# FangjinhuaWang/PatchmatchNet

Hardware: AMD Instinct MI355X
Metric: depth-maps/sec at 1600x1200 N=5 src views (higher is better)
Workload: dtype f32

## Files before the change

### include/pmn_hip.h

```cpp
#ifndef PMN_HIP_H
#define PMN_HIP_H

#include <stdint.h>

#ifdef __cplusplus
extern "C" {
#endif

#define PMN_ABI_VERSION 25
#define PMN_MLP_FLOATS 340
#define PMN_MAX_DEPTH 64
#define PMN_MAX_NEIGHBORS 17
#define PMN_MAX_FUSE_SRC 32
#define PMN_TSDF_MAX_VIEWS 16
#define PMN_TSDF_MARK_SPAN 8
#define PMN_RASTER_MAX_DIM 16384
#define PMN_RASTER_MAX_BOX 64
#define PMN_SPLAT_MAX_RADIUS 32

#define PMN_OK 0
#define PMN_ERR_ARG (-1)
#define PMN_ERR_SHAPE (-2)
#define PMN_ERR_LAUNCH (-3)

int pmn_abi_version(void);

const char *pmn_error_string(int code);

int pmn_nchw_to_nhwc(const float *in, float *out, int B, int C, int h, int w, void *stream);

int pmn_feature_weight(const float *ref_nhwc, const float *eval_offsets, const int *eval_table_host,
                       const float *mlp, int B, int C, int G, int K, int h, int w,
                       float *out_feature_weight, void *stream);

int pmn_init_hypotheses(const float *noise, const float *depth, int depth_shift, const float *depth_min,
                        const float *depth_max, int num_sample, float interval_scale, const float *propa_offsets,
                        const int *propa_table_host, int K, int B, int h, int w, float *depth_sample,
                        float *xnorm, void *stream);

int pmn_warp_correlate(const float *ref_nhwc, const float *src_nhwc, const float *rel_proj,
                       const float *depth_sample, const float *view_weights_in, int vw_shift,
                       const float *similarity_mlp, const float *pixelwise_mlp, int B, int N, int C,
                       int G, int D, int h, int w, int hs, int ws, float *cost_out, float *view_weights_out,
                       int *vw_argmax_out, float *similarity_out, void *stream);

int pmn_warp_correlate_views(const float *ref_nhwc, const void *src_view_table, const float *rel_proj,
                             const float *depth_sample, const float *view_weights_in, int vw_shift,
                             const float *similarity_mlp, const float *pixelwise_mlp, int B, int N, int C,
                             int G, int D, int h, int w, int hs, int ws, float *cost_out, float *view_weights_out,
                             int *vw_argmax_out, float *similarity_out, void *stream);

int pmn_aggregate_regress(const float *cost, const float *depth_sample, const float *xnorm,
                          const float *feature_weight, const float *eval_offsets, const int *eval_table_host,
                          int K, float interval_scale, int is_inverse, int B, int D, int h, int w,
                          float *score_out, float *depth_out, void *stream);

int pmn_confidence(const float *score, int B, int D, int h, int w, int H, int W, float *confidence_out,
                   int *depth_index_out, void *stream);

int pmn_conv2d(const float *in, const float *weights, const float *shift, const float *up, float *out, int N, int H,
               int W, int cin, int cout, int K, int stride, int pad, int dil, int relu, int in_nchw, int out_nchw,
               int up_h, int up_w, void *stream);

int pmn_fpn_tail(const float *x, const float *up, const float *w_in, const float *b_in, const float *w_out, float *out,
                 int N, int H, int W, int cin, int cmid, int cout, void *stream);

int pmn_conv2d_mfma(const float *in, const float *weights, const float *shift, float *out, float *out_b, int N, int H, int W,
                    int cin, int cout, int ca, int K, int stride, int pad, int dil, int relu, int planar, void *stream);


int pmn_conv2d_f16s(const float *in, const void *weights, const float *shift, float *out, int N, int H, int W, int cin, int cout,
                    int k, int stride, int relu, void *stream);

int pmn_conv2d_f16s_pair(const float *in, const void *weights_a, const float *shift_a, const void *weights_b, const float *shift_b,
                         float *out, int N, int H, int W, int channels, int relu, void *stream);

int pmn_offset_heads_f16s(const float *in, const void *weights, const float *shift, float *out_a, float *out_b, int N, int H, int W,
                          int cin, int cout, int ca, int dil, void *stream);

int pmn_fpn_level(const float *x, const float *u, const float *w, const float *b, float *out_a, float *out_b, int N, int H,
                  int W, int cin, int cout, int ca, void *stream);

int pmn_deconv3x3s2(const float *in, const float *weights, const float *shift, float *out, int N, int Hi, int Wi, int cin,
                    int cout, int relu, void *stream);

int pmn_refine_front(const float *img, const float *t2, const float *w0, const float *s0, const float *wd, const float *sd,
                     float *x16, int B, int H, int W, void *stream);
int pmn_refine_tail(const float *x16, const float *w3, const float *s3, const float *wr, const float *dnorm,
                    const float *depth_min, const float *depth_max, float *out, int B, int H, int W, void *stream);

int pmn_refine_fused(const float *img, const float *t2, const float *w0, const float *s0, const float *wd, const float *sd,
                     const void *w3a, const float *s3, const float *wr, const float *dnorm, const float *depth_min,
                     const float *depth_max, float *out, int B, int H, int W, void *stream);

int pmn_stage_projections(const float *intrinsics, const float *extrinsics, int B, int V, int nstages, float scale0,
                          float *rel, void *stream);

int pmn_stem(const float *img, const float *w0, const float *s0, const float *w1, const float *s1, float *out, int N, int H,
             int W, void *stream);

int pmn_stem_f16s(const float *img, const float *w0, const float *s0, const void *w1a, const float *s1, float *out, int N, int H,
                  int W, void *stream);

int pmn_stem_f16s_views(const float *const *img_table, int views, const float *w0, const float *s0, const void *w1a,
                        const float *s1, float *out, int B, int H, int W, void *stream);

int pmn_differentiable_warping(const float *src_nchw, const float *rel_proj, const float *depth, int B, int C,
                               int D, int h, int w, int hs, int ws, float *warped, void *stream);

int pmn_fuse_view(const float *maps, long long slot_stride, int ref_slot, const int *src_slots_host,
                  const int *src_hw_host, int n_src, const float *mats, int H, int W, float geo_pixel_thres, float geo_depth_thres, int geo_mask_thres,
                  float photo_thres, unsigned char *masks, float *xyz, double *depth_avg, int *geo_sum, void *stream);

int pmn_fuse_view_merged(const float *maps, long long slot_stride, int ref_slot, const int *src_slots_host,
                         const int *src_hw_host, int n_src, const float *mats, int H, int W, float geo_pixel_thres,
                         float geo_depth_thres, int geo_mask_thres, float photo_thres, unsigned char *masks, float *xyz,
                         double *depth_avg, int *geo_sum, unsigned char *claimed, long long claim_stride, unsigned char *emit,
                         void *stream);

int pmn_pack_points(const unsigned char *final_mask, const float *xyz, const void *image_hwc, int image_is_float, int H, int W,
                    unsigned char *records, long long capacity_points, long long *cursor, int *view_count, long long *scratch,
                    void *stream);

int pmn_pack_points_normals(const unsigned char *final_mask, const float *xyz, const float *normals_chw, const float *rotation,
                            int rotation_stride, const void *image_hwc, int image_is_float, int H, int W, unsigned char *records,
                            long long capacity_points, long long *cursor, int *view_count, long long *scratch, void *stream);

int pmn_depth_normals(const float *depth, int H, int W, const float *intrinsics_host, int radius, float rel_thres,
                      float *normals_out, void *stream);

int pmn_normalize_depth(const float *depth, const float *depth_min, const float *depth_max, int B, int n, float *out,
                        void *stream);

int pmn_check_f16_domain(const float *x, long long n, int *flag, void *stream);

#define PMN_PLAN_PART_PRE 0
#define PMN_PLAN_PART_SIDE 1
#define PMN_PLAN_PART_MAIN 2
#define PMN_PLAN_PART_POST 3
int pmn_plan_create(void **plan_out);
int pmn_plan_begin(void *plan);
int pmn_plan_end(void *plan);
int pmn_plan_count(const void *plan);
const char *pmn_plan_kernel_name(const void *plan, int index);
int pmn_plan_launch(const void *plan, void *stream);
int pmn_plan_destroy(void *plan);
int pmn_plan_fork(void *plan);
int pmn_plan_switch(void *plan, int branch);
int pmn_plan_join(void *plan);
int pmn_plan_entry_branch(const void *plan, int index);
int pmn_plan_launch_part(const void *plan, int part, void *stream);

int pmn_view_scores(const double *cam_centers, const double *xyz, const long long *obs_ptr, const int *obs_pt,
                    const long long *trk_ptr, const int *trk_img, int N, int P, long long n_obs, long long n_trk,
                    double theta0, double sigma1, double sigma2, double *score, void *stream);

#define PMN_METRICS_MAX_STAGES 4
#define PMN_METRICS_MAX_ITERS 5
#define PMN_METRICS_MAX_THRESHOLDS 8
#define PMN_METRICS_COUNT 0
#define PMN_METRICS_ABS 4
#define PMN_METRICS_THR 8
#define PMN_METRICS_SL1 16
#define PMN_METRICS_ROW 36
#define PMN_METRICS_PIXELS_PER_BLOCK 4096
#define PMN_METRICS_MAX_BLOCKS 128
#define PMN_METRICS_BLOCKS(H, W)                                                                                                     \
    ((int)((((long long)(H) * (W) + PMN_METRICS_PIXELS_PER_BLOCK - 1) / PMN_METRICS_PIXELS_PER_BLOCK) > PMN_METRICS_MAX_BLOCKS        \
               ? PMN_METRICS_MAX_BLOCKS                                                                                               \
               : (((long long)(H) * (W) + PMN_METRICS_PIXELS_PER_BLOCK - 1) / PMN_METRICS_PIXELS_PER_BLOCK)))
#define PMN_METRICS_SCRATCH(B, H, W) ((long long)(B) * PMN_METRICS_BLOCKS(H, W) * PMN_METRICS_ROW)
int pmn_depth_metrics(const float *depth_gt, const float *depth_min, const float *const *maps_host, const int *iters_host,
                      const int *hw_host, int stages, const float *thresholds_host, int n_thresholds, int B, int H, int W,
                      double *scratch, long long scratch_doubles, double *rows, void *stream);

int pmn_nn_distance(const float *to_xyz, const long long *to_keys, long long n_to, const double *origin_host, double cell,
                    const int *dims_host, const float *query, const int *order, long long n_from, double max_dist, double *dist,
                    int *index, void *stream);
int pmn_reduce_round(const float *xyz, const long long *keys, long long n, const double *origin_host, double cell,
                     const int *dims_host, double dst, const int *rank, unsigned char *state, unsigned int *counter, void *stream);

int pmn_tsdf_integrate(float *tsdf, float *weight, float *rgb, float *cweight, const int *dims_host, const float *origin_host,
                       float voxel, float trunc, const float *maps, long long slot_stride, const int *slots_host,
                       const int *hw_host, const void *const *masks_host, const void *const *images_host, const float *cams_host,
                       int n_views, void *stream);
int pmn_mt_count(const float *tsdf, const float *weight, const int *dims_host, float min_weight, unsigned char *vertex_mask,
                 unsigned char *cell_triangles, void *stream);
int pmn_mt_emit(const float *tsdf, const float *weight, const float *rgb, const float *cweight, const int *dims_host,
                const float *origin_host, float voxel, float min_weight, const unsigned char *vertex_mask,
                const unsigned char *cell_triangles, const int *vertex_scan, const int *triangle_scan, float *vertices,
                unsigned char *colors, float *normals, int *faces, void *stream);

int pmn_tsdf_mark_blocks(unsigned char *flags, int *overflow, const int *dims_host, const float *origin_host, float voxel, float trunc,
                         const float *maps, long long slot_stride, const int *slots_host, const int *hw_host,
                         const void *const *masks_host, const float *inv_cams_host, int n_views, void *stream);
int pmn_tsdf_integrate_blocks(float *tsdf, float *weight, float *rgb, float *cweight, const int *blocks, int n_blocks,
                              const int *dims_host, const float *origin_host, float voxel, float trunc, const float *maps,
                              long long slot_stride, const int *slots_host, const int *hw_host, const void *const *masks_host,
                              const void *const *images_host, const float *cams_host, int n_views, void *stream);
int pmn_mt_count_blocks(const float *tsdf, const float *weight, const int *table, const int *blocks, int n_blocks,
                        const int *dims_host, float min_weight, unsigned char *vertex_mask, unsigned char *cell_triangles, void *stream);
int pmn_mt_emit_blocks(const float *tsdf, const float *weight, const float *rgb, const float *cweight, const int *table,
                       const int *blocks, int n_blocks, const int *dims_host, const float *origin_host, float voxel, float min_weight,
                       const unsigned char *vertex_mask, const unsigned char *cell_triangles, const int *vertex_scan,
                       const int *triangle_scan, float *vertices, unsigned char *colors, float *normals, int *faces, void *stream);

int pmn_raster_triangles(const float *vertices, int n_vertices, const int *faces, int n_faces, const float *cam_host, int h, int w,
                         long long max_box, unsigned long long *keys, int *counters, int *worklist, void *stream);
int pmn_splat_points(const float *points, long long n_points, const float *cam_host, int h, int w, float radius_px, float radius_world,
                     unsigned long long *keys, int *counters, void *stream);
int pmn_raster_resolve(const unsigned long long *keys, int h, int w, const float *cam_host, const float *vertices, long long n_vertices,
                       const int *faces, long long n_faces, const unsigned char *colors, const float *normals, int shade, float *depth,
                       int *index, unsigned char *rgb, float *normal, void *stream);

#define PMN_ICP_SUMS 17
#define PMN_ICP_LIMBS 5
#define PMN_ICP_BLOCK_POINTS 256
#define PMN_ICP_BLOCKS(n) (((long long)(n) + PMN_ICP_BLOCK_POINTS - 1) / PMN_ICP_BLOCK_POINTS)
#define PMN_ICP_SCRATCH(n) (PMN_ICP_BLOCKS(n) * PMN_ICP_SUMS * PMN_ICP_LIMBS)
#define PMN_VOXEL_LONG_RUN 256
#define PMN_VOXEL_MAX_CHANNELS 8
#define PMN_CROP_MAX_VERTICES 4096
int pmn_icp_accumulate(const float *to_xyz, const long long *to_keys, long long n_to, const double *origin_host, double cell,
                       const int *dims_host, const float *src, const int *order, long long n, const double *pose_host,
                       const double *centre_host, double max_dist, double *scratch, long long scratch_doubles, double *sums,
                       void *stream);
int pmn_voxel_mean(const float *xyz, const float *attr, int channels, long long n, const long long *starts, long long m, float *out_xyz,
                   float *out_attr, void *stream);
int pmn_crop_prism(const float *xyz, long long n, const double *polygon, int k, int axis, double axis_min, double axis_max,
                   const double *pose_host, unsigned char *mask, void *stream);

int pmn_mesh_components(const int *faces, int n_faces, int n_vertices, int *label, int *invalid, void *stream);
int pmn_mesh_face_samples(const float *vertices, int n_vertices, const int *faces, int n_faces, double density, unsigned long long seed,
                          int *counts, int *invalid, void *stream);
int pmn_mesh_sample(const float *vertices, int n_vertices, const int *faces, int n_faces, const unsigned char *colors,
                    const long long *sample_scan, long long n_samples, unsigned long long seed, float *points, int *face,
                    unsigned char *out_colors, void *stream);

int pmn_undistort_image(const unsigned char *src, int Hs, int Ws, int channels, int model, const double *src_params_host,
                        const double *dst_pinhole_host, int Hd, int Wd, unsigned char *dst, unsigned char *valid, double *coords,
                        void *stream);

int pmn_knn_distance(const float *to_xyz, const long long *to_keys, long long n_to, const double *origin_host, double cell,
                     const int *dims_host, const float *query, const int *order, long long n_from, int k, double max_dist,
                     int same_cloud, double *d2, int *index, double *mean, void *stream);
int pmn_radius_count(const float *to_xyz, const long long *to_keys, long long n_to, const double *origin_host, double cell,
                     const int *dims_host, const float *query, const int *order, long long n_from, double radius, int same_cloud,
                     int *count, void *stream);

int pmn_mesh_distance(const float *ref_xyz, const long long *ref_keys, long long n_ref, const double *origin_host, double cell,
                      const int *dims_host, const int *entry_face, double radius, const float *vertices, int n_vertices,
                      const int *faces, int n_faces, const float *query, const int *order, long long n_query, double max_dist,
                      double *dist, int *face, double *closest, int *invalid, void *stream);

#define PMN_MESH_PLACE_LONG_RUN 256
#define PMN_MESH_SIMPLIFY_MAX_FACES 715827882
int pmn_mesh_remap_faces(const int *faces, int n_faces, int n_vertices, const int *cluster, int n_clusters, int *corner_cluster,
                         int *out_faces, unsigned char *flag, int *invalid, void *stream);
int pmn_mesh_cluster_place(const float *vertices, int n_vertices, const int *faces, int n_faces, const int *corners,
                           const long long *corner_starts, const long long *cluster_keys, int n_clusters, const float *mean,
                           const double *origin_host, double cell, const int *dims_host, double stiffness, float *out, void *stream);

#ifdef __cplusplus
}
#endif
#endif
```

### patchmatchnet_amd/_lib.py

```python
from __future__ import annotations

import ctypes
import os
import subprocess
from typing import Optional

_CSRC = os.path.join(os.path.dirname(os.path.abspath(__file__)), "csrc")
LIB_PATH = os.path.join(_CSRC, "libpmn_hip.so")
ABI_VERSION = 25
MLP_FLOATS = 340
MAX_DEPTH = 64
MAX_NEIGHBORS = 17
MAX_FUSE_SRC = 32
TSDF_MAX_VIEWS = 16
TSDF_MARK_SPAN = 8
RASTER_MAX_DIM = 16384
RASTER_MAX_BOX = 64
SPLAT_MAX_RADIUS = 32
ICP_SUMS = 17
ICP_LIMBS = 5
ICP_BLOCK_POINTS = 256
VOXEL_LONG_RUN = 256
VOXEL_MAX_CHANNELS = 8
CROP_MAX_VERTICES = 4096
MESH_PLACE_LONG_RUN = 256
MESH_SIMPLIFY_MAX_FACES = 715827882

_fp = ctypes.c_void_p
_ip = ctypes.c_void_p
_hp = ctypes.c_void_p
_i = ctypes.c_int
_f = ctypes.c_float
_s = ctypes.c_void_p

SIGNATURES = {
    "pmn_abi_version": [],
    "pmn_error_string": [_i],
    "pmn_nchw_to_nhwc": [_fp, _fp, _i, _i, _i, _i, _s],
    "pmn_feature_weight": [_fp, _fp, _hp, _fp, _i, _i, _i, _i, _i, _i, _fp, _s],
    "pmn_init_hypotheses": [_fp, _fp, _i, _fp, _fp, _i, _f, _fp, _hp, _i, _i, _i, _i, _fp, _fp, _s],
    "pmn_warp_correlate": [_fp, _fp, _fp, _fp, _fp, _i, _fp, _fp, _i, _i, _i, _i, _i, _i, _i, _i, _i, _fp, _fp, _ip,
                           _fp, _s],
    "pmn_warp_correlate_views": [_fp, _fp, _fp, _fp, _fp, _i, _fp, _fp, _i, _i, _i, _i, _i, _i, _i, _i, _i, _fp, _fp, _ip,
                                 _fp, _s],
    "pmn_aggregate_regress": [_fp, _fp, _fp, _fp, _fp, _hp, _i, _f, _i, _i, _i, _i, _i, _fp, _fp, _s],
    "pmn_confidence": [_fp, _i, _i, _i, _i, _i, _i, _fp, _ip, _s],
    "pmn_conv2d": [_fp, _fp, _fp, _fp, _fp] + [_i] * 14 + [_s],
    "pmn_fpn_tail": [_fp] * 6 + [_i] * 6 + [_s],
    "pmn_fpn_level": [_fp] * 6 + [_i] * 6 + [_s],
    "pmn_conv2d_f16s": [_fp] * 4 + [_i] * 8 + [_s],
    "pmn_offset_heads_f16s": [_fp] * 5 + [_i] * 7 + [_s],
    "pmn_conv2d_f16s_pair": [_fp] * 6 + [_i] * 5 + [_s],
    "pmn_refine_front": [_fp] * 7 + [_i] * 3 + [_s],
    "pmn_refine_tail": [_fp] * 8 + [_i] * 3 + [_s],
    "pmn_refine_fused": [_fp] * 13 + [_i] * 3 + [_s],
    "pmn_conv2d_mfma": [_fp] * 5 + [_i] * 12 + [_s],
    "pmn_deconv3x3s2": [_fp] * 4 + [_i] * 6 + [_s],
    "pmn_stage_projections": [_fp, _fp, _i, _i, _i, _f, _fp, _s],
    "pmn_stem": [_fp] * 6 + [_i] * 3 + [_s],
    "pmn_stem_f16s": [_fp] * 6 + [_i] * 3 + [_s],
    "pmn_stem_f16s_views": [_fp, _i] + [_fp] * 5 + [_i] * 3 + [_s],
    "pmn_differentiable_warping": [_fp, _fp, _fp, _i, _i, _i, _i, _i, _i, _i, _fp, _s],
    "pmn_fuse_view": [_fp, ctypes.c_longlong, _i, _hp, _hp, _i, _fp, _i, _i, _f, _f, _i, _f, _fp, _fp, _fp, _ip, _s],
    "pmn_fuse_view_merged": [_fp, ctypes.c_longlong, _i, _hp, _hp, _i, _fp, _i, _i, _f, _f, _i, _f, _fp, _fp, _fp, _ip, _fp,
                             ctypes.c_longlong, _fp, _s],
    "pmn_pack_points": [_fp, _fp, _fp, _i, _i, _i, _fp, ctypes.c_longlong, _fp, _ip, _fp, _s],
    "pmn_pack_points_normals": [_fp, _fp, _fp, _fp, _i, _fp, _i, _i, _i, _fp, ctypes.c_longlong, _fp, _ip, _fp, _s],
    "pmn_depth_normals": [_fp, _i, _i, _hp, _i, _f, _fp, _s],
    "pmn_normalize_depth": [_fp, _fp, _fp, _i, _i, _fp, _s],
    "pmn_check_f16_domain": [_fp, ctypes.c_longlong, _ip, _s],
    "pmn_plan_create": [ctypes.POINTER(ctypes.c_void_p)],
    "pmn_plan_begin": [_hp],
    "pmn_plan_end": [_hp],
    "pmn_plan_count": [_hp],
    "pmn_plan_kernel_name": [_hp, _i],
    "pmn_plan_launch": [_hp, _s],
    "pmn_plan_destroy": [_hp],
    "pmn_plan_fork": [_hp],
    "pmn_plan_switch": [_hp, _i],
    "pmn_plan_join": [_hp],
    "pmn_plan_entry_branch": [_hp, _i],
    "pmn_plan_launch_part": [_hp, _i, _s],
    "pmn_view_scores": [_fp] * 6 + [_i, _i, ctypes.c_longlong, ctypes.c_longlong] + [ctypes.c_double] * 3 + [_fp, _s],
    "pmn_depth_metrics": [_fp, _fp, _hp, _hp, _hp, _i, _hp, _i, _i, _i, _i, _fp, ctypes.c_longlong, _fp, _s],
    "pmn_nn_distance": [_fp, _ip, ctypes.c_longlong, _hp, ctypes.c_double, _hp, _fp, _ip, ctypes.c_longlong, ctypes.c_double, _fp, _ip,
                        _s],
    "pmn_reduce_round": [_fp, _ip, ctypes.c_longlong, _hp, ctypes.c_double, _hp, ctypes.c_double, _ip, _ip, _ip, _s],
    "pmn_tsdf_integrate": [_fp] * 4 + [_hp, _hp, _f, _f, _fp, ctypes.c_longlong] + [_hp] * 5 + [_i, _s],
    "pmn_mt_count": [_fp, _fp, _hp, _f, _ip, _ip, _s],
    "pmn_mt_emit": [_fp] * 4 + [_hp, _hp, _f, _f] + [_ip] * 4 + [_fp, _ip, _fp, _ip, _s],
    "pmn_tsdf_mark_blocks": [_ip, _ip, _hp, _hp, _f, _f, _fp, ctypes.c_longlong] + [_hp] * 4 + [_i, _s],
    "pmn_tsdf_integrate_blocks": [_fp] * 4 + [_ip, _i, _hp, _hp, _f, _f, _fp, ctypes.c_longlong] + [_hp] * 5 + [_i, _s],
    "pmn_mt_count_blocks": [_fp, _fp, _ip, _ip, _i, _hp, _f, _ip, _ip, _s],
    "pmn_mt_emit_blocks": [_fp] * 4 + [_ip, _ip, _i, _hp, _hp, _f, _f] + [_ip] * 4 + [_fp, _ip, _fp, _ip, _s],
    "pmn_raster_triangles": [_fp, _i, _ip, _i, _hp, _i, _i, ctypes.c_longlong, _ip, _ip, _ip, _s],
    "pmn_splat_points": [_fp, ctypes.c_longlong, _hp, _i, _i, _f, _f, _ip, _ip, _s],
    "pmn_raster_resolve": [_ip, _i, _i, _hp, _fp, ctypes.c_longlong, _ip, ctypes.c_longlong, _ip, _fp, _i, _fp, _ip, _ip, _fp, _s],
    "pmn_icp_accumulate": [_fp, _ip, ctypes.c_longlong, _hp, ctypes.c_double, _hp, _fp, _ip, ctypes.c_longlong, _hp, _hp, ctypes.c_double,
                           _fp, ctypes.c_longlong, _fp, _s],
    "pmn_voxel_mean": [_fp, _fp, _i, ctypes.c_longlong, _ip, ctypes.c_longlong, _fp, _fp, _s],
    "pmn_crop_prism": [_fp, ctypes.c_longlong, _fp, _i, _i, ctypes.c_double, ctypes.c_double, _hp, _ip, _s],
    "pmn_mesh_components": [_ip, _i, _i, _ip, _ip, _s],
    "pmn_mesh_face_samples": [_fp, _i, _ip, _i, ctypes.c_double, ctypes.c_ulonglong, _ip, _ip, _s],
    "pmn_mesh_sample": [_fp, _i, _ip, _i, _ip, _ip, ctypes.c_longlong, ctypes.c_ulonglong, _fp, _ip, _ip, _s],
    "pmn_undistort_image": [_fp, _i, _i, _i, _i, _hp, _hp, _i, _i, _fp, _fp, _fp, _s],
    "pmn_knn_distance": [_fp, _ip, ctypes.c_longlong, _hp, ctypes.c_double, _hp, _fp, _ip, ctypes.c_longlong, _i, ctypes.c_double, _i,
                         _fp, _ip, _fp, _s],
    "pmn_radius_count": [_fp, _ip, ctypes.c_longlong, _hp, ctypes.c_double, _hp, _fp, _ip, ctypes.c_longlong, ctypes.c_double, _i, _ip,
                         _s],
    "pmn_mesh_distance": [_fp, _ip, ctypes.c_longlong, _hp, ctypes.c_double, _hp, _ip, ctypes.c_double, _fp, _i, _ip, _i, _fp, _ip,
                          ctypes.c_longlong, ctypes.c_double, _fp, _ip, _fp, _ip, _s],
    "pmn_mesh_remap_faces": [_ip, _i, _i, _ip, _i, _ip, _ip, _ip, _ip, _s],
    "pmn_mesh_cluster_place": [_fp, _i, _ip, _i, _ip, _ip, _ip, _i, _fp, _hp, ctypes.c_double, _hp, ctypes.c_double, _fp, _s],
}

PLAN_PART_PRE, PLAN_PART_SIDE, PLAN_PART_MAIN, PLAN_PART_POST = 0, 1, 2, 3

METRICS_MAX_STAGES = 4
METRICS_MAX_ITERS = 5
METRICS_MAX_THRESHOLDS = 8
METRICS_COUNT, METRICS_ABS, METRICS_THR, METRICS_SL1 = 0, 4, 8, 16
METRICS_ROW = 36
METRICS_PIXELS_PER_BLOCK = 4096
METRICS_MAX_BLOCKS = 128


def metrics_scratch(B: int, H: int, W: int) -> int:
    return B * min(METRICS_MAX_BLOCKS, -(-H * W // METRICS_PIXELS_PER_BLOCK)) * METRICS_ROW

def icp_scratch(n: int) -> int:
    return -(-n // ICP_BLOCK_POINTS) * ICP_SUMS * ICP_LIMBS


EXPERIMENTAL_SIGNATURES = {"pmn_set_tuning": [_i, _i],
                           "pmn_conv3x3_wino": [_fp] * 4 + [_i] * 5 + [_s],
                           "pmn_conv5x5s2_wino": [_fp] * 4 + [_i] * 6 + [_s]}
EXPERIMENTAL_LIB_PATH = os.path.join(_CSRC, "libpmn_hip_experimental.so")


def experimental() -> bool:
    return os.environ.get("PMN_EXPERIMENTAL", "") == "1"


_LIB: Optional[ctypes.CDLL] = None


class PmnError(RuntimeError):
    pass


def build(force: bool = False, verbose: bool = False) -> str:
    args = ["make", "-C", _CSRC, "-j4"] + (["-B"] if force else []) + (["EXPERIMENTAL=1"] if experimental() else [])
    if not verbose:
        args.insert(1, "-s")
    subprocess.check_call(args)
    return LIB_PATH


def lib() -> ctypes.CDLL:
    global _LIB
    if _LIB is None:
        path, sigs = LIB_PATH, SIGNATURES
        if experimental():
            path, sigs = EXPERIMENTAL_LIB_PATH, {**SIGNATURES, **EXPERIMENTAL_SIGNATURES}
        if not os.path.isfile(path):
            raise PmnError(f"{path} not found: build it with `python -c 'import __graft_entry__ as g; g.build()'` "
                           f"or `make -C patchmatchnet_amd/csrc` -- patchmatchnet_amd has no fallback path")
        L = (ctypes.CDLL if os.environ.get("PMN_CTYPES", "") == "cdll" else ctypes.PyDLL)(path)
        for name, argtypes in sigs.items():
            try:
                fn = getattr(L, name)
            except AttributeError as e:
                raise PmnError(f"libpmn_hip.so does not export {name}") from e
            fn.argtypes = argtypes
            fn.restype = ctypes.c_char_p if name in ("pmn_error_string", "pmn_plan_kernel_name") else ctypes.c_int
        if L.pmn_abi_version() != ABI_VERSION:
            raise PmnError(f"libpmn_hip.so ABI {L.pmn_abi_version()} != expected {ABI_VERSION}: rebuild")
        _LIB = L
    return _LIB


def check(code: int, what: str) -> None:
    if code != 0:
        raise PmnError(f"{what} failed: {lib().pmn_error_string(code).decode()} (code {code})")
```

### patchmatchnet_amd/csrc/aggregate.hip

```cpp
#include <cstring>

#include "pmn_common.hpp"
#define PMN_DIV_DM1(acc, D) ((acc) / (float)((D) - 1))

struct AggArgs {
    const float* cost;
    const float* depth;
    const float* xnorm;
    const float* fweight;
    const float* offsets;
    float* score;
    float* depth_out;
    int K, is_inverse, B, D, h, w;
    float interval_scale;
    int table[2 * PMN_MAX_NEIGHBORS];
};

template <int KMAX, int DL>
__global__ __launch_bounds__(PMN_BLOCK, (KMAX <= 9 ? 3 : 1)) void aggregate_regress_kernel(const AggArgs a) {
#pragma clang fp contract(off)
    constexpr int NPX = PMN_BLOCK / DL;
    __shared__ float red[DL][NPX];
    __shared__ float red2[DL][NPX];
    const int h = a.h, w = a.w, hw = h * w, D = a.D, K = a.K;
    const int px = threadIdx.x % NPX, dl = threadIdx.x / NPX;
    const int p_raw = blockIdx.x * NPX + px;
    const bool ok = p_raw < hw;
    const int p = ok ? p_raw : hw - 1;
    const int b = blockIdx.y;
    const int y = p / w, x = p - y * w;

    int off[KMAX];
    float w00[KMAX], w01[KMAX], w10[KMAX], w11[KMAX], fw[KMAX];
#pragma unroll
    for (int k = 0; k < KMAX; ++k) {
        off[k] = 0;
        w00[k] = w01[k] = w10[k] = w11[k] = fw[k] = 0.0f;
        if (k < K) {
            const float ox = a.offsets[((size_t)b * 2 * K + 2 * k) * hw + p];
            const float oy = a.offsets[((size_t)b * 2 * K + 2 * k + 1) * hw + p];
            float ix, iy;
            pmn_neighbor_position((float)x, (float)y, a.table[2 * k], a.table[2 * k + 1], ox, oy, h, w, ix, iy);
            const PmnTaps t = pmn_make_taps(ix, iy, h, w);
            off[k] = t.off;
            w00[k] = t.w00;
            w01[k] = t.w01;
            w10[k] = t.w10;
            w11[k] = t.w11;
            fw[k] = a.fweight[((size_t)b * K + k) * hw + p];
        }
    }

    float smax = -__builtin_inff();
#pragma unroll 1
    for (int d = dl; d < D; d += DL) {
        const float* xp = a.xnorm + (size_t)b * hw * D + d;
        const float* cp = a.cost + (size_t)b * hw * D + d;
        const float xc = xp[(size_t)p * D];
        float wk[KMAX], ck[KMAX];
        float wsum = 0.0f;
#pragma unroll
        for (int k = 0; k < KMAX; ++k) {
            wk[k] = 0.0f;
            ck[k] = 0.0f;
            if (k < K) {
                const size_t o = (size_t)off[k] * D, o1 = o + D, o2 = o + (size_t)w * D, o3 = o2 + D;
                const float x1 = fmaf(xp[o3], w11[k], fmaf(xp[o2], w10[k], fmaf(xp[o1], w01[k], xp[o] * w00[k])));
                ck[k] = fmaf(cp[o3], w11[k], fmaf(cp[o2], w10[k], fmaf(cp[o1], w01[k], cp[o] * w00[k])));
                float t = fabsf(x1 - xc) / a.interval_scale;
                t = fminf(fmaxf(t, 0.0f), 4.0f);
                wk[k] = pmn_sigmoid(4.0f - 2.0f * t) * fw[k];
                wsum = wsum + wk[k];
            }
        }
        float s = 0.0f;
#pragma unroll
        for (int k = 0; k < KMAX; ++k)
            if (k < K) s = s + ck[k] * (wk[k] / wsum);
        if (ok) a.score[((size_t)b * D + d) * hw + p] = s;
        smax = fmaxf(smax, s);
    }
    red[dl][px] = smax;
    __syncthreads();
#pragma unroll
    for (int i = 0; i < DL; ++i) smax = fmaxf(smax, red[i][px]);
    __syncthreads();

    float esum = 0.0f;
#pragma unroll 1
    for (int d = dl; d < D; d += DL)
        if (ok) esum = esum + expf(a.score[((size_t)b * D + d) * hw + p] - smax);
    red[dl][px] = esum;
    __syncthreads();
    esum = 0.0f;
#pragma unroll
    for (int i = 0; i < DL; ++i) esum = esum + red[i][px];
    const float lse = logf(esum);

    float acc = 0.0f;
#pragma unroll 1
    for (int d = dl; d < D; d += DL) {
        if (ok) {
            const size_t o = ((size_t)b * D + d) * hw + p;
            const float prob = expf((a.score[o] - smax) - lse);
            a.score[o] = prob;
            acc = acc + (a.is_inverse ? (float)d : a.depth[o]) * prob;
        }
    }
    red2[dl][px] = acc;
    __syncthreads();
    if (dl != 0 || !ok) return;
    acc = 0.0f;
#pragma unroll
    for (int i = 0; i < DL; ++i) acc = acc + red2[i][px];
    float out = acc;
    if (a.is_inverse) {
        const float inv_min = 1.0f / a.depth[((size_t)b * D + (D - 1)) * hw + p];
        const float inv_max = 1.0f / a.depth[((size_t)b * D) * hw + p];
        const float inv = inv_max + PMN_DIV_DM1(acc, D) * (inv_min - inv_max);
        out = 1.0f / inv;
    }
    a.depth_out[(size_t)b * hw + p] = out;
}

__device__ __forceinline__ float sigmoid_rcp(float x) {
    const float d = 1.0f + __builtin_amdgcn_exp2f(x * -1.4426950408889634f);
    float r = __builtin_amdgcn_rcpf(d);
    return r * fmaf(-d, r, 2.0f);
}

template <int G, int SL>
__device__ __forceinline__ int agg_group_bcast_i(int v) {
    static_assert(G == 2 || G == 4 || G == 8 || G == 16, "lane groups inside a DPP row");
    if constexpr (G == 2) {
        return __builtin_amdgcn_mov_dpp(v, SL | (SL << 2) | ((2 + SL) << 4) | ((2 + SL) << 6), 0xF, 0xF, true);
    } else if constexpr (G == 4) {
        return __builtin_amdgcn_mov_dpp(v, SL | (SL << 2) | (SL << 4) | (SL << 6), 0xF, 0xF, true);
    } else if constexpr (G == 16) {
        return __builtin_amdgcn_mov_dpp(v, 0x150 + SL, 0xF, 0xF, true);
    } else {
        const int lo = __builtin_amdgcn_update_dpp(v, v, 0x150 + SL, 0xF, 0x3, false);
        return __builtin_amdgcn_update_dpp(lo, v, 0x150 + 8 + SL, 0xF, 0xC, false);
    }
}
template <int G, int SL>
__device__ __forceinline__ float agg_group_bcast_f(float v) {
    return __int_as_float(agg_group_bcast_i<G, SL>(__float_as_int(v)));
}

template <int KMAX>
__device__ __forceinline__ void agg_form_tap_set(const AggArgs& a, int b, int k, int p, int x, int y, int& off, float& w00, float& w01,
                                                 float& w10, float& w11, float& fw) {
    const int h = a.h, w = a.w, hw = h * w, K = a.K;
    const float ox = a.offsets[((size_t)b * 2 * K + 2 * k) * hw + p];
    const float oy = a.offsets[((size_t)b * 2 * K + 2 * k + 1) * hw + p];
    float ix, iy;
    pmn_neighbor_position((float)x, (float)y, a.table[2 * k], a.table[2 * k + 1], ox, oy, h, w, ix, iy);
    const PmnTaps t = pmn_make_taps(ix, iy, h, w);
    off = t.off;
    w00 = t.w00;
    w01 = t.w01;
    w10 = t.w10;
    w11 = t.w11;
    fw = a.fweight[((size_t)b * K + k) * hw + p];
}

template <int KMAX, int DQT>
__global__ __launch_bounds__(PMN_BLOCK, (KMAX <= 9 ? 3 : 1)) void aggregate_regress_q4_kernel(const AggArgs a) {
#pragma clang fp contract(off)
    __shared__ float red[PMN_BLOCK];
    const int h = a.h, w = a.w, hw = h * w, D = a.D, K = a.K, DQ = DQT > 0 ? DQT : D >> 2;
    const int npx = blockDim.x / DQ;
    const int px = threadIdx.x / DQ, q = threadIdx.x - px * DQ;
    const int p_raw = blockIdx.x * npx + px;
    const bool ok = p_raw < hw;
    const int p = ok ? p_raw : hw - 1;
    const int b = blockIdx.y;
    const int y = p / w, x = p - y * w;

    int off[KMAX];
    float w00[KMAX], w01[KMAX], w10[KMAX], w11[KMAX], fw[KMAX];
    if constexpr (DQT > 1) {
        constexpr int KPT = (KMAX + DQT - 1) / DQT;
        int moff[KPT];
        float m00[KPT], m01[KPT], m10[KPT], m11[KPT], mfw[KPT];
#pragma unroll
        for (int i = 0; i < KPT; ++i) {
            const int k = q + i * DQT;
            moff[i] = 0;
            m00[i] = m01[i] = m10[i] = m11[i] = mfw[i] = 0.0f;
            if (k < K) agg_form_tap_set<KMAX>(a, b, k, p, x, y, moff[i], m00[i], m01[i], m10[i], m11[i], mfw[i]);
        }
#define AGG_TAKE(k_)                                                                                         \
    if constexpr ((k_) < KMAX) {                                                                               \
        constexpr int sl_ = (k_) % DQT, it_ = (k_) / DQT;                                                      \
        off[k_] = agg_group_bcast_i<DQT, sl_>(moff[it_]);                                                      \
        w00[k_] = agg_group_bcast_f<DQT, sl_>(m00[it_]);                                                       \
        w01[k_] = agg_group_bcast_f<DQT, sl_>(m01[it_]);                                                       \
        w10[k_] = agg_group_bcast_f<DQT, sl_>(m10[it_]);                                                       \
        w11[k_] = agg_group_bcast_f<DQT, sl_>(m11[it_]);                                                       \
        fw[k_] = agg_group_bcast_f<DQT, sl_>(mfw[it_]);                                                        \
    }
        AGG_TAKE(0) AGG_TAKE(1) AGG_TAKE(2) AGG_TAKE(3) AGG_TAKE(4) AGG_TAKE(5) AGG_TAKE(6) AGG_TAKE(7) AGG_TAKE(8)
        static_assert(KMAX <= 9, "AGG_TAKE list");
#undef AGG_TAKE
    } else {
#pragma unroll
        for (int k = 0; k < KMAX; ++k) {
            off[k] = 0;
            w00[k] = w01[k] = w10[k] = w11[k] = fw[k] = 0.0f;
            if (k < K) agg_form_tap_set<KMAX>(a, b, k, p, x, y, off[k], w00[k], w01[k], w10[k], w11[k], fw[k]);
        }
    }

    const float inv_interval = 1.0f / a.interval_scale;
    const float* xn = a.xnorm + (size_t)b * hw * D + 4 * q;
    const float* cs = a.cost + (size_t)b * hw * D + 4 * q;
    const float4 xc4 = *reinterpret_cast<const float4*>(xn + (size_t)p * D);
    const float xc[4] = {xc4.x, xc4.y, xc4.z, xc4.w};
    float wk[KMAX][4], ck[KMAX][4], wsum[4] = {0.f, 0.f, 0.f, 0.f};
#pragma unroll
    for (int k = 0; k < KMAX; ++k) {
#pragma unroll
        for (int j = 0; j < 4; ++j) wk[k][j] = ck[k][j] = 0.0f;
        if (k < K) {
            const size_t o = (size_t)off[k] * D, o2 = o + (size_t)w * D;
            const float4 xa = *reinterpret_cast<const float4*>(xn + o), xb = *reinterpret_cast<const float4*>(xn + o + D);
            const float4 xcn = *reinterpret_cast<const float4*>(xn + o2), xd = *reinterpret_cast<const float4*>(xn + o2 + D);
            const float4 ca = *reinterpret_cast<const float4*>(cs + o), cb = *reinterpret_cast<const float4*>(cs + o + D);
            const float4 cc = *reinterpret_cast<const float4*>(cs + o2), cd = *reinterpret_cast<const float4*>(cs + o2 + D);
            const float x00[4] = {xa.x, xa.y, xa.z, xa.w}, x01[4] = {xb.x, xb.y, xb.z, xb.w};
            const float x10[4] = {xcn.x, xcn.y, xcn.z, xcn.w}, x11[4] = {xd.x, xd.y, xd.z, xd.w};
            const float c00[4] = {ca.x, ca.y, ca.z, ca.w}, c01[4] = {cb.x, cb.y, cb.z, cb.w};
            const float c10[4] = {cc.x, cc.y, cc.z, cc.w}, c11[4] = {cd.x, cd.y, cd.z, cd.w};
#pragma unroll
            for (int j = 0; j < 4; ++j) {
                const float x1 = fmaf(x11[j], w11[k], fmaf(x10[j], w10[k], fmaf(x01[j], w01[k], x00[j] * w00[k])));
                ck[k][j] = fmaf(c11[j], w11[k], fmaf(c10[j], w10[k], fmaf(c01[j], w01[k], c00[j] * w00[k])));
                float t = fabsf(x1 - xc[j]) * inv_interval;
                t = fminf(fmaxf(t, 0.0f), 4.0f);
                wk[k][j] = sigmoid_rcp(4.0f - 2.0f * t) * fw[k];
                wsum[j] = wsum[j] + wk[k][j];
            }
        }
    }
    float s[4] = {0.f, 0.f, 0.f, 0.f}, rsum[4];
#pragma unroll
    for (int j = 0; j < 4; ++j) rsum[j] = 1.0f / wsum[j];
#pragma unroll
    for (int k = 0; k < KMAX; ++k)
        if (k < K) {
#pragma unroll
            for (int j = 0; j < 4; ++j) s[j] = s[j] + ck[k][j] * (wk[k][j] * rsum[j]);
        }

    float smax = fmaxf(fmaxf(s[0], s[1]), fmaxf(s[2], s[3]));
    red[threadIdx.x] = smax;
    __syncthreads();
    for (int i = 0; i < DQ; ++i) smax = fmaxf(smax, red[px * DQ + i]);
    __syncthreads();
    float esum = ((expf(s[0] - smax) + expf(s[1] - smax)) + expf(s[2] - smax)) + expf(s[3] - smax);
    red[threadIdx.x] = esum;
    __syncthreads();
    esum = 0.0f;
    for (int i = 0; i < DQ; ++i) esum = esum + red[px * DQ + i];
    __syncthreads();
    const float lse = logf(esum);
    float acc = 0.0f;
#pragma unroll
    for (int j = 0; j < 4; ++j) {
        const int d = 4 * q + j;
        const size_t o = ((size_t)b * D + d) * hw + p;
        const float prob = expf((s[j] - smax) - lse);
        if (ok) a.score[o] = prob;
        acc = acc + (a.is_inverse ? (float)d : a.depth[o]) * prob;
    }
    red[threadIdx.x] = acc;
    __syncthreads();
    if (q != 0 || !ok) return;
    acc = 0.0f;
    for (int i = 0; i < DQ; ++i) acc = acc + red[px * DQ + i];
    float out = acc;
    if (a.is_inverse) {
        const float inv_min = 1.0f / a.depth[((size_t)b * D + (D - 1)) * hw + p];
        const float inv_max = 1.0f / a.depth[((size_t)b * D) * hw + p];
        const float inv = inv_max + PMN_DIV_DM1(acc, D) * (inv_min - inv_max);
        out = 1.0f / inv;
    }
    a.depth_out[(size_t)b * hw + p] = out;
}

template <int KMAX>
static int launch_agg_q4(const AggArgs& a, hipStream_t s) {
    const int DQ = a.D / 4, npx = PMN_BLOCK / DQ;
    const dim3 grid((a.h * a.w + npx - 1) / npx, a.B), block(npx * DQ);
    if (DQ == 2) PMN_LAUNCH((aggregate_regress_q4_kernel<KMAX, 2>), grid, block, 0, s, a);
    else if (DQ == 4) PMN_LAUNCH((aggregate_regress_q4_kernel<KMAX, 4>), grid, block, 0, s, a);
    else if (DQ == 8) PMN_LAUNCH((aggregate_regress_q4_kernel<KMAX, 8>), grid, block, 0, s, a);
    else if (DQ == 16) PMN_LAUNCH((aggregate_regress_q4_kernel<KMAX, 16>), grid, block, 0, s, a);
    else PMN_LAUNCH((aggregate_regress_q4_kernel<KMAX, 0>), grid, block, 0, s, a);
    PMN_CHECK_LAUNCH();
    return PMN_OK;
}

template <int KMAX, int DL>
static int launch_agg_dl(const AggArgs& a, hipStream_t s) {
    constexpr int NPX = PMN_BLOCK / DL;
    const dim3 grid((a.h * a.w + NPX - 1) / NPX, a.B), block(PMN_BLOCK);
    PMN_LAUNCH((aggregate_regress_kernel<KMAX, DL>), grid, block, 0, s, a);
    PMN_CHECK_LAUNCH();
    return PMN_OK;
}

template <int KMAX>
static int launch_agg(const AggArgs& a, hipStream_t s) {
    if constexpr (KMAX <= 9) {
        if (a.D % 4 == 0) return launch_agg_q4<KMAX>(a, s);
    }
    if (a.D >= 32) return launch_agg_dl<KMAX, 16>(a, s);
    if (a.D >= 16) return launch_agg_dl<KMAX, 4>(a, s);
    return launch_agg_dl<KMAX, 1>(a, s);
}

extern "C" int pmn_aggregate_regress(const float* cost, const float* depth_sample, const float* xnorm,
                                     const float* feature_weight, const float* eval_offsets, const int* eval_table_host,
                                     int K, float interval_scale, int is_inverse, int B, int D, int h, int w,
                                     float* score_out, float* depth_out, void* stream) {
    if (!cost || !depth_sample || !xnorm || !feature_weight || !eval_offsets || !eval_table_host || !score_out ||
        !depth_out)
        return PMN_ERR_ARG;
    if (B < 1 || D < 1 || h < 2 || w < 2) return PMN_ERR_ARG;
    if (K < 1 || K > PMN_MAX_NEIGHBORS || D > PMN_MAX_DEPTH) return PMN_ERR_SHAPE;
    if (is_inverse && D < 2) return PMN_ERR_ARG;
    AggArgs a;
    memset(&a, 0, sizeof(a));
    a.cost = cost;
    a.depth = depth_sample;
    a.xnorm = xnorm;
    a.fweight = feature_weight;
    a.offsets = eval_offsets;
    a.score = score_out;
    a.depth_out = depth_out;
    a.K = K;
    a.is_inverse = is_inverse;
    a.B = B; a.D = D; a.h = h; a.w = w;
    a.interval_scale = interval_scale;
    for (int i = 0; i < 2 * K; ++i) a.table[i] = eval_table_host[i];
    if (K <= 9) return launch_agg<9>(a, (hipStream_t)stream);
    return launch_agg<17>(a, (hipStream_t)stream);
}
```

### patchmatchnet_amd/csrc/gather_corr.hip

```cpp
#include <type_traits>

#include "gather_common.hpp"


template <int LPI, int SL>
__device__ __forceinline__ int group_bcast_i(int v) {
    if constexpr (LPI == 4) {
        return __builtin_amdgcn_mov_dpp(v, SL | (SL << 2) | (SL << 4) | (SL << 6), 0xF, 0xF, true);
    } else if constexpr (LPI == 16) {
        return __builtin_amdgcn_mov_dpp(v, 0x150 + SL, 0xF, 0xF, true);
    } else {
        const int lo = __builtin_amdgcn_update_dpp(v, v, 0x150 + SL, 0xF, 0x3, false);
        return __builtin_amdgcn_update_dpp(lo, v, 0x150 + 8 + SL, 0xF, 0xC, false);
    }
}
template <int LPI, int SL>
__device__ __forceinline__ float group_bcast_f(float v) {
    return __int_as_float(group_bcast_i<LPI, SL>(__float_as_int(v)));
}

template <int C>
__device__ __forceinline__ const char* pmn_view_base(const GatherArgs& a, int v, int b, int hs, int ws) {
    if (a.src_tab) return reinterpret_cast<const char*>(a.src_tab[v]) + ((size_t)b * hs * ws) * (C * 4);
    return reinterpret_cast<const char*>(a.src) + ((size_t)(v * a.B + b) * hs * ws) * (C * 4);
}

struct PmnCorners { float4 t00, t01, t10, t11; };

typedef float pmn_f4n __attribute__((ext_vector_type(4)));
typedef const pmn_f4n __attribute__((address_space(1))) * pmn_gptr4;
__device__ __forceinline__ float4 pmn_global_load4(const char __attribute__((address_space(1))) * p) {
    const pmn_f4n v = *(pmn_gptr4)p;
    return make_float4(v.x, v.y, v.z, v.w);
}
template <int C>
__device__ __forceinline__ PmnCorners load_corners(const char* __restrict__ sbase, const unsigned bo, const unsigned row_bytes) {
    typedef const char __attribute__((address_space(1))) * gptr1;
    const gptr1 g = (gptr1)sbase;
    PmnCorners c;
    c.t00 = pmn_global_load4(g + bo);
    c.t01 = pmn_global_load4(g + bo + C * 4);
    c.t10 = pmn_global_load4(g + (bo + row_bytes));
    c.t11 = pmn_global_load4(g + (bo + row_bytes) + C * 4);
    return c;
}

template <int LPG, int CG>
__device__ __forceinline__ float blend_corners(const PmnCorners& c, float4 w4, const float4 refq) {
    w4 = pmn_settle4(w4);
    const pmn_f2 wa = {w4.x, w4.x}, wb = {w4.y, w4.y}, wc = {w4.z, w4.z}, wd = {w4.w, w4.w};
    pmn_f2 lo = pmn_f2{c.t00.x, c.t00.y} * wa;
    pmn_f2 hi = pmn_f2{c.t00.z, c.t00.w} * wa;
    lo = __builtin_elementwise_fma(pmn_f2{c.t01.x, c.t01.y}, wb, lo);
    hi = __builtin_elementwise_fma(pmn_f2{c.t01.z, c.t01.w}, wb, hi);
    lo = __builtin_elementwise_fma(pmn_f2{c.t10.x, c.t10.y}, wc, lo);
    hi = __builtin_elementwise_fma(pmn_f2{c.t10.z, c.t10.w}, wc, hi);
    lo = __builtin_elementwise_fma(pmn_f2{c.t11.x, c.t11.y}, wd, lo);
    hi = __builtin_elementwise_fma(pmn_f2{c.t11.z, c.t11.w}, wd, hi);
    float s = fmaf(hi.y, refq.w, fmaf(hi.x, refq.z, fmaf(lo.y, refq.y, lo.x * refq.x)));
    if (LPG == 2) s += pmn_pair_swap(s);
    return s * (1.0f / CG);
}

template <int C, int G, int MODE, int DT, bool EXACT>
__global__ __launch_bounds__(PMN_BLOCK, (MODE == MODE_PIXELWISE ? 3 : (MODE == MODE_NEIGHBOR && DT <= 16) ? 5 : 4)) void gather_corr_kernel(const GatherArgs a) {
    constexpr int LPI = C / 4;
    constexpr int NPIX = PMN_BLOCK / LPI;
    constexpr int CG = C / G;
    constexpr int LPG = CG / 4;
    constexpr int PAD = 32 / G;
    constexpr int DSTEP = PMN_BLOCK / NPIX;
    constexpr int NIT = DT / DSTEP;
    constexpr int NI_MAX = (MODE == MODE_PIXELWISE) ? 2 : 4;
    constexpr int NI = NIT < NI_MAX ? NIT : NI_MAX;
    static_assert(CG == 4 || CG == 8, "group size must be 4 or 8 channels");
    static_assert(NIT >= 1, "DT must cover at least one hypothesis per item-role thread");

    const int tid = threadIdx.x;
    const int b = blockIdx.y;
    const int tile = pmn_xcd_tile(blockIdx.x, a.ntiles);
    constexpr int DEXACT = (MODE == MODE_NEIGHBOR) ? (DT == 16 ? 9 : 17) : DT;
    const int D = EXACT ? DEXACT : a.D;
    const int N = a.N, h = a.h, w = a.w, hs = a.hs, ws = a.ws;
    const int hw = h * w;
    const int items = NPIX * D;
    const int SS = items + PAD;
    const int p0 = tile * NPIX;

    extern __shared__ float4 smem4[];
    float* simt = reinterpret_cast<float*>(smem4);
    float* wlds_a = simt + ((G * SS + 3) & ~3);
    float* wlds_b = wlds_a + MLP_LDS_FLOATS;
    unsigned long long* vwkey = reinterpret_cast<unsigned long long*>(wlds_b + MLP_LDS_FLOATS);
    int* tab = reinterpret_cast<int*>(vwkey + NPIX);

    for (int i = tid; i < PMN_MLP_FLOATS; i += PMN_BLOCK) {
        wlds_a[i] = a.mlp_a[i];
        if (MODE == MODE_PIXELWISE) wlds_b[i] = a.mlp_b[i];
    }
    if (MODE == MODE_NEIGHBOR) {
#pragma unroll
        for (int i = 0; i < 2 * PMN_MAX_NEIGHBORS; ++i)
            if (tid == i) tab[i] = a.table[i];
    }

    const int pixA = tid % NPIX, dA0 = tid / NPIX;
    const int pA = p0 + pixA;
    const bool okA = pA < hw;
    const int yA = okA ? pA / w : 0, xA = okA ? pA - yA * w : 0;

    const int grp = tid / LPI, lc = tid % LPI;
    const int pB = p0 + grp;
    const bool okB = pB < hw;
    float4 refq = make_float4(0.f, 0.f, 0.f, 0.f);
    if (okB) refq = reinterpret_cast<const float4*>(a.ref)[((size_t)b * hw + pB) * LPI + lc];
    const int yB = okB ? pB / w : 0, xB = okB ? pB - yB * w : 0;
    const int wv = w >> a.vw_shift, hwv = (h >> a.vw_shift) * wv;
    const int vw_idx = (yB >> a.vw_shift) * wv + (xB >> a.vw_shift);
    const bool owner = (lc % LPG) == 0;
    const int gB = lc / LPG;


    if (MODE == MODE_VIEWS) {
        constexpr int RPL = DT / LPI;
        static_assert(DT % LPI == 0, "DT is a multiple of the lane-group size");
        float acc[DT];
#pragma unroll
        for (int d = 0; d < DT; ++d) acc[d] = 0.0f;
        const float xf = (float)xB, yf = (float)yB;
        float rdep[RPL];
#pragma unroll
        for (int j = 0; j < RPL; ++j) {
            const int d = lc + j * LPI;
            rdep[j] = (okB && d < D) ? a.depth[((size_t)b * D + d) * hw + pB] : -1.0f;
        }
        for (int v = 0; v < N; ++v) {
            const PmnPose lane_pose = pmn_make_pose(a.proj + ((size_t)b * N + v) * 16, xf, yf, h, w);
            float rw00[RPL], rw01[RPL], rw10[RPL], rw11[RPL];
            int roff[RPL];
#pragma unroll
            for (int j = 0; j < RPL; ++j) {
                const int d = lc + j * LPI;
                PmnTaps t;
                t.off = 0;
                t.w00 = t.w01 = t.w10 = t.w11 = 0.0f;
                if (okB && d < D) {
                    float ix, iy;
                    pmn_pose_position(lane_pose, rdep[j], h, w, hs, ws, ix, iy);
                    t = pmn_make_taps(ix, iy, hs, ws);
                }
                rw00[j] = t.w00; rw01[j] = t.w01; rw10[j] = t.w10; rw11[j] = t.w11;
                roff[j] = t.off;
            }
            const char* sbase = pmn_view_base<C>(a, v, b, hs, ws);
            const unsigned lane_bytes = lc * 16u, row_bytes = (unsigned)ws * (C * 4);
            const float vw = okB ? a.vw_in[((size_t)b * N + v) * hwv + vw_idx] : 0.0f;
            constexpr int NB = 2;
            static_assert(DT % NB == 0, "hypothesis bound is a multiple of the batch");
#pragma unroll
            for (int d0 = 0; d0 < DT; d0 += NB) {
                PmnCorners cn[NB];
                float4 wq[NB];
#pragma unroll
                for (int i = 0; i < NB; ++i) {
                    const int d = d0 + i;
                    if (EXACT || d < D) {
                        float4 w4;
                        int off;
#define PMN_BCAST_CASE(SL)                                                    \
    case SL:                                                                  \
        w4.x = group_bcast_f<LPI, SL>(rw00[d / LPI]);                         \
        w4.y = group_bcast_f<LPI, SL>(rw01[d / LPI]);                         \
        w4.z = group_bcast_f<LPI, SL>(rw10[d / LPI]);                         \
        w4.w = group_bcast_f<LPI, SL>(rw11[d / LPI]);                         \
        off = group_bcast_i<LPI, SL>(roff[d / LPI]);                          \
        break;
                        switch (d % LPI) {
                            PMN_BCAST_CASE(0) PMN_BCAST_CASE(1) PMN_BCAST_CASE(2) PMN_BCAST_CASE(3)
                            PMN_BCAST_CASE(4) PMN_BCAST_CASE(5) PMN_BCAST_CASE(6) PMN_BCAST_CASE(7)
                            PMN_BCAST_CASE(8) PMN_BCAST_CASE(9) PMN_BCAST_CASE(10) PMN_BCAST_CASE(11)
                            PMN_BCAST_CASE(12) PMN_BCAST_CASE(13) PMN_BCAST_CASE(14) PMN_BCAST_CASE(15)
                            default: w4 = make_float4(0.f, 0.f, 0.f, 0.f); off = 0; break;
                        }
#undef PMN_BCAST_CASE
                        wq[i] = w4;
                        cn[i] = load_corners<C>(sbase, (unsigned)off * (C * 4) + lane_bytes, row_bytes);
                    }
                }
                __builtin_amdgcn_sched_barrier(0);
#pragma unroll
                for (int i = 0; i < NB; ++i) {
                    const int d = d0 + i;
                    if (EXACT || d < D) acc[d] = mul_add_unfused(acc[d], blend_corners<LPG, CG>(cn[i], wq[i], refq), vw);
                }
                __builtin_amdgcn_sched_barrier(0);
            }
        }
        if (owner) {
#pragma unroll
            for (int d = 0; d < DT; ++d)
                if (d < D) simt[gB * SS + d * NPIX + grp] = acc[d];
        }
        __syncthreads();
        if (!okA) return;
        float wtot = 1e-5f;
        const int vwi = (yA >> a.vw_shift) * wv + (xA >> a.vw_shift);
        for (int v = 0; v < N; ++v) wtot += a.vw_in[((size_t)b * N + v) * hwv + vwi];
        float x[NIT][G], o[NIT];
#pragma unroll
        for (int j = 0; j < NIT; ++j) {
            const int d = min(dA0 + j * DSTEP, D - 1);
#pragma unroll
            for (int g = 0; g < G; ++g) x[j][g] = simt[g * SS + d * NPIX + pixA] / wtot;
        }
        mlp_items<G, NIT, NI>(wlds_a, x, o);
#pragma unroll
        for (int j = 0; j < NIT; ++j) {
            const int d = dA0 + j * DSTEP;
            if (d < D) {
                if (a.sim_out) {
#pragma unroll
                    for (int g = 0; g < G; ++g) a.sim_out[(((size_t)b * G + g) * D + d) * hw + pA] = x[j][g];
                }
                a.out[((size_t)b * hw + pA) * D + d] = o[j];
            }
        }
        return;
    }

    float ssum[NIT][G];
#pragma unroll
    for (int j = 0; j < NIT; ++j)
#pragma unroll
        for (int g = 0; g < G; ++g) ssum[j][g] = 0.0f;
    float wsum = 1e-5f;
    __syncthreads();

    for (int v = 0; v < N; ++v) {
        if (MODE == MODE_PIXELWISE && tid < NPIX) vwkey[tid] = 0ull;
        const char* sbase = MODE == MODE_NEIGHBOR ? reinterpret_cast<const char*>(a.ref) + ((size_t)b * hs * ws) * (C * 4)
                                                  : pmn_view_base<C>(a, v, b, hs, ws);
        const unsigned lane_bytes = lc * 16u, row_bytes = (unsigned)ws * (C * 4);
        if constexpr (MODE == MODE_PIXELWISE) {
            constexpr int RPL = DT / LPI;
            const float xf = (float)xB, yf = (float)yB;
            const PmnPose lane_pose = pmn_make_pose(a.proj + ((size_t)b * N + v) * 16, xf, yf, h, w);
            float rw00[RPL], rw01[RPL], rw10[RPL], rw11[RPL];
            int roff[RPL];
#pragma unroll
            for (int j = 0; j < RPL; ++j) {
                const int d = lc + j * LPI;
                PmnTaps t;
                t.off = 0;
                t.w00 = t.w01 = t.w10 = t.w11 = 0.0f;
                if (okB && d < D) {
                    float ix, iy;
                    pmn_pose_position(lane_pose, a.depth[((size_t)b * D + d) * hw + pB], h, w, hs, ws, ix, iy);
                    t = pmn_make_taps(ix, iy, hs, ws);
                }
                rw00[j] = t.w00; rw01[j] = t.w01; rw10[j] = t.w10; rw11[j] = t.w11;
                roff[j] = t.off;
            }
            constexpr int NB = 2;
#pragma unroll
            for (int d0 = 0; d0 < DT; d0 += NB) {
                PmnCorners cn[NB];
                float4 wq[NB];
#pragma unroll
                for (int i = 0; i < NB; ++i) {
                    const int d = d0 + i;
                    if (EXACT || d < D) {
                        float4 w4;
                        int off;
#define PMN_BCAST_CASE(SL)                                                    \
    case SL:                                                                  \
        w4.x = group_bcast_f<LPI, SL>(rw00[d / LPI]);                         \
        w4.y = group_bcast_f<LPI, SL>(rw01[d / LPI]);                         \
        w4.z = group_bcast_f<LPI, SL>(rw10[d / LPI]);                         \
        w4.w = group_bcast_f<LPI, SL>(rw11[d / LPI]);                         \
        off = group_bcast_i<LPI, SL>(roff[d / LPI]);                          \
        break;
                        switch (d % LPI) {
                            PMN_BCAST_CASE(0) PMN_BCAST_CASE(1) PMN_BCAST_CASE(2) PMN_BCAST_CASE(3)
                            PMN_BCAST_CASE(4) PMN_BCAST_CASE(5) PMN_BCAST_CASE(6) PMN_BCAST_CASE(7)
                            PMN_BCAST_CASE(8) PMN_BCAST_CASE(9) PMN_BCAST_CASE(10) PMN_BCAST_CASE(11)
                            PMN_BCAST_CASE(12) PMN_BCAST_CASE(13) PMN_BCAST_CASE(14) PMN_BCAST_CASE(15)
                            default: w4 = make_float4(0.f, 0.f, 0.f, 0.f); off = 0; break;
                        }
#undef PMN_BCAST_CASE
                        wq[i] = w4;
                        cn[i] = load_corners<C>(sbase, (unsigned)off * (C * 4) + lane_bytes, row_bytes);
                    }
                }
                __builtin_amdgcn_sched_barrier(0);
#pragma unroll
                for (int i = 0; i < NB; ++i) {
                    const int d = d0 + i;
                    if (EXACT || d < D) {
                        const float s = blend_corners<LPG, CG>(cn[i], wq[i], refq);
                        if (owner) simt[gB * SS + d * NPIX + grp] = s;
                    }
                }
                __builtin_amdgcn_sched_barrier(0);
            }
            __syncthreads();
        } else if constexpr (MODE == MODE_NEIGHBOR) {
// ... 134 lines not shown
        for (int j = 0; j < NIT; ++j) {
            const int d = min(dA0 + j * DSTEP, D - 1);
#pragma unroll
            for (int g = 0; g < G; ++g) ssum[j][g] = mul_add_unfused(ssum[j][g], pmn_settle(simt[g * SS + d * NPIX + pixA]), vwp);
        }
        wsum += vwp;
        if (tid < NPIX && okA) {
            const size_t o = ((size_t)b * N + v) * hw + pA;
            a.vw_out[o] = vwp;
            if (a.vw_argmax) a.vw_argmax[o] = (int)(0xFFFFFFFFu - (unsigned)(key & 0xFFFFFFFFull));
        }
        __syncthreads();
    }

    if constexpr (MODE == MODE_NEIGHBOR) return;
    if (!okA) return;
    float o[NIT];
#pragma unroll
    for (int j = 0; j < NIT; ++j)
#pragma unroll
        for (int g = 0; g < G; ++g) ssum[j][g] = ssum[j][g] / wsum;
    mlp_items<G, NIT, NI>(wlds_a, ssum, o);
#pragma unroll
    for (int j = 0; j < NIT; ++j) {
        const int d = dA0 + j * DSTEP;
        if (d < D) {
            if (a.sim_out) {
#pragma unroll
                for (int g = 0; g < G; ++g) a.sim_out[(((size_t)b * G + g) * D + d) * hw + pA] = ssum[j][g];
            }
            a.out[((size_t)b * hw + pA) * D + d] = o[j];
        }
    }
}

template <int LPI>
__device__ __forceinline__ void bcast_record(const int sl, const float r00, const float r01, const float r10, const float r11,
                                             const int ro, float4& w4, int& off) {
#define PMN_BCAST_CASE(SL)                      \
    case SL:                                    \
        w4.x = group_bcast_f<LPI, SL>(r00);     \
        w4.y = group_bcast_f<LPI, SL>(r01);     \
        w4.z = group_bcast_f<LPI, SL>(r10);     \
        w4.w = group_bcast_f<LPI, SL>(r11);     \
        off = group_bcast_i<LPI, SL>(ro);       \
        break;
    switch (sl) {
        PMN_BCAST_CASE(0) PMN_BCAST_CASE(1) PMN_BCAST_CASE(2) PMN_BCAST_CASE(3)
        PMN_BCAST_CASE(4) PMN_BCAST_CASE(5) PMN_BCAST_CASE(6) PMN_BCAST_CASE(7)
        PMN_BCAST_CASE(8) PMN_BCAST_CASE(9) PMN_BCAST_CASE(10) PMN_BCAST_CASE(11)
        PMN_BCAST_CASE(12) PMN_BCAST_CASE(13) PMN_BCAST_CASE(14) PMN_BCAST_CASE(15)
        default: w4 = make_float4(0.f, 0.f, 0.f, 0.f); off = 0; break;
    }
#undef PMN_BCAST_CASE
}

template <int CTRL>
__device__ __forceinline__ unsigned long long dpp_max_u64(const unsigned long long v) {
    const int lo = (int)(unsigned)(v & 0xFFFFFFFFull), hi = (int)(unsigned)(v >> 32);
    const unsigned olo = (unsigned)__builtin_amdgcn_update_dpp(lo, lo, CTRL, 0xF, 0xF, false);
    const unsigned ohi = (unsigned)__builtin_amdgcn_update_dpp(hi, hi, CTRL, 0xF, 0xF, false);
    const unsigned long long o = ((unsigned long long)ohi << 32) | olo;
    return o > v ? o : v;
}

#ifndef PMN_PW
#define PMN_PW 2
#endif
#ifndef PMN_PW_WAVES
#define PMN_PW_WAVES 4
#endif
#ifndef PMN_PW_INTERLEAVE
#define PMN_PW_INTERLEAVE 1
#endif

template <int PW, bool EXACT>
__global__ __launch_bounds__(PMN_BLOCK, PMN_PW_WAVES) void pixelwise_wave_kernel(const GatherArgs a) {
    constexpr int C = 64, G = 8, DT = 64, LPI = 16, CG = 8, LPG = 2;
    constexpr int LGP = 4 / PW;
    constexpr int DL = DT / LGP;
    constexpr int RPL = DL / LPI;
    constexpr int LPP = 64 / PW;
    constexpr int NIT = DT / LPP;
    constexpr int GS = DT + 4;
    constexpr int PS = G * GS;
    constexpr int WPB = PMN_BLOCK / 64;
    constexpr int NPIX = WPB * PW;
    constexpr bool IL = PMN_PW_INTERLEAVE != 0 && LGP > 1;
    auto hyp_of = [](int kk, int il) { return IL ? kk + LGP * il : kk * DL + il; };
    static_assert(PW == 4 || PW == 2, "pixels per wave");
    static_assert(NIT % 2 == 0, "PixelwiseNet runs on pairs of items");

    const int tid = threadIdx.x, wave = tid >> 6, lane = tid & 63;
    const int b = blockIdx.y;
    const int tile = pmn_xcd_tile(blockIdx.x, a.ntiles);
    const int D = EXACT ? DT : a.D;
    const int N = a.N, h = a.h, w = a.w, hs = a.hs, ws = a.ws;
    const int hw = h * w;
    const int pw0 = tile * NPIX + wave * PW;

    extern __shared__ float4 smem4[];
    float* wlds_a = reinterpret_cast<float*>(smem4);
    float* wlds_b = wlds_a + MLP_LDS_FLOATS;
    float* simw = wlds_b + MLP_LDS_FLOATS + wave * (PW * PS);
    for (int i = tid; i < PMN_MLP_FLOATS; i += PMN_BLOCK) {
        wlds_a[i] = a.mlp_a[i];
        wlds_b[i] = a.mlp_b[i];
    }
    __syncthreads();

    const int lg = lane >> 4, lc = lane & 15;
    const int pl = lg / LGP, k = lg % LGP;
    const int pB = pw0 + pl;
    const bool okB = pB < hw;
    float4 refq = make_float4(0.f, 0.f, 0.f, 0.f);
    if (okB) refq = reinterpret_cast<const float4*>(a.ref)[((size_t)b * hw + pB) * LPI + lc];
    const int yB = okB ? pB / w : 0, xB = okB ? pB - yB * w : 0;
    const bool owner = (lc % LPG) == 0;
    const int gB = lc / LPG;
    float rdep[RPL];
    bool rok[RPL];
#pragma unroll
    for (int j = 0; j < RPL; ++j) {
        const int d = hyp_of(k, lc + j * LPI);
        rok[j] = okB && (EXACT || d < D);
        rdep[j] = rok[j] ? a.depth[((size_t)b * D + d) * hw + pB] : 1.0f;
    }
    float* srow = simw + pl * PS + gB * GS + k * DL;

    const int pi = lane / LPP, q = lane % LPP;
    const int d0 = q * NIT;
    const int pA = pw0 + pi;
    const bool okA = pA < hw;
    const float* xrow = simw + pi * PS + d0;

    float ssum[NIT][G];
#pragma unroll
    for (int j = 0; j < NIT; ++j)
#pragma unroll
        for (int g = 0; g < G; ++g) ssum[j][g] = 0.0f;
    float wsum = 1e-5f;
    const float xf = (float)xB, yf = (float)yB;
    const unsigned lane_bytes = lc * 16u, row_bytes = (unsigned)ws * (C * 4);

    for (int v = 0; v < N; ++v) {
        const PmnPose lane_pose = pmn_make_pose(a.proj + ((size_t)b * N + v) * 16, xf, yf, h, w);
        float rw00[RPL], rw01[RPL], rw10[RPL], rw11[RPL];
        int roff[RPL];
#pragma unroll
        for (int j = 0; j < RPL; ++j) {
            PmnTaps t;
            t.off = 0;
            t.w00 = t.w01 = t.w10 = t.w11 = 0.0f;
            if (rok[j]) {
                float ix, iy;
                pmn_pose_position(lane_pose, rdep[j], h, w, hs, ws, ix, iy);
                t = pmn_make_taps(ix, iy, hs, ws);
            }
            rw00[j] = t.w00; rw01[j] = t.w01; rw10[j] = t.w10; rw11[j] = t.w11;
            roff[j] = t.off;
        }
        const char* sbase = pmn_view_base<C>(a, v, b, hs, ws);
        constexpr int NB = 2;
#pragma unroll
        for (int i0 = 0; i0 < DL; i0 += 2 * NB) {
            float sv[2 * NB];
#pragma unroll
            for (int hb = 0; hb < 2; ++hb) {
                PmnCorners cn[NB];
                float4 wq[NB];
#pragma unroll
                for (int i = 0; i < NB; ++i) {
                    const int il = i0 + hb * NB + i;
                    float4 w4;
                    int off;
                    bcast_record<LPI>(il % LPI, rw00[il / LPI], rw01[il / LPI], rw10[il / LPI], rw11[il / LPI], roff[il / LPI], w4, off);
                    wq[i] = w4;
                    cn[i] = load_corners<C>(sbase, (unsigned)off * (C * 4) + lane_bytes, row_bytes);
                }
                __builtin_amdgcn_sched_barrier(0);
#pragma unroll
                for (int i = 0; i < NB; ++i) sv[hb * NB + i] = blend_corners<LPG, CG>(cn[i], wq[i], refq);
                __builtin_amdgcn_sched_barrier(0);
            }
            if (owner) *reinterpret_cast<float4*>(srow + i0) = make_float4(sv[0], sv[1], sv[2], sv[3]);
        }
        __builtin_amdgcn_fence(__ATOMIC_RELEASE, "wavefront");
        __builtin_amdgcn_wave_barrier();
        __builtin_amdgcn_fence(__ATOMIC_ACQUIRE, "wavefront");

        float x[NIT][G];
        if constexpr (NIT == 2) {
#pragma unroll
            for (int g = 0; g < G; ++g) {
                const float2 t2 = *reinterpret_cast<const float2*>(xrow + g * GS);
                x[0][g] = t2.x; x[1][g] = t2.y;
            }
#pragma unroll
            for (int g = 0; g < G; ++g) {
                x[0][g] = pmn_settle(x[0][g]); x[1][g] = pmn_settle(x[1][g]);
            }
        }
        unsigned long long best = 0ull;
#pragma unroll
        for (int c = 0; c < NIT / 2; ++c) {
            pmn_f2 xq[1][G], rq[1];
#pragma unroll
            for (int g = 0; g < G; ++g) {
                if constexpr (NIT == 2) {
                    xq[0][g] = pmn_f2{x[0][g], x[1][g]};
                } else {
                    const float2 t2 = *reinterpret_cast<const float2*>(xrow + g * GS + 2 * c);
                    xq[0][g] = pmn_f2{pmn_settle(t2.x), pmn_settle(t2.y)};
                }
            }
            mlp_pairs_from_lds<G, 1>(wlds_b, xq, rq);
            const float r[2] = {rq[0].x, rq[0].y};
#pragma unroll
            for (int i = 0; i < 2; ++i) {
                const int d = hyp_of((d0 + 2 * c + i) / DL, (d0 + 2 * c + i) % DL);
                if (EXACT || d < D) {
                    const unsigned long long key = ((unsigned long long)__float_as_uint(pmn_sigmoid(r[i])) << 32) |
                                                   (unsigned long long)(0xFFFFFFFFu - (unsigned)d);
                    best = key > best ? key : best;
                }
            }
        }
        best = dpp_max_u64<0xB1>(best);
        best = dpp_max_u64<0x4E>(best);
        best = dpp_max_u64<0x124>(best);
        best = dpp_max_u64<0x128>(best);
        if constexpr (LPP == 32) {
            const unsigned long long o = __shfl_xor(best, 16, 64);
            best = o > best ? o : best;
        }
        const float vwp = __uint_as_float((unsigned)(best >> 32));
        if constexpr (NIT == 4) {
#pragma unroll
            for (int g = 0; g < G; ++g) {
                const float4 t4 = pmn_settle4(*reinterpret_cast<const float4*>(xrow + g * GS));
                x[0][g] = t4.x; x[1][g] = t4.y; x[2][g] = t4.z; x[3][g] = t4.w;
            }
        }
#pragma unroll
        for (int j = 0; j < NIT; ++j)
#pragma unroll
            for (int g = 0; g < G; ++g) ssum[j][g] = mul_add_unfused(ssum[j][g], x[j][g], vwp);
        wsum += vwp;
        if (q == 0 && okA) {
            const size_t o = ((size_t)b * N + v) * hw + pA;
            a.vw_out[o] = vwp;
            if (a.vw_argmax) a.vw_argmax[o] = (int)(0xFFFFFFFFu - (unsigned)(best & 0xFFFFFFFFull));
        }
        __builtin_amdgcn_fence(__ATOMIC_RELEASE, "wavefront");
        __builtin_amdgcn_wave_barrier();
    }

    if (!okA) return;
    float o[NIT];
#pragma unroll
    for (int j = 0; j < NIT; ++j)
#pragma unroll
        for (int g = 0; g < G; ++g) ssum[j][g] = ssum[j][g] / wsum;
    mlp_items<G, NIT, 2>(wlds_a, ssum, o);
    float* orow = a.out + ((size_t)b * hw + pA) * D + d0;
    if constexpr (IL) {
#pragma unroll
        for (int j = 0; j < NIT; ++j) {
            const int d = hyp_of((d0 + j) / DL, (d0 + j) % DL);
            if (EXACT || d < D) a.out[((size_t)b * hw + pA) * D + d] = o[j];
        }
    } else if constexpr (EXACT) {
        if constexpr (NIT == 4) *reinterpret_cast<float4*>(orow) = make_float4(o[0], o[1], o[2], o[3]);
        else *reinterpret_cast<float2*>(orow) = make_float2(o[0], o[1]);
    } else {
#pragma unroll
        for (int j = 0; j < NIT; ++j)
            if (d0 + j < D) orow[j] = o[j];
    }
    if (a.sim_out) {
#pragma unroll
        for (int j = 0; j < NIT; ++j) {
            const int d = hyp_of((d0 + j) / DL, (d0 + j) % DL);
            if (d < D) {
#pragma unroll
                for (int g = 0; g < G; ++g) a.sim_out[(((size_t)b * G + g) * D + d) * hw + pA] = ssum[j][g];
            }
        }
    }
}

template <int PW>
static int launch_pixelwise_wave(GatherArgs& a, hipStream_t stream) {
    constexpr int NPIX = (PMN_BLOCK / 64) * PW, PS = 8 * (64 + 4);
    a.ntiles = (a.h * a.w + NPIX - 1) / NPIX;
    const size_t lds = (size_t)2 * MLP_LDS_FLOATS * 4 + (size_t)NPIX * PS * 4;
    if (a.D == 64) {
        PMN_LAUNCH((pixelwise_wave_kernel<PW, true>), dim3(a.ntiles, a.B), dim3(PMN_BLOCK), lds, stream, a);
    } else {
        PMN_LAUNCH((pixelwise_wave_kernel<PW, false>), dim3(a.ntiles, a.B), dim3(PMN_BLOCK), lds, stream, a);
    }
    PMN_CHECK_LAUNCH();
    return PMN_OK;
}


template <int C, int G, int MODE, int DT, bool EXACT>
static int launch_gather_impl(GatherArgs& a, hipStream_t stream) {
    constexpr int LPI = C / 4, NPIX = PMN_BLOCK / LPI, PAD = 32 / G;
    const int hw = a.h * a.w;
    a.ntiles = (hw + NPIX - 1) / NPIX;
    const int items = NPIX * a.D, SS = items + PAD;
    size_t lds = (size_t)((G * SS + 3) & ~3) * 4 + 2 * MLP_LDS_FLOATS * 4 + NPIX * 8 +
                 2 * PMN_MAX_NEIGHBORS * 4;
    lds = (lds + 15) & ~(size_t)15;
    auto kern = gather_corr_kernel<C, G, MODE, DT, EXACT>;
    if (lds > 160 * 1024) return PMN_ERR_SHAPE;
    if (lds > 48 * 1024) {
        const int rc = pmn_raise_dynamic_lds(reinterpret_cast<const void*>(kern), lds);
        if (rc != PMN_OK) return rc;
    }
    PMN_LAUNCH(kern, dim3(a.ntiles, a.B), dim3(PMN_BLOCK), lds, stream, a);
    PMN_CHECK_LAUNCH();
    return PMN_OK;
}

template <int C, int G, int MODE, int DT>
static int launch_gather(GatherArgs& a, hipStream_t stream) {
    if constexpr (MODE == MODE_VIEWS || MODE == MODE_PIXELWISE) {
        if (a.D == DT) return launch_gather_impl<C, G, MODE, DT, true>(a, stream);
    } else {
        if (a.D == (DT == 16 ? 9 : 17)) return launch_gather_impl<C, G, MODE, DT, true>(a, stream);
    }
    return launch_gather_impl<C, G, MODE, DT, false>(a, stream);
}

template <int C, int G, int MODE>
static int dispatch_depth(GatherArgs& a, hipStream_t stream) {
    constexpr int DSTEP = C / 4;
    if constexpr (MODE == MODE_PIXELWISE) {
        return launch_gather<C, G, MODE, 64>(a, stream);
    } else if constexpr (MODE == MODE_NEIGHBOR) {
        if (a.D <= 16) return launch_gather<C, G, MODE, 16>(a, stream);
        return launch_gather<C, G, MODE, 32>(a, stream);
    } else {
        if constexpr (DSTEP <= 8) {
            if (a.D <= 8) return launch_gather<C, G, MODE, 8>(a, stream);
        }
        if (a.D <= 16) return launch_gather<C, G, MODE, 16>(a, stream);
        if (a.D <= 32) return launch_gather<C, G, MODE, 32>(a, stream);
        return launch_gather<C, G, MODE, 64>(a, stream);
    }
}

template <int MODE>
static int dispatch_gather(GatherArgs& a, int C, int G, hipStream_t stream) {
    if (C == 64 && G == 8) return dispatch_depth<64, 8, MODE>(a, stream);
    if (C == 32 && G == 8) return dispatch_depth<32, 8, MODE>(a, stream);
    if (C == 16 && G == 4) return dispatch_depth<16, 4, MODE>(a, stream);
    return PMN_ERR_SHAPE;
}

static int warp_correlate_impl(const float* ref_nhwc, const float* src_nhwc, const unsigned long long* src_table,
                               const float* rel_proj, const float* depth_sample, const float* view_weights_in, int vw_shift,
                               const float* similarity_mlp, const float* pixelwise_mlp, int B, int N, int C, int G,
                               int D, int h, int w, int hs, int ws, float* cost_out, float* view_weights_out,
                               int* vw_argmax_out, float* similarity_out, void* stream) {
    if (!ref_nhwc || (!src_nhwc && !src_table) || !rel_proj || !depth_sample || !similarity_mlp || !cost_out) return PMN_ERR_ARG;
    if (!view_weights_in && (!pixelwise_mlp || !view_weights_out)) return PMN_ERR_ARG;
    if (B < 1 || N < 1 || D < 1 || h < 2 || w < 2 || hs < 2 || ws < 2 || vw_shift < 0 || vw_shift > 2) return PMN_ERR_ARG;
    if (D > PMN_MAX_DEPTH) return PMN_ERR_SHAPE;
    if ((h | w) & ((1 << vw_shift) - 1)) return PMN_ERR_ARG;
    GatherArgs a;
    memset(&a, 0, sizeof(a));
    a.ref = ref_nhwc;
    a.src = src_nhwc;
    a.src_tab = src_table;
    a.proj = rel_proj;
    a.depth = depth_sample;
    a.vw_in = view_weights_in;
    a.mlp_a = similarity_mlp;
    a.mlp_b = pixelwise_mlp;
    a.vw_out = view_weights_out;
    a.vw_argmax = vw_argmax_out;
    a.sim_out = similarity_out;
    a.out = cost_out;
    a.B = B; a.N = N; a.D = D; a.h = h; a.w = w; a.hs = hs; a.ws = ws;
    a.vw_shift = vw_shift;
#ifdef PMN_EXPERIMENTAL
    const int flags = src_table ? 0 : pmn_gather_flags();
    const bool pixelwise = view_weights_in == nullptr;
    if (flags & 64) {
        const int rc = pmn_launch_corr_mfma(a, C, G, pixelwise, (hipStream_t)stream);
        if (rc != PMN_ERR_SHAPE) return rc;
    }
    if ((flags & 32) && !pixelwise) {
        const int rc = pmn_launch_gather_tile(a, C, G, (hipStream_t)stream);
        if (rc != PMN_ERR_SHAPE) return rc;
    }
    if ((flags & 1) && !(flags & (pixelwise ? 4 : 8))) {
        const int rc = (flags & 16) ? pmn_launch_gather_win(a, C, G, pixelwise, (hipStream_t)stream)
                                    : pmn_launch_gather_lane(a, C, G, pixelwise, (hipStream_t)stream);
        if (rc != PMN_ERR_SHAPE) return rc;
    }
#endif
    if (view_weights_in) return dispatch_gather<MODE_VIEWS>(a, C, G, (hipStream_t)stream);
#if PMN_PW != 0
    if (C == 64 && G == 8 && D <= 64) return launch_pixelwise_wave<PMN_PW>(a, (hipStream_t)stream);
#endif
    return dispatch_gather<MODE_PIXELWISE>(a, C, G, (hipStream_t)stream);
}

extern "C" int pmn_warp_correlate(const float* ref_nhwc, const float* src_nhwc, const float* rel_proj,
                                  const float* depth_sample, const float* view_weights_in, int vw_shift,
                                  const float* similarity_mlp, const float* pixelwise_mlp, int B, int N, int C, int G,
                                  int D, int h, int w, int hs, int ws, float* cost_out, float* view_weights_out,
                                  int* vw_argmax_out, float* similarity_out, void* stream) {
    return warp_correlate_impl(ref_nhwc, src_nhwc, nullptr, rel_proj, depth_sample, view_weights_in, vw_shift, similarity_mlp,
                               pixelwise_mlp, B, N, C, G, D, h, w, hs, ws, cost_out, view_weights_out, vw_argmax_out, similarity_out,
                               stream);
}

extern "C" int pmn_warp_correlate_views(const float* ref_nhwc, const void* src_view_table, const float* rel_proj,
                                        const float* depth_sample, const float* view_weights_in, int vw_shift,
                                        const float* similarity_mlp, const float* pixelwise_mlp, int B, int N, int C, int G,
                                        int D, int h, int w, int hs, int ws, float* cost_out, float* view_weights_out,
                                        int* vw_argmax_out, float* similarity_out, void* stream) {
    if (!src_view_table) return PMN_ERR_ARG;
    return warp_correlate_impl(ref_nhwc, nullptr, static_cast<const unsigned long long*>(src_view_table), rel_proj, depth_sample,
                               view_weights_in, vw_shift, similarity_mlp, pixelwise_mlp, B, N, C, G, D, h, w, hs, ws, cost_out,
                               view_weights_out, vw_argmax_out, similarity_out, stream);
}

extern "C" int pmn_feature_weight(const float* ref_nhwc, const float* eval_offsets, const int* eval_table_host,
                                  const float* mlp, int B, int C, int G, int K, int h, int w, float* out_feature_weight,
                                  void* stream) {
    if (!ref_nhwc || !eval_offsets || !eval_table_host || !mlp || !out_feature_weight) return PMN_ERR_ARG;
    if (B < 1 || h < 2 || w < 2) return PMN_ERR_ARG;
    if (K < 1 || K > PMN_MAX_NEIGHBORS) return PMN_ERR_SHAPE;
    GatherArgs a;
    memset(&a, 0, sizeof(a));
    a.ref = ref_nhwc;
    a.src = ref_nhwc;
    a.offsets = eval_offsets;
    a.mlp_a = mlp;
    a.out = out_feature_weight;
    a.B = B; a.N = 1; a.D = K; a.h = h; a.w = w; a.hs = h; a.ws = w;
    for (int i = 0; i < 2 * K; ++i) a.table[i] = eval_table_host[i];
    return dispatch_gather<MODE_NEIGHBOR>(a, C, G, (hipStream_t)stream);
}
```

### patchmatchnet_amd/csrc/hypotheses.hip

```cpp
#include <cstring>

#include "pmn_common.hpp"
#define PMN_DIV48(u) ((u) / 48.0f)
#define PMN_DIV48R(u) pmn_div_by((u), 48.0f, r48)

struct HypArgs {
    const float* noise;
    const float* depth;
    const float* depth_min;
    const float* depth_max;
    const float* offsets;
    float* depth_sample;
    float* xnorm;
    int depth_shift, num_sample, K, B, h, w;
    float interval_scale;
    int table[2 * PMN_MAX_NEIGHBORS];
};

__device__ __forceinline__ float centre_hypothesis(const HypArgs& a, int b, int qy, int qx, float inv_min, float inv_max,
                                                   float interval, int kc) {
#pragma clang fp contract(off)
    const int h = a.h, w = a.w;
    if (a.noise) {
        const float u = a.noise[((size_t)b * 48 + 24) * h * w + (size_t)qy * w + qx] + 24.0f;
        const float inv = inv_max + PMN_DIV48(u) * (inv_min - inv_max);
        return 1.0f / inv;
    }
    const int ws = w >> a.depth_shift;
    const float dprev = a.depth[(size_t)b * (h >> a.depth_shift) * ws + (size_t)(qy >> a.depth_shift) * ws +
                                (qx >> a.depth_shift)];
    if (a.num_sample == 1) return dprev;
    float inv = 1.0f / dprev + interval * (float)kc;
    inv = fminf(fmaxf(inv, inv_max), inv_min);
    return 1.0f / inv;
}

template <int NP2>
__global__ __launch_bounds__(PMN_BLOCK) void init_hypotheses_kernel(const HypArgs a) {
#pragma clang fp contract(off)
    const int h = a.h, w = a.w, hw = h * w;
    const int p = blockIdx.x * blockDim.x + threadIdx.x;
    const int b = blockIdx.y;
    if (p >= hw) return;
    const int y = p / w, x = p - y * w;
    const float inv_min = 1.0f / a.depth_min[b];
    const float inv_max = 1.0f / a.depth_max[b];
    const int D0 = a.noise ? 48 : a.num_sample;
    const int K = a.K;
    const int D = D0 + K;
    const float interval = (inv_min - inv_max) * a.interval_scale;
    const int k0 = -((a.num_sample + 1) / 2);
    const int kc = k0 + a.num_sample / 2;

    float v[NP2];
#pragma unroll
    for (int j = 0; j < NP2; ++j) v[j] = __builtin_inff();

    if (a.noise) {
#pragma unroll
        for (int j = 0; j < 48; ++j) {
            if (j < NP2) {
                const float u = a.noise[((size_t)b * 48 + j) * hw + p] + (float)j;
                const float inv = inv_max + PMN_DIV48(u) * (inv_min - inv_max);
                v[j] = 1.0f / inv;
            }
        }
    } else {
        const int ws = w >> a.depth_shift;
        const float dprev =
            a.depth[(size_t)b * (h >> a.depth_shift) * ws + (size_t)(y >> a.depth_shift) * ws + (x >> a.depth_shift)];
        if (a.num_sample == 1) {
            v[0] = dprev;
        } else {
            const float inv_prev = 1.0f / dprev;
#pragma unroll
            for (int j = 0; j < NP2; ++j) {
                if (j < a.num_sample) {
                    float inv = inv_prev + interval * (float)(k0 + j);
                    inv = fminf(fmaxf(inv, inv_max), inv_min);
                    v[j] = 1.0f / inv;
                }
            }
        }
    }

    if (K > 0) {
        for (int k = 0; k < K; ++k) {
            const float ox = a.offsets[((size_t)b * 2 * K + 2 * k) * hw + p];
            const float oy = a.offsets[((size_t)b * 2 * K + 2 * k + 1) * hw + p];
            float ix, iy;
            pmn_neighbor_position((float)x, (float)y, a.table[2 * k], a.table[2 * k + 1], ox, oy, h, w, ix, iy);
            const PmnTaps t = pmn_make_taps(ix, iy, h, w);
            const int qy = t.off / w, qx = t.off - qy * w;
            const float c00 = centre_hypothesis(a, b, qy, qx, inv_min, inv_max, interval, kc);
            const float c01 = centre_hypothesis(a, b, qy, qx + 1, inv_min, inv_max, interval, kc);
            const float c10 = centre_hypothesis(a, b, qy + 1, qx, inv_min, inv_max, interval, kc);
            const float c11 = centre_hypothesis(a, b, qy + 1, qx + 1, inv_min, inv_max, interval, kc);
            const float val = fmaf(c11, t.w11, fmaf(c10, t.w10, fmaf(c01, t.w01, c00 * t.w00)));
            const int slot = D0 + k;
#pragma unroll
            for (int j = 0; j < NP2; ++j)
                if (j == slot) v[j] = val;
        }
#pragma unroll
        for (int kk = 2; kk <= NP2; kk <<= 1) {
#pragma unroll
            for (int jj = kk >> 1; jj > 0; jj >>= 1) {
#pragma unroll
                for (int i = 0; i < NP2; ++i) {
                    const int l = i ^ jj;
                    if (l > i) {
                        const float lo = fminf(v[i], v[l]), hi = fmaxf(v[i], v[l]);
                        if ((i & kk) == 0) {
                            v[i] = lo;
                            v[l] = hi;
                        } else {
                            v[i] = hi;
                            v[l] = lo;
                        }
                    }
                }
            }
        }
    }

    const float range = inv_min - inv_max;
#pragma unroll
    for (int j = 0; j < NP2; ++j) {
        if (j < D) {
            const size_t o = ((size_t)b * D + j) * hw + p;
            a.depth_sample[o] = v[j];
            a.xnorm[((size_t)b * hw + p) * D + j] = (1.0f / v[j] - inv_max) / range;
        }
    }
}

template <int NP2, int D0T, int KT>
__global__ __launch_bounds__(PMN_BLOCK) void init_hypotheses_fixed_kernel(const HypArgs a) {
#pragma clang fp contract(off)
    static_assert(D0T + KT <= NP2, "hypotheses fit the sorting network");
    const int h = a.h, w = a.w, hw = h * w;
    const int p = blockIdx.x * blockDim.x + threadIdx.x;
    const int b = blockIdx.y;
    if (p >= hw) return;
    const int y = p / w, x = p - y * w;
    const float inv_min = 1.0f / a.depth_min[b];
    const float inv_max = 1.0f / a.depth_max[b];
    constexpr int D = D0T + KT;
    const float interval = (inv_min - inv_max) * a.interval_scale;
    const int k0 = -((a.num_sample + 1) / 2);
    const int kc = k0 + a.num_sample / 2;
    const bool from_noise = a.noise != nullptr;
    const float r48 = pmn_uniform(pmn_rcp_refined(48.0f));

    float v[NP2];
#pragma unroll
    for (int j = 0; j < NP2; ++j) v[j] = __builtin_inff();

    const int ws = w >> a.depth_shift;
    if (from_noise) {
        float u[D0T];
#pragma unroll
        for (int j = 0; j < D0T; ++j) u[j] = a.noise[((size_t)b * 48 + j) * hw + p];
#pragma unroll
        for (int j = 0; j < D0T; ++j) {
            const float inv = inv_max + PMN_DIV48R(u[j] + (float)j) * (inv_min - inv_max);
            v[j] = pmn_div(1.0f, inv);
        }
    } else {
        const float dprev =
            a.depth[(size_t)b * (h >> a.depth_shift) * ws + (size_t)(y >> a.depth_shift) * ws + (x >> a.depth_shift)];
        if (D0T == 1) {
            v[0] = dprev;
        } else {
            const float inv_prev = pmn_div(1.0f, dprev);
#pragma unroll
            for (int j = 0; j < D0T; ++j) {
                float inv = inv_prev + interval * (float)(k0 + j);
                inv = fminf(fmaxf(inv, inv_max), inv_min);
                v[j] = pmn_div(1.0f, inv);
            }
        }
    }

    if constexpr (KT > 0) {
        constexpr int KB = KT < 8 ? KT : 8;
        static_assert(KT % KB == 0, "whole batches");
        const float* cbase = from_noise ? a.noise + ((size_t)b * 48 + 24) * hw
                                        : a.depth + (size_t)b * (h >> a.depth_shift) * ws;
        const int sh = from_noise ? 0 : a.depth_shift, cw = from_noise ? w : ws;
#pragma unroll
        for (int k0b = 0; k0b < KT; k0b += KB) {
            float ox[KB], oy[KB];
#pragma unroll
            for (int i = 0; i < KB; ++i) {
                ox[i] = a.offsets[((size_t)b * 2 * KT + 2 * (k0b + i)) * hw + p];
                oy[i] = a.offsets[((size_t)b * 2 * KT + 2 * (k0b + i) + 1) * hw + p];
            }
            PmnTaps t[KB];
            float c[KB][4];
#pragma unroll
            for (int i = 0; i < KB; ++i) {
                float ix, iy;
                pmn_neighbor_position((float)x, (float)y, a.table[2 * (k0b + i)], a.table[2 * (k0b + i) + 1], ox[i], oy[i], h, w, ix,
                                      iy);
                t[i] = pmn_make_taps(ix, iy, h, w);
                const int qy = t[i].off / w, qx = t[i].off - qy * w;
                c[i][0] = cbase[(size_t)(qy >> sh) * cw + (qx >> sh)];
                c[i][1] = cbase[(size_t)(qy >> sh) * cw + ((qx + 1) >> sh)];
                c[i][2] = cbase[(size_t)((qy + 1) >> sh) * cw + (qx >> sh)];
                c[i][3] = cbase[(size_t)((qy + 1) >> sh) * cw + ((qx + 1) >> sh)];
            }
#pragma unroll
            for (int i = 0; i < KB; ++i) {
                float cc[4];
#pragma unroll
                for (int q = 0; q < 4; ++q) {
                    if (from_noise) {
                        const float inv = inv_max + PMN_DIV48R(c[i][q] + 24.0f) * (inv_min - inv_max);
                        cc[q] = pmn_div(1.0f, inv);
                    } else if (a.num_sample == 1) {
                        cc[q] = c[i][q];
                    } else {
                        float inv = pmn_div(1.0f, c[i][q]) + interval * (float)kc;
                        inv = fminf(fmaxf(inv, inv_max), inv_min);
                        cc[q] = pmn_div(1.0f, inv);
                    }
                }
                v[D0T + k0b + i] = fmaf(cc[3], t[i].w11, fmaf(cc[2], t[i].w10, fmaf(cc[1], t[i].w01, cc[0] * t[i].w00)));
            }
        }
#pragma unroll
        for (int kk = 2; kk <= NP2; kk <<= 1) {
#pragma unroll
            for (int jj = kk >> 1; jj > 0; jj >>= 1) {
#pragma unroll
                for (int i = 0; i < NP2; ++i) {
                    const int l = i ^ jj;
                    if (l > i) {
                        const float lo = fminf(v[i], v[l]), hi = fmaxf(v[i], v[l]);
                        if ((i & kk) == 0) {
                            v[i] = lo;
                            v[l] = hi;
                        } else {
                            v[i] = hi;
                            v[l] = lo;
                        }
                    }
                }
            }
        }
    }

    const float range = inv_min - inv_max, rrange = pmn_rcp_refined(range);
#pragma unroll
    for (int j = 0; j < D; ++j) {
        const size_t o = ((size_t)b * D + j) * hw + p;
        a.depth_sample[o] = v[j];
        a.xnorm[((size_t)b * hw + p) * D + j] = pmn_div_by(pmn_div(1.0f, v[j]) - inv_max, range, rrange);
    }
}

extern "C" int pmn_init_hypotheses(const float* noise, const float* depth, int depth_shift, const float* depth_min,
                                   const float* depth_max, int num_sample, float interval_scale,
                                   const float* propa_offsets, const int* propa_table_host, int K, int B, int h, int w,
                                   float* depth_sample, float* xnorm, void* stream) {
    if ((!noise && !depth) || !depth_min || !depth_max || !depth_sample || !xnorm) return PMN_ERR_ARG;
    if (B < 1 || h < 2 || w < 2 || K < 0 || depth_shift < 0 || depth_shift > 1) return PMN_ERR_ARG;
    if (K > 0 && (!propa_offsets || !propa_table_host)) return PMN_ERR_ARG;
    if (K > 16) return PMN_ERR_SHAPE;
    if (!noise && num_sample < 1) return PMN_ERR_ARG;
    if (depth_shift && ((h | w) & 1)) return PMN_ERR_ARG;
    const int D0 = noise ? 48 : num_sample;
    const int D = D0 + K;
    if (D > PMN_MAX_DEPTH) return PMN_ERR_SHAPE;
    HypArgs a;
    memset(&a, 0, sizeof(a));
    a.noise = noise;
    a.depth = noise ? nullptr : depth;
    a.depth_min = depth_min;
    a.depth_max = depth_max;
    a.offsets = propa_offsets;
    a.depth_sample = depth_sample;
    a.xnorm = xnorm;
    a.depth_shift = depth_shift;
    a.num_sample = noise ? 48 : num_sample;
    a.K = K;
    a.B = B; a.h = h; a.w = w;
    a.interval_scale = interval_scale;
    for (int i = 0; i < 2 * K; ++i) a.table[i] = propa_table_host[i];
    const int bs = (h * w <= 64 * 1024) ? 64 : PMN_BLOCK;
    const dim3 grid((h * w + bs - 1) / bs, B), block(bs);
    hipStream_t s = (hipStream_t)stream;
    if (noise && K == 16) PMN_LAUNCH((init_hypotheses_fixed_kernel<64, 48, 16>), grid, block, 0, s, a);
    else if (!noise && num_sample == 16 && K == 16) PMN_LAUNCH((init_hypotheses_fixed_kernel<32, 16, 16>), grid, block, 0, s, a);
    else if (!noise && num_sample == 8 && K == 8) PMN_LAUNCH((init_hypotheses_fixed_kernel<16, 8, 8>), grid, block, 0, s, a);
    else if (!noise && num_sample == 8 && K == 0) PMN_LAUNCH((init_hypotheses_fixed_kernel<8, 8, 0>), grid, block, 0, s, a);
    else if (D <= 8) PMN_LAUNCH(init_hypotheses_kernel<8>, grid, block, 0, s, a);
    else if (D <= 16) PMN_LAUNCH(init_hypotheses_kernel<16>, grid, block, 0, s, a);
    else if (D <= 32) PMN_LAUNCH(init_hypotheses_kernel<32>, grid, block, 0, s, a);
    else PMN_LAUNCH(init_hypotheses_kernel<64>, grid, block, 0, s, a);
    PMN_CHECK_LAUNCH();
    return PMN_OK;
}
```

### patchmatchnet_amd/net.py

```python
from __future__ import annotations

from typing import Dict, List, Optional, Tuple

import warnings

import numpy as np
import torch
import torch.nn as nn
import torch.nn.functional as F

from . import _lib, ops, params
from ._lib import PmnError
from .module import ConvBnReLU
from .patchmatch import PatchMatch


class FeatureNet(nn.Module):

    def __init__(self) -> None:
        super().__init__()
        spec = [(3, 8, 3, 1, 1), (8, 8, 3, 1, 1), (8, 16, 5, 2, 2), (16, 16, 3, 1, 1), (16, 16, 3, 1, 1),
                (16, 32, 5, 2, 2), (32, 32, 3, 1, 1), (32, 32, 3, 1, 1), (32, 64, 5, 2, 2), (64, 64, 3, 1, 1),
                (64, 64, 3, 1, 1)]
        for i, (cin, cout, k, s, p) in enumerate(spec):
# ... 66 lines not shown
        B, _, H, W = imgs[0].shape
        in_place = image_table is not None
        if in_place and not (self.f16_split and "conv1_f16s" in pk):
            raise PmnError("image_table: only the fp16-split stem (FeatureNet.f16_split, weights inside its domain) reads images in place")
        if in_place:
            t = ops.stem_f16s_views(image_table, *pk["conv0"], *pk["conv1_f16s"])
        else:
            t = torch.empty((B * len(imgs), H, W, 8), dtype=torch.float32, device=imgs[0].device)
        for i, im in enumerate(() if in_place else imgs):
            if self.f16_split and "conv1_f16s" in pk:
                ops.stem_f16s(im.contiguous(), *pk["conv0"], *pk["conv1_f16s"], out=t[i * B:(i + 1) * B])
            else:
                ops.stem(im.contiguous(), *pk["conv0"], *pk["conv1"], out=t[i * B:(i + 1) * B])
        feats = {}
        for i, (k, s, p) in enumerate(self._SPEC):
            if i < 2:
                continue
            if i == 4 and self.f16_split and self.fuse_conv34 and "conv3_f16s" in pk and "conv4_f16s" in pk:
                continue
            if i == 3 and self.f16_split and self.fuse_conv34 and "conv3_f16s" in pk and "conv4_f16s" in pk:
                t = ops.conv2d_f16s_pair(t, *pk["conv3_f16s"], *pk["conv4_f16s"], relu=True)
                feats[4] = t
            elif self.f16_split and f"conv{i}_f16s" in pk:
                t = ops.conv2d_f16s(t, *pk[f"conv{i}_f16s"], k, s, relu=True)
            elif self.layer_hook is not None and (hooked := self.layer_hook(i, t)) is not None:
                t = hooked
            else:
                w, sh = pk[f"conv{i}"]
                t = ops.conv2d(t, w, sh, getattr(self, f"conv{i}").conv.out_channels, k, s, p, relu=True)
            if i in (4, 7, 10):
                feats[i] = t
        half, quarter, eighth = feats[4], feats[7], feats[10]
        if self.fold_fpn:
            if self.fpn8_valu:
                f3, u8 = ops.fpn_level(eighth, None, *pk["fpn8"], ca=64)
            else:
                f3, u8 = ops.pointwise_split_mfma(eighth, *pk["fpn8_mfma"], cout=112, ca=64)
            if pending is not None:
                pending.update(half=half, quarter=quarter, u8=u8)
                return {3: f3}
            return {3: f3, **self.finish_hip(dict(half=half, quarter=quarter, u8=u8))}
        out = {3: ops.conv2d(eighth, *pk["output1"], 64, 1)}
        top = ops.conv2d(quarter, *pk["inner1"], 64, 1, up=eighth)
        out[2] = ops.conv2d(top, *pk["output2"], 32, 1)
        out[1] = ops.fpn_tail(half, top, pk["inner2"][0], pk["inner2"][1], pk["output3"][0])
        return out

    def finish_hip(self, pending: dict) -> Dict[int, torch.Tensor]:
        pk = self._packed()
        f2, u4 = ops.fpn_level(pending["quarter"], pending["u8"], *pk["fpn4"], ca=32)
        f1, _ = ops.fpn_level(pending["half"], u4, *pk["fpn2"], ca=16)
        return {2: f2, 1: f1}

    def forward(self, x: torch.Tensor) -> Dict[int, torch.Tensor]:
        half = self.conv4(self.conv3(self.conv2(self.conv1(self.conv0(x)))))
        quarter = self.conv7(self.conv6(self.conv5(half)))
        eighth = self.conv10(self.conv9(self.conv8(quarter)))
        out: Dict[int, torch.Tensor] = {3: self.output1(eighth)}
        top = F.interpolate(eighth, scale_factor=2.0, mode="bilinear", align_corners=False) + self.inner1(quarter)
        out[2] = self.output2(top)
        top = F.interpolate(top, scale_factor=2.0, mode="bilinear", align_corners=False) + self.inner2(half)
        out[1] = self.output3(top)
        return out


class Refinement(nn.Module):

    def __init__(self) -> None:
        super().__init__()
        self.conv0 = ConvBnReLU(in_channels=3, out_channels=8)
        self.conv1 = ConvBnReLU(in_channels=1, out_channels=8)
        self.conv2 = ConvBnReLU(in_channels=8, out_channels=8)
        self.deconv = nn.ConvTranspose2d(8, 8, kernel_size=3, padding=1, output_padding=1, stride=2, bias=False)
        self.bn = nn.BatchNorm2d(8)
        self.conv3 = ConvBnReLU(in_channels=16, out_channels=8)
        self.res = nn.Conv2d(8, 1, kernel_size=3, padding=1, bias=False)
        self.f16_split = True
        self.f16_domain_error: Optional[str] = None
        self.research = dict(layers=False)

    def _packed(self):
        srcs = [p for p in self.parameters()] + [b for b in self.buffers() if b.dtype.is_floating_point]
        key = params.versions(srcs)
        if getattr(self, "_pack_key", None) != key:
            dev = self.res.weight.device

            def bn_of(m):
                return (m.weight, m.bias, m.running_mean, m.running_var)

            pk = {}
            for name in ("conv0", "conv1", "conv2", "conv3"):
                m = getattr(self, name)
                w, s = params.pack_conv(m.conv.weight, bn=bn_of(m.bn), eps=m.bn.eps)
                pk[name] = (torch.from_numpy(w).to(dev), torch.from_numpy(s).to(dev))
            w, s = params.pack_deconv(self.deconv.weight, bn=bn_of(self.bn), eps=self.bn.eps)
            pk["deconv"] = (torch.from_numpy(w).to(dev), torch.from_numpy(s).to(dev))
            w, s = params.pack_conv(self.res.weight)
            pk["res"] = (torch.from_numpy(w).to(dev), torch.from_numpy(s).to(dev))
            pk["tail"] = tuple(torch.from_numpy(a).to(dev) for a in params.pack_refine_tail(
                self.conv3.conv.weight, bn_of(self.conv3.bn), self.res.weight, eps=self.conv3.bn.eps))
            self.f16_domain_error = None
            try:
                w, s = params.pack_refine_conv3_f16s(self.conv3.conv.weight, bn_of(self.conv3.bn), eps=self.conv3.bn.eps)
                pk["conv3_f16s"] = (torch.from_numpy(w).to(dev), torch.from_numpy(s).to(dev))
            except params.F16DomainError as e:
                self.f16_domain_error = f"conv3: {e}"
                warnings.warn("Refinement: " + self.f16_domain_error + " -- using the fp32 kernels (pmn_refine_front / pmn_refine_tail)",
                              RuntimeWarning, stacklevel=2)
            self._pack, self._pack_key = pk, key
        return self._pack

    def forward_hip(self, img: torch.Tensor, depth_0: torch.Tensor, depth_min: torch.Tensor, depth_max: torch.Tensor
                    ) -> torch.Tensor:
        pk = self._packed()
        b = depth_min.size()[0]
        if not self.research["layers"]:
            d = ops.normalize_depth(depth_0, depth_min, depth_max)
        else:
            lo = depth_min.view(b, 1, 1, 1)
            span = (depth_max - depth_min).view(b, 1, 1, 1)
            d = ((depth_0 - lo) / span).contiguous()
        t = ops.conv2d(d, *pk["conv1"], 8, 3, 1, 1, relu=True, in_nchw=True)
        t = ops.conv2d(t, *pk["conv2"], 8, 3, 1, 1, relu=True)
        if not self.research["layers"]:
            if self.f16_split and "conv3_f16s" in pk:
                return ops.refine_fused(img.contiguous(), t, *pk["conv0"], *pk["deconv"], *pk["conv3_f16s"], pk["tail"][2], d,
                                        depth_min.float().contiguous(), depth_max.float().contiguous())
            x16 = ops.refine_front(img.contiguous(), t, *pk["conv0"], *pk["deconv"])
            return ops.refine_tail(x16, *pk["tail"], d, depth_min.float().contiguous(), depth_max.float().contiguous())
        img_feat = ops.conv2d(img.contiguous(), *pk["conv0"], 8, 3, 1, 1, relu=True, in_nchw=True)
        up = ops.deconv3x3s2(t, *pk["deconv"], relu=True)
        t = ops.conv2d(torch.cat((up, img_feat), dim=3), *pk["conv3"], 8, 3, 1, 1, relu=True)
        res = ops.conv2d(t, *pk["res"], 1, 3, 1, 1, out_nchw=True)
        d = F.interpolate(d, scale_factor=2.0, mode="nearest") + res
        return d * span + lo

    def forward(self, img: torch.Tensor, depth_0: torch.Tensor, depth_min: torch.Tensor, depth_max: torch.Tensor
                ) -> torch.Tensor:
        b = depth_min.size()[0]
        lo = depth_min.view(b, 1, 1, 1)
        span = (depth_max - depth_min).view(b, 1, 1, 1)
        d = (depth_0 - lo) / span
        img_feat = self.conv0(img)
        up = F.relu(self.bn(self.deconv(self.conv2(self.conv1(d)))), inplace=True)
        res = self.res(self.conv3(torch.cat((up, img_feat), dim=1)))
        d = F.interpolate(d, scale_factor=2.0, mode="nearest") + res
        return d * span + lo


class PatchmatchNet(nn.Module):

    def __init__(self, patchmatch_interval_scale: List[float], propagation_range: List[int],
                 patchmatch_iteration: List[int], patchmatch_num_sample: List[int], propagate_neighbors: List[int],
                 evaluate_neighbors: List[int]) -> None:
        super().__init__()
        self.stages = 4
        self.feature = FeatureNet()
        self.patchmatch_num_sample = patchmatch_num_sample
        num_features = [16, 32, 64]
        self.propagate_neighbors = propagate_neighbors
        self.evaluate_neighbors = evaluate_neighbors
        self.G = [4, 8, 8]
        for i in range(self.stages - 1):
            setattr(self, f"patchmatch_{i + 1}", PatchMatch(
                propagation_out_range=propagation_range[i], patchmatch_iteration=patchmatch_iteration[i],
                patchmatch_num_sample=patchmatch_num_sample[i], patchmatch_interval_scale=patchmatch_interval_scale[i],
                num_feature=num_features[i], G=self.G[i], propagate_neighbors=self.propagate_neighbors[i],
                evaluate_neighbors=evaluate_neighbors[i], stage=i + 1))
        self.upsample_net = Refinement()
        self.batch_feature_extraction = True
        self.hip_feature_net = True
        self.hip_projections = True

    def load_state_dict(self, state_dict, strict: bool = True, **kw):
        if any(k.startswith("module.") for k in state_dict):
            state_dict = {(k[len("module."):] if k.startswith("module.") else k): v for k, v in state_dict.items()}
        return super().load_state_dict(state_dict, strict=strict, **kw)

    @staticmethod
    def scripted_module_config(archive) -> Dict[str, list]:
        stages = [getattr(archive, f"patchmatch_{i}") for i in (1, 2, 3)]
        return dict(patchmatch_interval_scale=[float(s.patchmatch_interval_scale) for s in stages],
                    propagation_range=[int(s.dilation) for s in stages],
                    patchmatch_iteration=[int(s.patchmatch_iteration) for s in stages],
                    patchmatch_num_sample=[int(x) for x in archive.patchmatch_num_sample],
                    propagate_neighbors=[int(s.propagate_neighbors) for s in stages],
                    evaluate_neighbors=[int(s.evaluate_neighbors) for s in stages])

    @classmethod
    def from_scripted_module(cls, path: str) -> "PatchmatchNet":
        archive = torch.jit.load(path, map_location="cpu")
        model = cls(**cls.scripted_module_config(archive))
        model.load_state_dict({k: v.detach().clone() for k, v in archive.state_dict().items()}, strict=True)
        return model

    def extract_features(self, images: List[torch.Tensor], stacked: Optional[dict] = None,
                         image_table: Optional["ops.SourceTable"] = None, pending: Optional[dict] = None
                         ) -> List[Dict[int, torch.Tensor]]:
        same = all(im.shape == images[0].shape for im in images)
        B = images[0].shape[0]
        if image_table is not None and not (self.hip_feature_net and same and images[0].is_cuda and self.feature.f16_split):
            raise PmnError("image_table needs the HIP FeatureNet (f16_split) and same-size images on a ROCm device")
        if self.hip_feature_net and same and images[0].is_cuda:
            f = self.feature.forward_hip(images, image_table=image_table, pending=pending)
            if stacked is not None:
                stacked.update({("nhwc", s): t for s, t in f.items()})
            return [{s: t[i * B:(i + 1) * B].permute(0, 3, 1, 2) for s, t in f.items()} for i in range(len(images))]
        if self.hip_feature_net and images[0].is_cuda:
            outs = [self.feature.forward_hip(im) for im in images]
            return [{s: t.permute(0, 3, 1, 2) for s, t in f.items()} for f in outs]
        if self.batch_feature_extraction and same and len(images) > 1:
            f = self.feature(torch.cat(images, dim=0))
            if stacked is not None:
                stacked.update(f)
            return [{s: t[i * B:(i + 1) * B] for s, t in f.items()} for i in range(len(images))]
        return [self.feature(im) for im in images]

    def finish_features(self, features: List[Dict[int, torch.Tensor]], stacked: dict, pending: dict) -> None:
        f = self.feature.finish_hip(pending)
        B = f[2].shape[0] // len(features)
        stacked.update({("nhwc", s): t for s, t in f.items()})
        for i, view in enumerate(features):
            view.update({s: t[i * B:(i + 1) * B].permute(0, 3, 1, 2) for s, t in f.items()})

    def forward(self, images: List[torch.Tensor], intrinsics: torch.Tensor, extrinsics: torch.Tensor,
                depth_min: torch.Tensor, depth_max: torch.Tensor, noise: Optional[torch.Tensor] = None,
                features: Optional[List[Dict[int, torch.Tensor]]] = None, debug: Optional[dict] = None,
                features_nhwc: Optional[Dict[int, torch.Tensor]] = None, source_tables: Optional[Dict[int, "ops.SourceTable"]] = None,
                ref_nhwc_maps: Optional[Dict[int, torch.Tensor]] = None, image_table: Optional["ops.SourceTable"] = None
                ) -> Tuple[torch.Tensor, torch.Tensor, Dict[int, List[torch.Tensor]]]:
        assert len(images) == intrinsics.size()[1], "Different number of images and intrinsic matrices"
        assert len(images) == extrinsics.size()[1], "Different number of images and extrinsic matrices"
        if self.training:
            raise PmnError("patchmatchnet_amd.PatchmatchNet is inference-only: call .eval() (the HIP kernels have no "
                           "backward pass)")
        images, intrinsics, orig_height, orig_width = adjust_image_dims(images, intrinsics)
        ref_image = images[0]
        _, _, ref_height, ref_width = ref_image.size()

        stacked: Dict[int, torch.Tensor] = {}
        pending: dict = {}
        if features is None:
            features = self.extract_features(images, stacked, image_table, pending)
        elif features_nhwc is not None:
            stacked.update({("nhwc", st): t for st, t in features_nhwc.items()})
        ref_feature, src_features = features[0], features[1:]
        batch = ref_image.shape[0]

        depth_min = depth_min.float()
        depth_max = depth_max.float()
        device = intrinsics.device
        depth = torch.empty(0, device=device)
        score = torch.empty(0, device=device)
        view_weights = torch.empty(0, device=device)
        depth_patchmatch: Dict[int, List[torch.Tensor]] = {}

        scale = 0.125
        depth_shift, vw_shift = 0, 0
        rel_all = ops.stage_projections(intrinsics, extrinsics, self.stages - 1, scale) if self.hip_projections else None


        def stage_maps(stage):
            if source_tables is not None:
                return ref_nhwc_maps[stage], source_tables[stage]
            if ("nhwc", stage) in stacked:
                allv = stacked[("nhwc", stage)]
            elif stage in stacked:
                allv = stacked[("nhwc", stage)] = ops.nchw_to_nhwc(stacked[stage].contiguous())
            else:
                return None, None
            return allv[:batch], allv[batch:].view(len(features) - 1, batch, *allv.shape[1:])

        precomputed: Dict[int, dict] = {}
        ops.plan_fork()
        ops.plan_switch(1)
        if pending:
            self.finish_features(features, stacked, pending)
        for stage in range(self.stages - 2, 0, -1):
            precomputed[stage] = getattr(self, f"patchmatch_{stage}").prepare(features[0][stage], stage_maps(stage)[0])
        ops.plan_switch(0)
        for stage in range(self.stages - 1, 0, -1):
            if stage == self.stages - 2:
                ops.plan_join()
                pending.clear()
            if rel_all is None:
                intrinsics_l = intrinsics.clone()
                intrinsics_l[:, :, :2] *= scale
                proj = extrinsics.clone()
                proj[:, :, :3, :4] = torch.matmul(intrinsics_l, extrinsics[:, :, :3, :4])
                proj_l = torch.unbind(proj, 1)
                ref_proj, src_proj = proj_l[0], proj_l[1:]
            else:
                ref_proj, src_proj = extrinsics[:, 0], [extrinsics[:, i] for i in range(1, extrinsics.shape[1])]
            scale *= 2.0

            dbg = [] if debug is not None else None
            pm: PatchMatch = getattr(self, f"patchmatch_{stage}")
            ref_nhwc, src_nhwc = stage_maps(stage)
            depths, score, view_weights = pm(
                ref_feature=ref_feature[stage], src_features=[f[stage] for f in src_features], ref_proj=ref_proj,
                src_projs=list(src_proj), depth_min=depth_min, depth_max=depth_max, depth=depth,
                view_weights=view_weights, depth_shift=depth_shift, vw_shift=vw_shift,
                noise=noise if stage == self.stages - 1 else None, debug=dbg, ref_nhwc=ref_nhwc, src_nhwc=src_nhwc,
                rel_proj=None if rel_all is None else rel_all[self.stages - 1 - stage], precomputed=precomputed.get(stage))
            if debug is not None:
                debug[stage] = dbg
            depth_patchmatch[stage] = depths
            depth = depths[-1].detach()
            if stage > 1:
                depth_shift = 1
                vw_shift = vw_shift + 1 if view_weights.shape[-1] != depths[-1].shape[-1] else 1

        if self.hip_feature_net and ref_image.is_cuda:
            depth = self.upsample_net.forward_hip(ref_image, depth, depth_min, depth_max)
        else:
            depth = self.upsample_net(ref_image, depth, depth_min, depth_max)
        if ref_width != orig_width or ref_height != orig_height:
            depth = F.interpolate(depth, size=[orig_height, orig_width], mode="bilinear", align_corners=False)
        depth_patchmatch[0] = [depth]

        confidence, _ = ops.confidence(score.contiguous(), orig_height, orig_width)
        return depth, confidence, depth_patchmatch


def adjust_image_dims(images: List[torch.Tensor], intrinsics: torch.Tensor
                      ) -> Tuple[List[torch.Tensor], torch.Tensor, int, int]:
    _, _, ref_height, ref_width = images[0].size()
    for i in range(len(images)):
        _, _, height, width = images[i].size()
        new_height = int(round(height / 8)) * 8
        new_width = int(round(width / 8)) * 8
        if new_width != width or new_height != height:
            intrinsics[:, i, 0] *= new_width / width
            intrinsics[:, i, 1] *= new_height / height
            images[i] = F.interpolate(images[i], size=[new_height, new_width], mode="bilinear", align_corners=False)
    return images, intrinsics, ref_height, ref_width
```

### patchmatchnet_amd/ops.py

```python
from __future__ import annotations

import ctypes
import threading
from typing import List, Optional, Sequence, Tuple

import numpy as np
import torch

from . import _lib
from ._lib import PmnError, check


_TIMING = None
_TIMING_ON = True


def enable_kernel_timing() -> None:
    global _TIMING, _TIMING_ON
    _TIMING, _TIMING_ON = [], True


def pause_kernel_timing(paused: bool) -> None:
    global _TIMING_ON
    _TIMING_ON = not paused


def disable_kernel_timing():
    global _TIMING
    rec, _TIMING = _TIMING, None
    if not rec:
        return []
    torch.cuda.synchronize()
    return [(s.elapsed_time(e), nbytes, tag) for s, e, nbytes, tag in rec]


TUNE_WINDOW_BYTES, TUNE_FLAGS, TUNE_WINDOW_BYTES_PIXELWISE, TUNE_ABLATE = 0, 1, 2, 3
TUNE_LANE_WINDOW_BYTES, TUNE_LANE_ABLATE, TUNE_LANE_WAVES_PER_SIMD = 4, 5, 6
TUNE_TILE_WINDOW_BYTES = 10
FLAG_WINDOWED, FLAG_NO_ROTATION, FLAG_STREAM_PIXELWISE, FLAG_STREAM_VIEWS, FLAG_WIN_V1, FLAG_TILE, FLAG_MFMA = 1, 2, 4, 8, 16, 32, 64
DEFAULT_FLAGS = 0


def set_tuning(key: int, value: int) -> None:
    if not _lib.experimental():
        raise PmnError("pmn_set_tuning exists only in libpmn_hip_experimental.so: build with `make -C patchmatchnet_amd/csrc "
                       "EXPERIMENTAL=1` and run with PMN_EXPERIMENTAL=1")
    check(_lib.lib().pmn_set_tuning(int(key), int(value)), "pmn_set_tuning")


import os as _os

F16_DOMAIN_CHECK = _os.environ.get("PMN_CHECK_F16_DOMAIN", "") == "1"
_F16_FLAGS = {}


def _f16_domain_probe(*tensors: Optional[torch.Tensor]) -> None:
    if not F16_DOMAIN_CHECK:
        return
    for t in tensors:
        if t is None or not t.is_cuda or t.numel() == 0:
            continue
        flag = _F16_FLAGS.get(t.device)
        if flag is None:
            flag = _F16_FLAGS[t.device] = torch.zeros(1, dtype=torch.int32, device=t.device)
        with torch.cuda.device(t.device):
            check(_lib.lib().pmn_check_f16_domain(t.data_ptr(), t.numel(), flag.data_ptr(), _stream(t)), "pmn_check_f16_domain")


def f16_domain_check(reset: bool = True) -> None:
    bad = [str(d) for d, f in _F16_FLAGS.items() if int(f.item()) != 0]
    if reset:
        for f in _F16_FLAGS.values():
            f.zero_()
    if bad:
        raise PmnError("an activation outside the fp16-split kernels' domain (|x| >= 65504 or not finite) reached pmn_*_f16s on " +
                       ", ".join(bad) + ": the outputs contain inf / NaN where an fp32 convolution is finite -- set f16_split = False on "
                       "FeatureNet / Refinement / PatchMatch for this checkpoint or input range (include/pmn_hip.h)")


def _dev(t: torch.Tensor, name: str) -> torch.Tensor:
    if not isinstance(t, torch.Tensor):
        raise PmnError(f"{name}: expected a torch.Tensor")
    if not t.is_cuda:
        raise PmnError(f"{name}: tensor is on {t.device}; patchmatchnet_amd runs only on a ROCm GPU (no CPU fallback)")
    if t.dtype != torch.float32:
        raise PmnError(f"{name}: expected float32, got {t.dtype}")
    if not t.is_contiguous():
        raise PmnError(f"{name}: tensor must be contiguous")
    return t


def _dlast(t: torch.Tensor, name: str) -> torch.Tensor:
    if not isinstance(t, torch.Tensor) or not t.is_cuda or t.dtype != torch.float32:
        raise PmnError(f"{name}: expected a float32 tensor on a ROCm GPU (no CPU fallback)")
    if t.permute(0, 2, 3, 1).is_contiguous():
        return t
    return t.permute(0, 2, 3, 1).contiguous().permute(0, 3, 1, 2)


def _dev_as(t: torch.Tensor, name: str, dtype: torch.dtype) -> torch.Tensor:
    if not isinstance(t, torch.Tensor) or not t.is_cuda:
        raise PmnError(f"{name}: expected a tensor on a ROCm GPU (no CPU fallback)")
    if t.dtype != dtype or not t.is_contiguous():
        raise PmnError(f"{name}: expected a contiguous {dtype} tensor")
    return t


def _ptr(t: Optional[torch.Tensor]) -> Optional[int]:
    return None if t is None else t.data_ptr()


def _stream(t: torch.Tensor) -> int:
    return torch.cuda.current_stream(t.device).cuda_stream


_RECORDING = threading.local()


class PlanRegion:

    def __init__(self, plan) -> None:
        self.plan, self.open, self.branch, self.forked = plan, False, 0, False
        self.held: List[torch.Tensor] = []
        self.reads = {0: [], 1: []}
        self.writes = {0: [], 1: []}
        self.allocated = {0: [], 1: []}
        self.held_bytes = 0


def begin_plan_recording(plan) -> PlanRegion:
    _RECORDING.region = PlanRegion(plan)
    return _RECORDING.region


def end_plan_recording() -> None:
    _RECORDING.region = None


def _region() -> Optional[PlanRegion]:
    return getattr(_RECORDING, "region", None)


def plan_fork() -> None:
    r = _region()
    if r is not None:
        check(_lib.lib().pmn_plan_fork(r.plan), "pmn_plan_fork")
        r.open, r.branch, r.forked = True, 0, True


def plan_switch(branch: int) -> None:
    r = _region()
    if r is not None:
        check(_lib.lib().pmn_plan_switch(r.plan, int(branch)), "pmn_plan_switch")
        r.branch = int(branch)


def plan_join() -> None:
    r = _region()
    if r is not None:
        for b in (0, 1):
            for rng in r.allocated[b]:
                if not any(_ranges_overlap(rng, w) for w in r.writes[b]):
                    raise PmnError("plan_join: a tensor allocated between fork and join is not among the outputs its branch's calls "
                                   "declared (ops._note): the overlap check would not see it")
        check_branch_overlap(r.reads[0], r.writes[0], r.reads[1], r.writes[1])
        check(_lib.lib().pmn_plan_join(r.plan), "pmn_plan_join")
        r.open, r.branch = False, 0
        r.held.clear()


def _range(t: torch.Tensor) -> Tuple[int, int]:
    return (t.data_ptr(), t.numel() * t.element_size())


def _ranges_overlap(a: Tuple[int, int], b: Tuple[int, int]) -> bool:
    return a[1] > 0 and b[1] > 0 and a[0] < b[0] + b[1] and b[0] < a[0] + a[1]


def check_branch_overlap(main_reads, main_writes, side_reads, side_writes) -> None:
    for who, writes, others in (("main", main_writes, list(side_reads) + list(side_writes)),
                                ("side", side_writes, list(main_reads) + list(main_writes))):
        for w in writes:
            for o in others:
                if _ranges_overlap(w, o):
                    raise PmnError(f"plan fork: the {who} branch writes [{w[0]:#x}, +{w[1]}) which the other branch touches at "
                                   f"[{o[0]:#x}, +{o[1]}): the branches run concurrently on replay and must not share a buffer")


def _hold(t, fresh: bool) -> None:
    r = _region()
    if r is not None and r.open and isinstance(t, torch.Tensor) and t.is_cuda:
        r.held.append(t)
        if fresh and t.numel():
            r.allocated[r.branch].append(_range(t))
            r.held_bytes += t.numel() * t.element_size()


def _note(reads, writes) -> None:
    r = _region()
    if r is not None and r.open:
        r.reads[r.branch] += [_range(t) for t in reads if t is not None]
        r.writes[r.branch] += [_range(t) for t in writes if t is not None]


def _host_f32(a: np.ndarray, n: int, name: str):
    a = np.ascontiguousarray(a, np.float32)
    if a.size != n:
        raise PmnError(f"{name}: expected {n} floats, got {a.size}")
    return a, a.ctypes.data_as(ctypes.c_void_p)


def _host_i32(a: np.ndarray, n: int, name: str):
    a = np.ascontiguousarray(a, np.int32)
    if a.size != n:
        raise PmnError(f"{name}: expected {n} ints, got {a.size}")
    return a, a.ctypes.data_as(ctypes.c_void_p)


def nchw_to_nhwc(x: torch.Tensor, out: Optional[torch.Tensor] = None) -> torch.Tensor:
    if out is None and isinstance(x, torch.Tensor) and x.is_cuda and x.dtype == torch.float32 and not x.is_contiguous():
        v = x.permute(0, 2, 3, 1)
        if v.is_contiguous():
            return v
        x = x.contiguous()
    _dev(x, "x")
    B, C, h, w = x.shape
    if out is None:
        out = torch.empty((B, h, w, C), dtype=torch.float32, device=x.device)
    else:
        _dev(out, "out")
        if tuple(out.shape) != (B, h, w, C):
            raise PmnError("nchw_to_nhwc: bad output shape")
    _note((x,), (out,))
    with torch.cuda.device(x.device):
        check(_lib.lib().pmn_nchw_to_nhwc(x.data_ptr(), out.data_ptr(), B, C, h, w, _stream(x)), "pmn_nchw_to_nhwc")
    return out


def stack_sources_nhwc(src_features: Sequence[torch.Tensor]) -> torch.Tensor:
    buf, sizes = stack_sources_padded(src_features)
    if any(sz != sizes[0] for sz in sizes):
        raise PmnError("all source feature maps of one stage must share a shape (stack_sources_padded handles mixed sizes)")
    return buf


def stack_sources_padded(src_features: Sequence[torch.Tensor]):
    if len(src_features) == 0:
        raise PmnError("at least one source view is required")
    B, C = src_features[0].shape[:2]
    sizes = [(int(f.shape[2]), int(f.shape[3])) for f in src_features]
    if any(tuple(f.shape[:2]) != (B, C) for f in src_features):
        raise PmnError("source feature maps of one stage must share batch size and channels")
    hs, ws = max(h for h, _ in sizes), max(w for _, w in sizes)
    mixed = any(sz != (hs, ws) for sz in sizes)
    alloc = torch.zeros if mixed else torch.empty
    buf = alloc((len(src_features), B, hs, ws, C), dtype=torch.float32, device=src_features[0].device)
    for i, f in enumerate(src_features):
        v = f.permute(0, 2, 3, 1)
        if sizes[i] != (hs, ws):
            _dev(f.contiguous(), "src_feature")
            buf[i][:, :sizes[i][0], :sizes[i][1], :].copy_(v)
        elif f.is_cuda and f.dtype == torch.float32 and v.is_contiguous():
            buf[i].copy_(v)
        else:
            nchw_to_nhwc(f.contiguous(), buf[i])
    return buf, sizes


def rescale_projection_rows(rel_proj: torch.Tensor, sizes, padded_hw) -> torch.Tensor:
    HS, WS = padded_hw
    if all(sz == (HS, WS) for sz in sizes):
        return rel_proj
    out = rel_proj.clone()
    for v, (h_v, w_v) in enumerate(sizes):
        if (h_v, w_v) != (HS, WS):
            out[:, v, 0, :] *= (w_v - 1) / (WS - 1)
            out[:, v, 1, :] *= (h_v - 1) / (HS - 1)
    return out.contiguous()


def _mlp_dev(t: torch.Tensor, name: str) -> torch.Tensor:
    _dev(t, name)
    if t.numel() != _lib.MLP_FLOATS:
        raise PmnError(f"{name}: expected a packed MLP block of {_lib.MLP_FLOATS} floats")
    return t


def feature_weight(ref_nhwc: torch.Tensor, eval_offsets: torch.Tensor, table: np.ndarray, mlp: torch.Tensor,
                   G: int) -> torch.Tensor:
    _dev(ref_nhwc, "ref_nhwc")
    _dev(eval_offsets, "eval_offsets")
    B, h, w, C = ref_nhwc.shape
    K = eval_offsets.shape[1] // 2
    if tuple(eval_offsets.shape) != (B, 2 * K, h, w):
        raise PmnError("feature_weight: eval_offsets must be [B,2K,h,w]")
    tab, tab_p = _host_i32(table, 2 * K, "table")
    _mlp_dev(mlp, "mlp")
    out = torch.empty((B, K, h, w), dtype=torch.float32, device=ref_nhwc.device)
    _note((ref_nhwc, eval_offsets, mlp), (out,))
    with torch.cuda.device(ref_nhwc.device):
        check(_lib.lib().pmn_feature_weight(ref_nhwc.data_ptr(), eval_offsets.data_ptr(), tab_p, mlp.data_ptr(), B, C, G,
                                            K, h, w,
                                            out.data_ptr(), _stream(out)), "pmn_feature_weight")
    return out


def init_hypotheses(noise: Optional[torch.Tensor], depth: Optional[torch.Tensor], depth_shift: int,
                    depth_min: torch.Tensor, depth_max: torch.Tensor, num_sample: int, interval_scale: float,
                    propa_offsets: Optional[torch.Tensor], table: Optional[np.ndarray], h: int, w: int
                    ) -> Tuple[torch.Tensor, torch.Tensor]:
    _dev(depth_min, "depth_min")
    _dev(depth_max, "depth_max")
    B = depth_min.shape[0]
    dev = depth_min.device
    if noise is not None:
        _dev(noise, "noise")
        if tuple(noise.shape) != (B, 48, h, w):
            raise PmnError("init_hypotheses: noise must be [B,48,h,w]")
        D0 = 48
    else:
        if depth is None:
            raise PmnError("init_hypotheses: need noise or depth")
        _dev(depth, "depth")
        if tuple(depth.shape) != (B, 1, h >> depth_shift, w >> depth_shift):
            raise PmnError(f"init_hypotheses: depth must be [B,1,{h >> depth_shift},{w >> depth_shift}], "
                           f"got {tuple(depth.shape)}")
        D0 = num_sample
    K = 0
    tab_p = None
    tab = None
    if propa_offsets is not None:
        _dev(propa_offsets, "propa_offsets")
        K = propa_offsets.shape[1] // 2
        if tuple(propa_offsets.shape) != (B, 2 * K, h, w):
            raise PmnError("init_hypotheses: propa_offsets must be [B,2K,h,w]")
        tab, tab_p = _host_i32(table, 2 * K, "table")
    D = D0 + K
    ds = torch.empty((B, D, h, w), dtype=torch.float32, device=dev)
    xn = torch.empty((B, h, w, D), dtype=torch.float32, device=dev).permute(0, 3, 1, 2)
    _note((noise, depth if noise is None else None, depth_min, depth_max, propa_offsets), (ds, xn))
    with torch.cuda.device(dev):
        check(_lib.lib().pmn_init_hypotheses(_ptr(noise), _ptr(depth) if noise is None else None, depth_shift,
                                             depth_min.data_ptr(), depth_max.data_ptr(), num_sample,
                                             float(interval_scale), _ptr(propa_offsets), tab_p, K, B, h, w,
                                             ds.data_ptr(), xn.data_ptr(), _stream(ds)), "pmn_init_hypotheses")
    del tab
    return ds, xn


class SourceTable:

    def __init__(self, table: torch.Tensor, shape) -> None:
        if table.dtype != torch.int64 or not table.is_cuda or table.numel() != int(shape[0]):
            raise PmnError("SourceTable: int64 device tensor with one address per source view")
        self.table, self.shape, self.device = table, tuple(int(x) for x in shape), table.device

    @staticmethod
    def image_in_place(im: torch.Tensor) -> bool:
        return bool(im.is_cuda and im.dtype == torch.float32 and im.is_contiguous() and im.data_ptr() % 16 == 0)

    @staticmethod
    def addresses(maps) -> list:
        out = []
        for m in maps:
            if not (m.is_cuda and m.dtype == torch.float32 and m.is_contiguous()):
                raise PmnError("SourceTable: dense float32 channels-last device maps")
            out.append(m.data_ptr())
        return out


def warp_correlate(ref_nhwc: torch.Tensor, src_nhwc, rel_proj: torch.Tensor, depth_sample: torch.Tensor,
                   view_weights: Optional[torch.Tensor], vw_shift: int, similarity_mlp: torch.Tensor,
                   pixelwise_mlp: Optional[torch.Tensor], G: int, want_similarity: bool = False,
                   want_argmax: bool = False):
    _dev(ref_nhwc, "ref_nhwc")
    table = src_nhwc if isinstance(src_nhwc, SourceTable) else None
    if table is None:
        _dev(src_nhwc, "src_nhwc")
    _dev(rel_proj, "rel_proj")
    _dev(depth_sample, "depth_sample")
    B, h, w, C = ref_nhwc.shape
    N, Bs, hs, ws, Cs = src_nhwc.shape
    D = depth_sample.shape[1]
    if Bs != B or Cs != C or tuple(depth_sample.shape) != (B, D, h, w) or tuple(rel_proj.shape) != (B, N, 4, 4):
        raise PmnError("warp_correlate: inconsistent shapes")
    dev = ref_nhwc.device
    sim_p = _mlp_dev(similarity_mlp, "similarity_mlp").data_ptr()
    pix_p, vw_out, argmax = None, None, None
    if view_weights is not None:
        _dev(view_weights, "view_weights")
        if tuple(view_weights.shape) != (B, N, h >> vw_shift, w >> vw_shift):
            raise PmnError("Patchmatch Evaluation: Different number of images and view weights")
    else:
        if pixelwise_mlp is None:
            raise PmnError("warp_correlate: pixelwise_mlp required when view_weights is None")
        pix_p = _mlp_dev(pixelwise_mlp, "pixelwise_mlp").data_ptr()
        vw_out = torch.empty((B, N, h, w), dtype=torch.float32, device=dev)
        if want_argmax:
            argmax = torch.empty((B, N, h, w), dtype=torch.int32, device=dev)
    cost = torch.empty((B, h, w, D), dtype=torch.float32, device=dev).permute(0, 3, 1, 2)
    sim = torch.empty((B, G, D, h, w), dtype=torch.float32, device=dev) if want_similarity else None
    _note((ref_nhwc, src_nhwc if table is None else table.table, rel_proj, depth_sample, view_weights, similarity_mlp, pixelwise_mlp),
          (cost, vw_out, argmax, sim))
    with torch.cuda.device(dev):
        if _TIMING is not None and _TIMING_ON:
            ev0, ev1 = torch.cuda.Event(enable_timing=True), torch.cuda.Event(enable_timing=True)
            ev0.record()
        fn = _lib.lib().pmn_warp_correlate if table is None else _lib.lib().pmn_warp_correlate_views
        check(fn(ref_nhwc.data_ptr(), (src_nhwc if table is None else table.table).data_ptr(), rel_proj.data_ptr(),
                 depth_sample.data_ptr(), _ptr(view_weights), vw_shift, sim_p, pix_p, B, N, C,
                 G, D, h, w, hs, ws, cost.data_ptr(), _ptr(vw_out), _ptr(argmax), _ptr(sim),
                 _stream(cost)), "pmn_warp_correlate")
        if _TIMING is not None and _TIMING_ON:
            ev1.record()
            _TIMING.append((ev0, ev1, 4 * B * h * w * ((1 + N) * C + D + N + G * D),
                            f"C{C}_D{D}_{h}x{w}_N{N}_{'vw' if view_weights is not None else 'pixelwise'}"))
    return cost, (view_weights if view_weights is not None else vw_out), argmax, sim


def aggregate_regress(cost: torch.Tensor, depth_sample: torch.Tensor, xnorm: torch.Tensor, feature_weight_: torch.Tensor,
                      eval_offsets: torch.Tensor, table: np.ndarray, interval_scale: float, is_inverse: bool
                      ) -> Tuple[torch.Tensor, torch.Tensor]:
    for n, t in (("depth_sample", depth_sample), ("feature_weight", feature_weight_), ("eval_offsets", eval_offsets)):
        _dev(t, n)
    cost, xnorm = _dlast(cost, "cost"), _dlast(xnorm, "xnorm")
    B, D, h, w = cost.shape
    K = feature_weight_.shape[1]
    if tuple(depth_sample.shape) != (B, D, h, w) or tuple(xnorm.shape) != (B, D, h, w) or \
            tuple(feature_weight_.shape) != (B, K, h, w) or tuple(eval_offsets.shape) != (B, 2 * K, h, w):
        raise PmnError("aggregate_regress: inconsistent shapes")
    tab, tab_p = _host_i32(table, 2 * K, "table")
    score = torch.empty((B, D, h, w), dtype=torch.float32, device=cost.device)
    depth = torch.empty((B, h, w), dtype=torch.float32, device=cost.device)
    _note((cost, depth_sample, xnorm, feature_weight_, eval_offsets), (score, depth))
    with torch.cuda.device(cost.device):
        check(_lib.lib().pmn_aggregate_regress(cost.data_ptr(), depth_sample.data_ptr(), xnorm.data_ptr(),
                                               feature_weight_.data_ptr(), eval_offsets.data_ptr(), tab_p, K,
                                               float(interval_scale), 1 if is_inverse else 0, B, D, h, w,
                                               score.data_ptr(), depth.data_ptr(), _stream(cost)),
              "pmn_aggregate_regress")
    return score, depth


def confidence(score: torch.Tensor, H: int, W: int, want_index: bool = False):
    _dev(score, "score")
    B, D, h, w = score.shape
    conf = torch.empty((B, H, W), dtype=torch.float32, device=score.device)
    idx = torch.empty((B, h, w), dtype=torch.int32, device=score.device) if want_index else None
    with torch.cuda.device(score.device):
        check(_lib.lib().pmn_confidence(score.data_ptr(), B, D, h, w, H, W, conf.data_ptr(), _ptr(idx), _stream(score)),
              "pmn_confidence")
    return conf, idx


def relative_projection(src_projs: Sequence[torch.Tensor], ref_proj: torch.Tensor) -> torch.Tensor:
    inv = torch.inverse(ref_proj)
    return torch.matmul(torch.stack(list(src_projs), dim=1), inv.unsqueeze(1)).contiguous()


def differentiable_warping(src_fea: torch.Tensor, src_proj: torch.Tensor, ref_proj: torch.Tensor,
                           depth_samples: torch.Tensor) -> torch.Tensor:
    src_fea = _dev(src_fea.contiguous(), "src_fea")
    depth_samples = _dev(depth_samples.contiguous(), "depth_samples")
    B, C, hs, ws = src_fea.shape
    _, D, h, w = depth_samples.shape
    proj = torch.matmul(src_proj, torch.inverse(ref_proj)).contiguous()
    _dev(proj, "proj")
    out = torch.empty((B, C, D, h, w), dtype=torch.float32, device=src_fea.device)
    with torch.cuda.device(src_fea.device):
        check(_lib.lib().pmn_differentiable_warping(src_fea.data_ptr(), proj.data_ptr(), depth_samples.data_ptr(), B, C,
                                                    D, h, w, hs, ws, out.data_ptr(), _stream(out)),
              "pmn_differentiable_warping")
    return out


def stage_projections(intrinsics: torch.Tensor, extrinsics: torch.Tensor, nstages: int = 3, scale0: float = 0.125
                      ) -> torch.Tensor:
    intrinsics = _dev(intrinsics.float().contiguous(), "intrinsics")
    extrinsics = _dev(extrinsics.float().contiguous(), "extrinsics")
    B, V = intrinsics.shape[:2]
    rel = torch.empty((nstages, B, V - 1, 4, 4), dtype=torch.float32, device=intrinsics.device)
    with torch.cuda.device(rel.device):
        check(_lib.lib().pmn_stage_projections(intrinsics.data_ptr(), extrinsics.data_ptr(), B, V, nstages, float(scale0),
                                               rel.data_ptr(), _stream(rel)), "pmn_stage_projections")
    return rel


def normalize_depth(depth: torch.Tensor, depth_min: torch.Tensor, depth_max: torch.Tensor) -> torch.Tensor:
    depth = _dev(depth.contiguous(), "depth")
    lo, hi = _dev(depth_min.float().contiguous(), "depth_min"), _dev(depth_max.float().contiguous(), "depth_max")
    B = depth.shape[0]
    if lo.numel() != B or hi.numel() != B:
        raise PmnError("normalize_depth: depth_min / depth_max must hold one value per batch element")
    out = torch.empty_like(depth)
    with torch.cuda.device(depth.device):
        check(_lib.lib().pmn_normalize_depth(depth.data_ptr(), lo.data_ptr(), hi.data_ptr(), B, depth.numel() // B, out.data_ptr(),
                                             _stream(out)), "pmn_normalize_depth")
    return out


def conv2d(x: torch.Tensor, weights: torch.Tensor, shift: torch.Tensor, cout: int, K: int, stride: int = 1, pad: int = 0,
           dil: int = 1, relu: bool = False, up: Optional[torch.Tensor] = None, in_nchw: bool = False,
           out_nchw: bool = False, out: Optional[torch.Tensor] = None) -> torch.Tensor:
    _dev(x, "x")
    _dev(weights, "weights")
    _dev(shift, "shift")
    if in_nchw:
        N, cin, H, W = x.shape
    else:
        N, H, W, cin = x.shape
    if tuple(weights.shape[:3]) != (K, K, cin) or shift.numel() != weights.shape[3]:
        raise PmnError("conv2d: packed weights do not match the input")
    Ho = (H + 2 * pad - dil * (K - 1) - 1) // stride + 1
    Wo = (W + 2 * pad - dil * (K - 1) - 1) // stride + 1
    shape = (N, cout, Ho, Wo) if out_nchw else (N, Ho, Wo, cout)
    if out is None:
        out = torch.empty(shape, dtype=torch.float32, device=x.device)
    else:
        _dev(out, "out")
        if tuple(out.shape) != shape:
            raise PmnError("conv2d: bad `out` shape")
    up_h = up_w = 0
    if up is not None:
        _dev(up, "up")
        if tuple(up.shape) != (N, Ho // 2, Wo // 2, cout) or Ho % 2 or Wo % 2:
            raise PmnError("conv2d: `up` must be [N,Ho/2,Wo/2,cout]")
        up_h, up_w = up.shape[1], up.shape[2]
    _note((x, weights, shift, up), (out,))
    with torch.cuda.device(x.device):
        check(_lib.lib().pmn_conv2d(x.data_ptr(), weights.data_ptr(), shift.data_ptr(), _ptr(up), out.data_ptr(), N, H, W,
                                    cin, cout, K, stride, pad, dil, 1 if relu else 0, 1 if in_nchw else 0,
                                    1 if out_nchw else 0, up_h, up_w, _stream(x)), "pmn_conv2d")
    return out


def fpn_tail(x: torch.Tensor, up: torch.Tensor, w_in: torch.Tensor, b_in: torch.Tensor, w_out: torch.Tensor) -> torch.Tensor:
    for n_, t_ in (("x", x), ("up", up), ("w_in", w_in), ("b_in", b_in), ("w_out", w_out)):
        _dev(t_, n_)
    N, H, W, cin = x.shape
    cmid, cout = up.shape[3], w_out.shape[3]
    if tuple(up.shape) != (N, H // 2, W // 2, cmid) or tuple(w_in.shape) != (1, 1, cin, cmid) or \
            tuple(w_out.shape) != (1, 1, cmid, cout):
        raise PmnError("fpn_tail: inconsistent shapes")
    out = torch.empty((N, H, W, cout), dtype=torch.float32, device=x.device)
    with torch.cuda.device(x.device):
        check(_lib.lib().pmn_fpn_tail(x.data_ptr(), up.data_ptr(), w_in.data_ptr(), b_in.data_ptr(), w_out.data_ptr(),
                                      out.data_ptr(), N, H, W, cin, cmid, cout, _stream(x)), "pmn_fpn_tail")
    return out


MFMA_CONV_SHAPES = {(64, 64, 3, 1), (32, 32, 3, 1), (32, 64, 5, 2), (16, 32, 5, 2)}
MFMA_HEAD_SHAPES = {(64, 2), (32, 4), (16, 6)}


def conv2d_mfma(x: torch.Tensor, weights: torch.Tensor, shift: torch.Tensor, K: int, stride: int = 1, pad: int = 0,
                relu: bool = True) -> torch.Tensor:
    for n_, t_ in (("x", x), ("weights", weights), ("shift", shift)):
        _dev(t_, n_)
    N, H, W, cin = x.shape
    cout = shift.shape[0]
    if tuple(weights.shape) != (K * K, cin // 8, cout // 32, 64, 4):
        raise PmnError("conv2d_mfma: weights are not in pack_conv_mfma layout for this input")
    Ho, Wo = (H + 2 * pad - K) // stride + 1, (W + 2 * pad - K) // stride + 1
    out = torch.empty((N, Ho, Wo, cout), dtype=torch.float32, device=x.device)
    with torch.cuda.device(x.device):
        check(_lib.lib().pmn_conv2d_mfma(x.data_ptr(), weights.data_ptr(), shift.data_ptr(), out.data_ptr(), None, N, H, W,
                                         cin, cout, cout, K, stride, pad, 1, 1 if relu else 0, 0, _stream(x)),
              "pmn_conv2d_mfma")
    return out


def conv3x3_wino(x: torch.Tensor, weights: torch.Tensor, shift: torch.Tensor, relu: bool = True) -> torch.Tensor:
    if not _lib.experimental():
        raise PmnError("conv3x3_wino: research build only (make -C patchmatchnet_amd/csrc EXPERIMENTAL=1, PMN_EXPERIMENTAL=1)")
    for n_, t_ in (("x", x), ("weights", weights), ("shift", shift)):
        _dev(t_, n_)
    N, H, W, C = x.shape
    if tuple(weights.shape) != (C // 16, 16, C // 16, 64, 4) or tuple(shift.shape) != (C,):
        raise PmnError("conv3x3_wino: weights are not in pack_conv_wino layout for this input")
    out = torch.empty((N, H, W, C), dtype=torch.float32, device=x.device)
    with torch.cuda.device(x.device):
        check(_lib.lib().pmn_conv3x3_wino(x.data_ptr(), weights.data_ptr(), shift.data_ptr(), out.data_ptr(), N, H, W, C,
                                          1 if relu else 0, _stream(x)), "pmn_conv3x3_wino")
    return out


def conv5x5s2_wino(x: torch.Tensor, weights: torch.Tensor, shift: torch.Tensor, relu: bool = True) -> torch.Tensor:
    if not _lib.experimental():
        raise PmnError("conv5x5s2_wino: research build only (make -C patchmatchnet_amd/csrc EXPERIMENTAL=1, PMN_EXPERIMENTAL=1)")
    for n_, t_ in (("x", x), ("weights", weights), ("shift", shift)):
        _dev(t_, n_)
    N, H, W, cin = x.shape
    cout = shift.shape[0]
    if tuple(weights.shape) != (cin // 8, 49, cout // 16, 64, 2):
        raise PmnError("conv5x5s2_wino: weights are not in pack_conv5x5s2_wino layout for this input")
    out = torch.empty((N, (H - 1) // 2 + 1, (W - 1) // 2 + 1, cout), dtype=torch.float32, device=x.device)
    with torch.cuda.device(x.device):
        check(_lib.lib().pmn_conv5x5s2_wino(x.data_ptr(), weights.data_ptr(), shift.data_ptr(), out.data_ptr(), N, H, W, cin,
                                            cout, 1 if relu else 0, _stream(x)), "pmn_conv5x5s2_wino")
    return out


F16S_SHAPES = {(3, 1, 16, 16), (3, 1, 32, 32), (3, 1, 64, 64), (5, 2, 8, 16), (5, 2, 16, 32), (5, 2, 32, 64)}


def conv2d_f16s(x: torch.Tensor, weights: torch.Tensor, shift: torch.Tensor, k: int, stride: int, relu: bool = True) -> torch.Tensor:
    _dev(x, "x")
    _f16_domain_probe(x)
    _dev(shift, "shift")
    _dev_as(weights, "conv2d_f16s: weights (params.pack_conv_f16s)", torch.float16)
    N, H, W, cin = x.shape
    cout = shift.shape[0]
    if (k, stride, cin, cout) not in F16S_SHAPES:
        raise PmnError(f"conv2d_f16s: unsupported layer (k={k}, stride={stride}, cin={cin}, cout={cout})")
    from . import params as _params
    cc = _params.f16s_chunk(cin, k)
    if tuple(weights.shape) != (cin // cc, (k * k * (cc // 8) + 3) // 4, cout // 16, 2, 64, 8):
        raise PmnError("conv2d_f16s: weights are not in pack_conv_f16s layout for this input")
    out = torch.empty((N, (H - 1) // stride + 1, (W - 1) // stride + 1, cout), dtype=torch.float32, device=x.device)
    with torch.cuda.device(x.device):
        check(_lib.lib().pmn_conv2d_f16s(x.data_ptr(), weights.data_ptr(), shift.data_ptr(), out.data_ptr(), N, H, W, cin, cout, k,
                                         stride, 1 if relu else 0, _stream(x)), "pmn_conv2d_f16s")
    return out


def conv2d_f16s_pair(x: torch.Tensor, weights_a: torch.Tensor, shift_a: torch.Tensor, weights_b: torch.Tensor, shift_b: torch.Tensor,
                     relu: bool = True) -> torch.Tensor:
    _dev(x, "x")
    _f16_domain_probe(x)
    N, H, W, C = x.shape
    for w_, s_ in ((weights_a, shift_a), (weights_b, shift_b)):
        _dev(s_, "shift")
        _dev_as(w_, "conv2d_f16s_pair: weights", torch.float16)
        if tuple(w_.shape) != (1, 5, 1, 2, 64, 8) or s_.numel() != 16:
            raise PmnError("conv2d_f16s_pair: weights must be params.pack_conv_f16s of a (3, 1, 16, 16) layer")
    if C != 16:
        raise PmnError("conv2d_f16s_pair: 16-channel layers only")
    out = torch.empty((N, H, W, 16), dtype=torch.float32, device=x.device)
    with torch.cuda.device(x.device):
        check(_lib.lib().pmn_conv2d_f16s_pair(x.data_ptr(), weights_a.data_ptr(), shift_a.data_ptr(), weights_b.data_ptr(), shift_b.data_ptr(),
                                              out.data_ptr(), N, H, W, 16, 1 if relu else 0, _stream(x)), "pmn_conv2d_f16s_pair")
    return out


def pointwise_split_mfma(x: torch.Tensor, weights: torch.Tensor, shift: torch.Tensor, cout: int, ca: int):
    for n_, t_ in (("x", x), ("weights", weights), ("shift", shift)):
        _dev(t_, n_)
    N, H, W, cin = x.shape
    coutp = shift.shape[0]
    if tuple(weights.shape) != (1, cin // 8, coutp // 32, 64, 4) or not 0 < ca < cout <= coutp:
        raise PmnError("pointwise_split_mfma: weights are not in pack_conv_mfma layout for this input")
    out_a = torch.empty((N, H, W, ca), dtype=torch.float32, device=x.device)
    out_b = torch.empty((N, H, W, cout - ca), dtype=torch.float32, device=x.device)
    with torch.cuda.device(x.device):
        check(_lib.lib().pmn_conv2d_mfma(x.data_ptr(), weights.data_ptr(), shift.data_ptr(), out_a.data_ptr(), out_b.data_ptr(),
                                         N, H, W, cin, cout, ca, 1, 1, 0, 1, 0, 0, _stream(x)), "pmn_conv2d_mfma")
    return out_a, out_b


def offset_heads_mfma(x: torch.Tensor, weights: torch.Tensor, shift: torch.Tensor, cout: int, ca: int, dil: int):
    for n_, t_ in (("x", x), ("weights", weights), ("shift", shift)):
        _dev(t_, n_)
    N, H, W, cin = x.shape
    coutp = shift.shape[0]
    if tuple(weights.shape) != (9, cin // 8, coutp // 32, 64, 4) or not 0 < ca <= cout <= coutp:
        raise PmnError("offset_heads_mfma: weights are not in pack_conv_mfma layout for this input")
    out_a = torch.empty((N, ca, H, W), dtype=torch.float32, device=x.device)
    out_b = torch.empty((N, cout - ca, H, W), dtype=torch.float32, device=x.device) if ca < cout else None
    with torch.cuda.device(x.device):
        check(_lib.lib().pmn_conv2d_mfma(x.data_ptr(), weights.data_ptr(), shift.data_ptr(), out_a.data_ptr(), _ptr(out_b), N,
                                         H, W, cin, cout, ca, 3, 1, dil, dil, 0, 1, _stream(x)), "pmn_conv2d_mfma")
    return out_a, out_b


F16S_HEAD_SHAPES = {(64, 2), (32, 4), (16, 6)}


def offset_heads_f16s(x: torch.Tensor, weights: torch.Tensor, shift: torch.Tensor, cout: int, ca: int, dil: int):
    _dev(x, "x")
    _f16_domain_probe(x)
    _dev(shift, "shift")
    N, H, W, cin = x.shape
    coutp = shift.shape[0]
    _dev_as(weights, "offset_heads_f16s: weights", torch.float16)
    if tuple(weights.shape) != (cin // 16, (9 * 2 + 3) // 4, coutp // 16, 2, 64, 8) or not 0 < ca <= cout <= coutp \
            or coutp != (cout + 15) // 16 * 16:
        raise PmnError("offset_heads_f16s: weights are not in pack_offset_heads_f16s layout for this input")
    out_a = torch.empty((N, ca, H, W), dtype=torch.float32, device=x.device)
    out_b = torch.empty((N, cout - ca, H, W), dtype=torch.float32, device=x.device) if ca < cout else None
    _note((x, weights, shift), (out_a, out_b))
    with torch.cuda.device(x.device):
        check(_lib.lib().pmn_offset_heads_f16s(x.data_ptr(), weights.data_ptr(), shift.data_ptr(), out_a.data_ptr(), _ptr(out_b), N,
                                               H, W, cin, cout, ca, dil, _stream(x)), "pmn_offset_heads_f16s")
    return out_a, out_b


def fpn_level(x: torch.Tensor, u: Optional[torch.Tensor], w: torch.Tensor, b: torch.Tensor, ca: int):
    for n_, t_ in (("x", x), ("w", w), ("b", b)):
        _dev(t_, n_)
    N, H, W, cin = x.shape
    cout = w.shape[1]
    if tuple(w.shape) != (cin, cout) or tuple(b.shape) != (cout,) or not 0 < ca <= cout:
        raise PmnError("fpn_level: inconsistent shapes")
    if u is not None:
        _dev(u, "u")
        if tuple(u.shape) != (N, H // 2, W // 2, cout) or H % 2 or W % 2:
            raise PmnError("fpn_level: `u` must be [N,H/2,W/2,cout]")
    out_a = torch.empty((N, H, W, ca), dtype=torch.float32, device=x.device)
    out_b = torch.empty((N, H, W, cout - ca), dtype=torch.float32, device=x.device) if ca < cout else None
    _note((x, u, w, b), (out_a, out_b))
    with torch.cuda.device(x.device):
        check(_lib.lib().pmn_fpn_level(x.data_ptr(), _ptr(u), w.data_ptr(), b.data_ptr(), out_a.data_ptr(), _ptr(out_b),
                                       N, H, W, cin, cout, ca, _stream(x)), "pmn_fpn_level")
    return out_a, out_b


def refine_front(img: torch.Tensor, t2: torch.Tensor, w0: torch.Tensor, s0: torch.Tensor, wd: torch.Tensor,
                 sd: torch.Tensor) -> torch.Tensor:
    for n_, t_ in (("img", img), ("t2", t2), ("w0", w0), ("s0", s0), ("wd", wd), ("sd", sd)):
        _dev(t_, n_)
    B, c, H, W = img.shape
    if c != 3 or H % 2 or W % 2 or tuple(t2.shape) != (B, H // 2, W // 2, 8) or tuple(w0.shape) != (3, 3, 3, 8) or \
            tuple(wd.shape) != (3, 3, 8, 8):
        raise PmnError("refine_front: inconsistent shapes")
    out = torch.empty((B, H, W, 16), dtype=torch.float32, device=img.device)
    with torch.cuda.device(img.device):
        check(_lib.lib().pmn_refine_front(img.data_ptr(), t2.data_ptr(), w0.data_ptr(), s0.data_ptr(), wd.data_ptr(),
                                          sd.data_ptr(), out.data_ptr(), B, H, W, _stream(img)), "pmn_refine_front")
    return out


def refine_tail(x16: torch.Tensor, w3: torch.Tensor, s3: torch.Tensor, wr: torch.Tensor, dnorm: torch.Tensor,
                depth_min: torch.Tensor, depth_max: torch.Tensor) -> torch.Tensor:
    for n_, t_ in (("x16", x16), ("w3", w3), ("s3", s3), ("wr", wr), ("dnorm", dnorm), ("depth_min", depth_min),
                   ("depth_max", depth_max)):
        _dev(t_, n_)
    B, H, W, c = x16.shape
    if c != 16 or H % 2 or W % 2 or tuple(dnorm.shape) != (B, 1, H // 2, W // 2) or tuple(w3.shape) != (2, 3, 3, 16, 4) or \
            tuple(wr.shape) != (3, 3, 8) or depth_min.numel() != B or depth_max.numel() != B:
        raise PmnError("refine_tail: inconsistent shapes")
    out = torch.empty((B, 1, H, W), dtype=torch.float32, device=x16.device)
    with torch.cuda.device(x16.device):
        check(_lib.lib().pmn_refine_tail(x16.data_ptr(), w3.data_ptr(), s3.data_ptr(), wr.data_ptr(), dnorm.data_ptr(),
# ... 776 lines not shown
```

### patchmatchnet_amd/patchmatch.py

```python
from __future__ import annotations

from typing import List, Optional, Tuple

import numpy as np
import torch
import torch.nn as nn

import warnings

from . import _lib, ops, params
from ._lib import PmnError
from .module import ConvBnReLU3D, is_empty


class _PointwiseMLP(nn.Module):

    _last = "similarity"

    def __init__(self, G: int) -> None:
        super().__init__()
        self.G = G
        self.conv0 = ConvBnReLU3D(in_channels=G, out_channels=16, kernel_size=1, stride=1, pad=0)
        self.conv1 = ConvBnReLU3D(in_channels=16, out_channels=8, kernel_size=1, stride=1, pad=0)
        self._packed: Optional[np.ndarray] = None
        self._packed_key = None
        self._packed_dev: Optional[torch.Tensor] = None

    def _sources(self) -> List[torch.Tensor]:
        last = getattr(self, self._last)
        return [self.conv0.conv.weight, *self.conv0.bn_tensors(), self.conv1.conv.weight, *self.conv1.bn_tensors(),
                last.weight, last.bias]

    def packed(self) -> np.ndarray:
        key = params.versions(self._sources())
        if self._packed is None or key != self._packed_key:
            last = getattr(self, self._last)
            self._packed = params.pack_mlp(self.conv0.conv.weight, self.conv0.bn_tensors(), self.conv1.conv.weight,
                                           self.conv1.bn_tensors(), last.weight, last.bias)
            self._packed_key = key
            self._packed_dev = None
        return self._packed

    def packed_device(self) -> torch.Tensor:
        blk = self.packed()
        dev = self.conv0.conv.weight.device
        if self._packed_dev is None or self._packed_dev.device != dev:
            self._packed_dev = torch.from_numpy(blk).to(dev)
        return self._packed_dev


class PixelwiseNet(_PointwiseMLP):

    _last = "conv2"

    def __init__(self, G: int) -> None:
        super().__init__(G)
        self.conv2 = nn.Conv3d(in_channels=8, out_channels=1, kernel_size=1, stride=1, padding=0)
        self.output = nn.Sigmoid()


class SimilarityNet(_PointwiseMLP):

    def __init__(self, G: int) -> None:
        super().__init__(G)
        self.similarity = nn.Conv3d(in_channels=8, out_channels=1, kernel_size=1, stride=1, padding=0)


class FeatureWeightNet(_PointwiseMLP):

    def __init__(self, neighbors: int = 9, G: int = 8) -> None:
        super().__init__(G)
        self.neighbors = neighbors
        self.similarity = nn.Conv3d(in_channels=8, out_channels=1, kernel_size=1, stride=1, padding=0)
        self.output = nn.Sigmoid()

    def forward(self, ref_nhwc: torch.Tensor, eval_offsets: torch.Tensor, table: np.ndarray) -> torch.Tensor:
        return ops.feature_weight(ref_nhwc, eval_offsets, table, self.packed_device(), self.G)


class DepthInitialization(nn.Module):

    def __init__(self, patchmatch_num_sample: int = 1) -> None:
        super().__init__()
        self.patchmatch_num_sample = patchmatch_num_sample

    def forward(self, min_depth: torch.Tensor, max_depth: torch.Tensor, height: int, width: int,
                depth_interval_scale: float, device: torch.device, depth: torch.Tensor) -> torch.Tensor:
        noise = None
        if is_empty(depth):
            noise = torch.rand(size=(min_depth.size()[0], 48, height, width), device=device)
        ds, _ = ops.init_hypotheses(noise, None if noise is not None else depth.detach().contiguous(), 0,
                                    min_depth.float().contiguous(), max_depth.float().contiguous(),
                                    self.patchmatch_num_sample, depth_interval_scale, None, None, height, width)
        return ds


class Propagation(nn.Module):

    def __init__(self) -> None:
        super().__init__()


class Evaluation(nn.Module):

    def __init__(self, G: int = 8) -> None:
        super().__init__()
        self.G = G
        self.pixel_wise_net = PixelwiseNet(self.G)
        self.softmax = nn.LogSoftmax(dim=1)
        self.similarity_net = SimilarityNet(self.G)

    def forward(self, ref_feature: torch.Tensor, src_features: List[torch.Tensor], ref_proj: torch.Tensor,
                src_projs: List[torch.Tensor], depth_sample: torch.Tensor, grid: Optional[torch.Tensor],
                weight: Optional[torch.Tensor], view_weights: torch.Tensor, is_inverse: bool, *,
                fused: Optional[dict] = None, debug: Optional[dict] = None) -> Tuple[torch.Tensor, torch.Tensor, torch.Tensor]:
        N = len(src_features) if src_features is not None else fused["src_nhwc"].shape[0]
        if src_features is not None and src_projs is not None and len(src_features) != len(src_projs):
            raise AssertionError("Patchmatch Evaluation: Different number of images and projection matrices")
        have_vw = not is_empty(view_weights)
        if have_vw and view_weights.size()[1] != N:
            raise AssertionError("Patchmatch Evaluation: Different number of images and view weights")
        f = fused or {}
        ref_nhwc = f.get("ref_nhwc")
        src_nhwc = f.get("src_nhwc")
        rel_proj = f.get("rel_proj")
        if ref_nhwc is None:
            ref_nhwc = ops.nchw_to_nhwc(ref_feature.detach())
        if rel_proj is None:
            rel_proj = ops.relative_projection(src_projs, ref_proj)
        if src_nhwc is None:
            src_nhwc, sizes = ops.stack_sources_padded([s.detach() for s in src_features])
            rel_proj = ops.rescale_projection_rows(rel_proj, sizes, tuple(src_nhwc.shape[2:4]))
        depth_sample = depth_sample.contiguous()
        cost, vw, argmax, sim = ops.warp_correlate(
            ref_nhwc, src_nhwc, rel_proj.contiguous(), depth_sample, view_weights.contiguous() if have_vw else None,
            int(f.get("vw_shift", 0)), self.similarity_net.packed_device(),
            None if have_vw else self.pixel_wise_net.packed_device(), self.G,
            want_similarity=debug is not None, want_argmax=debug is not None and not have_vw)
        if fused is not None and grid is None:
            score, depth = ops.aggregate_regress(cost, depth_sample, f["xnorm"], f["feature_weight"], f["eval_offsets"],
                                                 f["table"], f["interval_scale"], is_inverse)
        else:
            if grid is None or weight is None:
                raise PmnError("Evaluation.forward needs grid and weight (reference signature) or the fused-form arguments")
            B, D, h, w = depth_sample.shape
            K = grid.shape[1] // h
            sampled = torch.nn.functional.grid_sample(cost.contiguous(), grid, mode="bilinear", padding_mode="border",
                                                      align_corners=False).view(B, D, K, h, w)
            score = torch.sum(sampled * weight, dim=2)
            score = torch.exp(self.softmax(score))
            if is_inverse:
                index = torch.arange(0, D, 1, device=score.device).view(1, D, 1, 1)
                index = torch.sum(index * score, dim=1)
                inv_min = 1.0 / depth_sample[:, -1, :, :]
                inv_max = 1.0 / depth_sample[:, 0, :, :]
                depth = 1.0 / (inv_max + index / (D - 1) * (inv_min - inv_max))
            else:
                depth = torch.sum(depth_sample * score, dim=1)
        if debug is not None:
            debug.update(cost=cost, similarity=sim, view_weight_argmax=argmax)
        return depth, score, vw.detach()


class PatchMatch(nn.Module):

    def __init__(self, propagation_out_range: int = 2, patchmatch_iteration: int = 2, patchmatch_num_sample: int = 16,
                 patchmatch_interval_scale: float = 0.025, num_feature: int = 64, G: int = 8,
                 propagate_neighbors: int = 16, evaluate_neighbors: int = 9, stage: int = 3) -> None:
        super().__init__()
        self.patchmatch_iteration = patchmatch_iteration
        self.patchmatch_interval_scale = patchmatch_interval_scale
        self.propa_num_feature = num_feature
        self.G = G
        self.stage = stage
        self.dilation = propagation_out_range
        self.propagate_neighbors = propagate_neighbors
        self.evaluate_neighbors = evaluate_neighbors
        if propagate_neighbors not in (0, 4, 8, 16) or evaluate_neighbors not in (9, 17):
            raise NotImplementedError

        self.depth_initialization = DepthInitialization(patchmatch_num_sample)
        self.propagation = Propagation()
        self.evaluation = Evaluation(self.G)
        self.propa_conv = nn.Conv2d(num_feature, max(2 * propagate_neighbors, 1), kernel_size=3, stride=1,
                                    padding=self.dilation, dilation=self.dilation, bias=True)
        nn.init.constant_(self.propa_conv.weight, 0.0)
        nn.init.constant_(self.propa_conv.bias, 0.0)
        self.eval_conv = nn.Conv2d(num_feature, 2 * evaluate_neighbors, kernel_size=3, stride=1, padding=self.dilation,
                                   dilation=self.dilation, bias=True)
        nn.init.constant_(self.eval_conv.weight, 0.0)
        nn.init.constant_(self.eval_conv.bias, 0.0)
        self.feature_weight_net = FeatureWeightNet(evaluate_neighbors, self.G)

        self.hip_offset_heads = True
        self.f16_split = True
        self.f16_domain_error: Optional[str] = None
        self.heads_hook = None
        self._heads = None
        self._heads_key = None
        self._ptable = params.propagation_table(propagate_neighbors, self.dilation) if propagate_neighbors > 0 else None
        self._etable = params.evaluation_table(evaluate_neighbors, self.dilation)

    def _packed_heads(self):
        srcs = [self.propa_conv.weight, self.propa_conv.bias, self.eval_conv.weight, self.eval_conv.bias]
        key = params.versions(srcs)
        if self._heads is None or key != self._heads_key:
            dev = self.eval_conv.weight.device
            pk = {}
            for name, m in (("propa", self.propa_conv), ("eval", self.eval_conv)):
                w, s = params.pack_conv(m.weight, bias=m.bias)
                pk[name] = (torch.from_numpy(w).to(dev), torch.from_numpy(s).to(dev))
            self.f16_domain_error = None
            for name, mods in (("both", (self.propa_conv, self.eval_conv)), ("eval_only", (self.eval_conv,))):
                wcat = torch.cat([m.weight.detach() for m in mods], 0)
                bcat = torch.cat([m.bias.detach() for m in mods], 0)
                rows = wcat.shape[0]
                if (self.eval_conv.in_channels, self.dilation) in ops.F16S_HEAD_SHAPES and (rows + 15) // 16 * 16 in (32, 48, 64):
                    try:
                        w, s = params.pack_offset_heads_f16s(wcat, bcat)
                        pk["f16s_" + name] = (torch.from_numpy(w).to(dev), torch.from_numpy(s).to(dev))
                    except params.F16DomainError as e:
                        self.f16_domain_error = f"offset heads: {e}"
            if self.f16_domain_error is not None:
                warnings.warn(f"PatchMatch stage {self.stage}: " + self.f16_domain_error + " -- using pmn_conv2d (fp32)", RuntimeWarning,
                              stacklevel=2)
            self._heads, self._heads_key = pk, key
        return self._heads

    def prepare(self, ref_feature: torch.Tensor, ref_nhwc: Optional[torch.Tensor] = None) -> dict:
        if not ref_feature.is_cuda:
            raise PmnError("patchmatchnet_amd.PatchMatch runs on a ROCm GPU only (no CPU fallback)")
        propagate_any = self.propagate_neighbors > 0 and not (self.stage == 1 and self.patchmatch_iteration == 1)
        if ref_nhwc is None:
            ref_nhwc = ops.nchw_to_nhwc(ref_feature.detach())
        if self.hip_offset_heads:
            pk = self._packed_heads()
            fkey = "f16s_both" if propagate_any else "f16s_eval_only"
            if self.f16_split and fkey in pk:
                n_p, n_e = (2 * self.propagate_neighbors if propagate_any else 0), 2 * self.evaluate_neighbors
                a_, b_ = ops.offset_heads_f16s(ref_nhwc, *pk[fkey], n_p + n_e, n_p if propagate_any else n_e, self.dilation)
                propa_offsets, eval_offsets = (a_, b_) if propagate_any else (None, a_)
            elif self.heads_hook is not None and (hooked := self.heads_hook(self, ref_nhwc, propagate_any)) is not None:
                propa_offsets, eval_offsets = hooked
            else:
                propa_offsets = ops.conv2d(ref_nhwc, *pk["propa"], 2 * self.propagate_neighbors, 3, 1, self.dilation,
                                           self.dilation, out_nchw=True) if propagate_any else None
                eval_offsets = ops.conv2d(ref_nhwc, *pk["eval"], 2 * self.evaluate_neighbors, 3, 1, self.dilation,
                                          self.dilation, out_nchw=True)
        else:
            ref_feature = ref_feature.contiguous()
            propa_offsets = self.propa_conv(ref_feature).contiguous() if propagate_any else None
            eval_offsets = self.eval_conv(ref_feature).contiguous()
        feature_weight = self.feature_weight_net(ref_nhwc, eval_offsets, self._etable)
        return dict(ref_nhwc=ref_nhwc, propa_offsets=propa_offsets, eval_offsets=eval_offsets, feature_weight=feature_weight)

    def forward(self, ref_feature: torch.Tensor, src_features: List[torch.Tensor], ref_proj: torch.Tensor,
                src_projs: List[torch.Tensor], depth_min: torch.Tensor, depth_max: torch.Tensor, depth: torch.Tensor,
                view_weights: torch.Tensor, depth_shift: int = 0, vw_shift: int = 0, noise: Optional[torch.Tensor] = None,
                debug: Optional[list] = None, ref_nhwc: Optional[torch.Tensor] = None,
                src_nhwc: Optional[torch.Tensor] = None, rel_proj: Optional[torch.Tensor] = None,
                precomputed: Optional[dict] = None) -> Tuple[List[torch.Tensor], torch.Tensor, torch.Tensor]:
        if len(src_features) != len(src_projs):
            raise AssertionError("Patchmatch Evaluation: Different number of images and projection matrices")
        if not ref_feature.is_cuda:
            raise PmnError("patchmatchnet_amd.PatchMatch runs on a ROCm GPU only (no CPU fallback)")
        device = ref_feature.device
        batch, _, height, width = ref_feature.size()

        if precomputed is None:
            precomputed = self.prepare(ref_feature, ref_nhwc)
        ref_nhwc, propa_offsets = precomputed["ref_nhwc"], precomputed["propa_offsets"]
        eval_offsets, feature_weight = precomputed["eval_offsets"], precomputed["feature_weight"]
        if rel_proj is None:
            rel_proj = ops.relative_projection(src_projs, ref_proj)
        if src_nhwc is None:
            src_nhwc, sizes = ops.stack_sources_padded([f.detach() for f in src_features])
            rel_proj = ops.rescale_projection_rows(rel_proj, sizes, tuple(src_nhwc.shape[2:4]))
        rel_proj = rel_proj.contiguous()
        depth_min = depth_min.float().contiguous()
        depth_max = depth_max.float().contiguous()

        depth_sample = depth
        cur_shift = depth_shift
        score = torch.empty(0, device=device)
        depth_samples: List[torch.Tensor] = []
        for it in range(1, self.patchmatch_iteration + 1):
            is_inverse = self.stage == 1 and it == self.patchmatch_iteration
            first_random = is_empty(depth_sample)
            if first_random and noise is None:
                noise = torch.rand(size=(batch, 48, height, width), device=device)
            propagate = self.propagate_neighbors > 0 and not (self.stage == 1 and it == self.patchmatch_iteration)
            hyp, xnorm = ops.init_hypotheses(
                noise.contiguous() if first_random else None,
                None if first_random else depth_sample.detach().contiguous(), cur_shift, depth_min, depth_max,
                self.depth_initialization.patchmatch_num_sample, self.patchmatch_interval_scale,
                propa_offsets if propagate else None, self._ptable if propagate else None, height, width)
            rec = {} if debug is not None else None
            had_view_weights = not is_empty(view_weights)
            d, score, view_weights = self.evaluation(
                ref_feature=ref_feature, src_features=src_features, ref_proj=ref_proj, src_projs=src_projs, depth_sample=hyp,
                grid=None, weight=None, view_weights=view_weights, is_inverse=is_inverse,
                fused=dict(xnorm=xnorm, eval_offsets=eval_offsets, table=self._etable, feature_weight=feature_weight,
                           interval_scale=self.patchmatch_interval_scale, vw_shift=vw_shift, ref_nhwc=ref_nhwc,
                           src_nhwc=src_nhwc, rel_proj=rel_proj), debug=rec)
            if not had_view_weights:
                vw_shift = 0
            if rec is not None:
                rec.update(depth_sample=hyp, xnorm=xnorm, feature_weight=feature_weight, score=score, depth=d,
                           view_weights=view_weights, eval_offsets=eval_offsets, propa_offsets=propa_offsets)
                debug.append(rec)
            depth_sample = d.unsqueeze(1)
            cur_shift = 0
            depth_samples.append(depth_sample)
        return depth_samples, score, view_weights
```

Baseline: 393.5.

## Generate local inverse-depth hypotheses inside warp and aggregate kernels, skip unused scores

For stage-1 last iteration (no propagation, inverse sampling), hypotheses are computed on the fly inside the gather-correlate and aggregate kernels from the previous depth, instead of running init_hypotheses and reading a depth_sample tensor. The correlate kernel also writes xnorm. Score output is skipped for non-final iterations when not needed. This removes a kernel launch and a D-plane depth tensor write/read, at the cost of recomputing sample depths in two kernels and narrow shape constraints (C=16, G=4, 8 samples, K=9).

```diff
diff --git a/include/pmn_hip.h b/include/pmn_hip.h
--- a/include/pmn_hip.h
+++ b/include/pmn_hip.h
@@ -54,6 +54,22 @@
                           const float *feature_weight, const float *eval_offsets, const int *eval_table_host,
                           int K, float interval_scale, int is_inverse, int B, int D, int h, int w,
                           float *score_out, float *depth_out, void *stream);
+
+int pmn_aggregate_regress_opt(const float *cost, const float *depth_sample, const float *xnorm,
+                              const float *feature_weight, const float *eval_offsets, const int *eval_table_host,
+                              int K, float interval_scale, int is_inverse, int B, int D, int h, int w,
+                              float *score_out, float *depth_out, void *stream);
+
+int pmn_warp_correlate_local(const float *ref_nhwc, const float *src_nhwc, const void *src_view_table, const float *rel_proj,
+                             const float *prev_depth, int depth_shift, const float *depth_min, const float *depth_max,
+                             int num_sample, float interval_scale, const float *view_weights_in, int vw_shift,
+                             const float *similarity_mlp, int B, int N, int C, int G, int h, int w, int hs, int ws,
+                             float *cost_out, float *xnorm_out, void *stream);
+int pmn_aggregate_regress_local(const float *cost, const float *xnorm, const float *prev_depth, int depth_shift,
+                                const float *depth_min, const float *depth_max, int num_sample,
+                                const float *feature_weight, const float *eval_offsets, const int *eval_table_host,
+                                int K, float interval_scale, int B, int h, int w, float *score_out, float *depth_out,
+                                void *stream);
 
 int pmn_confidence(const float *score, int B, int D, int h, int w, int H, int W, float *confidence_out,
                    int *depth_index_out, void *stream);
diff --git a/patchmatchnet_amd/_lib.py b/patchmatchnet_amd/_lib.py
--- a/patchmatchnet_amd/_lib.py
+++ b/patchmatchnet_amd/_lib.py
@@ -44,6 +44,10 @@
     "pmn_warp_correlate_views": [_fp, _fp, _fp, _fp, _fp, _i, _fp, _fp, _i, _i, _i, _i, _i, _i, _i, _i, _i, _fp, _fp, _ip,
                                  _fp, _s],
     "pmn_aggregate_regress": [_fp, _fp, _fp, _fp, _fp, _hp, _i, _f, _i, _i, _i, _i, _i, _fp, _fp, _s],
+    "pmn_aggregate_regress_opt": [_fp, _fp, _fp, _fp, _fp, _hp, _i, _f, _i, _i, _i, _i, _i, _fp, _fp, _s],
+    "pmn_warp_correlate_local": [_fp, _fp, _fp, _fp, _fp, _i, _fp, _fp, _i, _f, _fp, _i, _fp, _i, _i, _i, _i, _i, _i, _i, _i, _fp, _fp,
+                                 _s],
+    "pmn_aggregate_regress_local": [_fp, _fp, _fp, _i, _fp, _fp, _i, _fp, _fp, _hp, _i, _f, _i, _i, _i, _fp, _fp, _s],
     "pmn_confidence": [_fp, _i, _i, _i, _i, _i, _i, _fp, _ip, _s],
     "pmn_conv2d": [_fp, _fp, _fp, _fp, _fp] + [_i] * 14 + [_s],
     "pmn_fpn_tail": [_fp] * 6 + [_i] * 6 + [_s],
diff --git a/patchmatchnet_amd/csrc/aggregate.hip b/patchmatchnet_amd/csrc/aggregate.hip
--- a/patchmatchnet_amd/csrc/aggregate.hip
+++ b/patchmatchnet_amd/csrc/aggregate.hip
@@ -1,6 +1,6 @@
 #include <cstring>
 
-#include "pmn_common.hpp"
+#include "hyp_local.hpp"
 #define PMN_DIV_DM1(acc, D) ((acc) / (float)((D) - 1))
 
 struct AggArgs {
@@ -165,8 +165,8 @@
     fw = a.fweight[((size_t)b * K + k) * hw + p];
 }
 
-template <int KMAX, int DQT>
-__global__ __launch_bounds__(PMN_BLOCK, (KMAX <= 9 ? 3 : 1)) void aggregate_regress_q4_kernel(const AggArgs a) {
+template <int KMAX, int DQT, bool LOCAL>
+__device__ __forceinline__ void aggregate_regress_q4_body(const AggArgs& a, const LocalHypArgs* l) {
 #pragma clang fp contract(off)
     __shared__ float red[PMN_BLOCK];
     const int h = a.h, w = a.w, hw = h * w, D = a.D, K = a.K, DQ = DQT > 0 ? DQT : D >> 2;
@@ -272,8 +272,8 @@
         const int d = 4 * q + j;
         const size_t o = ((size_t)b * D + d) * hw + p;
         const float prob = expf((s[j] - smax) - lse);
-        if (ok) a.score[o] = prob;
-        acc = acc + (a.is_inverse ? (float)d : a.depth[o]) * prob;
+        if (ok && a.score) a.score[o] = prob;
+        acc = acc + ((LOCAL || a.is_inverse) ? (float)d : a.depth[o]) * prob;
     }
     red[threadIdx.x] = acc;
     __syncthreads();
@@ -281,13 +281,33 @@
     acc = 0.0f;
     for (int i = 0; i < DQ; ++i) acc = acc + red[px * DQ + i];
     float out = acc;
-    if (a.is_inverse) {
-        const float inv_min = 1.0f / a.depth[((size_t)b * D + (D - 1)) * hw + p];
-        const float inv_max = 1.0f / a.depth[((size_t)b * D) * hw + p];
+    if (LOCAL || a.is_inverse) {
+        float first, last;
+        if constexpr (LOCAL) {
+            const PmnLocalRange lr = pmn_local_range(l->depth_min, l->depth_max, b, l->num_sample, l->interval_scale);
+            const float inv_prev = pmn_div(1.0f, pmn_local_prev(l->prev, b, y, x, h, w, l->depth_shift));
+            first = pmn_local_sample(lr, inv_prev, 0);
+            last = pmn_local_sample(lr, inv_prev, D - 1);
+        } else {
+            last = a.depth[((size_t)b * D + (D - 1)) * hw + p];
+            first = a.depth[((size_t)b * D) * hw + p];
+        }
+        const float inv_min = 1.0f / last;
+        const float inv_max = 1.0f / first;
         const float inv = inv_max + PMN_DIV_DM1(acc, D) * (inv_min - inv_max);
         out = 1.0f / inv;
     }
     a.depth_out[(size_t)b * hw + p] = out;
+}
+
+template <int KMAX, int DQT>
+__global__ __launch_bounds__(PMN_BLOCK, (KMAX <= 9 ? 3 : 1)) void aggregate_regress_q4_kernel(const AggArgs a) {
+    aggregate_regress_q4_body<KMAX, DQT, false>(a, nullptr);
+}
+
+template <int KMAX, int DQT>
+__global__ __launch_bounds__(PMN_BLOCK, 3) void aggregate_regress_local_kernel(const AggArgs a, const LocalHypArgs l) {
+    aggregate_regress_q4_body<KMAX, DQT, true>(a, &l);
 }
 
 template <int KMAX>
@@ -322,13 +342,15 @@
     return launch_agg_dl<KMAX, 1>(a, s);
 }
 
-extern "C" int pmn_aggregate_regress(const float* cost, const float* depth_sample, const float* xnorm,
-                                     const float* feature_weight, const float* eval_offsets, const int* eval_table_host,
-                                     int K, float interval_scale, int is_inverse, int B, int D, int h, int w,
-                                     float* score_out, float* depth_out, void* stream) {
-    if (!cost || !depth_sample || !xnorm || !feature_weight || !eval_offsets || !eval_table_host || !score_out ||
-        !depth_out)
+static bool agg_takes_q4(int K, int D) { return K <= 9 && D % 4 == 0; }
+
+extern "C" int pmn_aggregate_regress_opt(const float* cost, const float* depth_sample, const float* xnorm,
+                                         const float* feature_weight, const float* eval_offsets, const int* eval_table_host,
+                                         int K, float interval_scale, int is_inverse, int B, int D, int h, int w,
+                                         float* score_out, float* depth_out, void* stream) {
+    if (!cost || !depth_sample || !xnorm || !feature_weight || !eval_offsets || !eval_table_host || !depth_out)
         return PMN_ERR_ARG;
+    if (!score_out && !agg_takes_q4(K, D)) return PMN_ERR_ARG;
     if (B < 1 || D < 1 || h < 2 || w < 2) return PMN_ERR_ARG;
     if (K < 1 || K > PMN_MAX_NEIGHBORS || D > PMN_MAX_DEPTH) return PMN_ERR_SHAPE;
     if (is_inverse && D < 2) return PMN_ERR_ARG;
@@ -349,3 +371,49 @@
     if (K <= 9) return launch_agg<9>(a, (hipStream_t)stream);
     return launch_agg<17>(a, (hipStream_t)stream);
 }
+
+extern "C" int pmn_aggregate_regress(const float* cost, const float* depth_sample, const float* xnorm,
+                                     const float* feature_weight, const float* eval_offsets, const int* eval_table_host,
+                                     int K, float interval_scale, int is_inverse, int B, int D, int h, int w,
+                                     float* score_out, float* depth_out, void* stream) {
+    if (!score_out) return PMN_ERR_ARG;
+    return pmn_aggregate_regress_opt(cost, depth_sample, xnorm, feature_weight, eval_offsets, eval_table_host, K, interval_scale,
+                                     is_inverse, B, D, h, w, score_out, depth_out, stream);
+}
+
+extern "C" int pmn_aggregate_regress_local(const float* cost, const float* xnorm, const float* prev_depth, int depth_shift,
+                                           const float* depth_min, const float* depth_max, int num_sample,
+                                           const float* feature_weight, const float* eval_offsets, const int* eval_table_host,
+                                           int K, float interval_scale, int B, int h, int w, float* score_out, float* depth_out,
+                                           void* stream) {
+    if (!cost || !xnorm || !prev_depth || !depth_min || !depth_max || !feature_weight || !eval_offsets || !eval_table_host ||
+        !depth_out)
+        return PMN_ERR_ARG;
+    if (B < 1 || h < 2 || w < 2 || depth_shift < 0 || depth_shift > 1 || (depth_shift && ((h | w) & 1))) return PMN_ERR_ARG;
+    if (K != 9 || num_sample != 8) return PMN_ERR_SHAPE;
+    constexpr int DT = 8, DQ = DT / 4, NPX = PMN_BLOCK / DQ;
+    AggArgs a;
+    memset(&a, 0, sizeof(a));
+    a.cost = cost;
+    a.xnorm = xnorm;
+    a.fweight = feature_weight;
+    a.offsets = eval_offsets;
+    a.score = score_out;
+    a.depth_out = depth_out;
+    a.K = K;
+    a.is_inverse = 1;
+    a.B = B; a.D = DT; a.h = h; a.w = w;
+    a.interval_scale = interval_scale;
+    for (int i = 0; i < 2 * K; ++i) a.table[i] = eval_table_host[i];
+    LocalHypArgs l;
+    memset(&l, 0, sizeof(l));
+    l.prev = prev_depth;
+    l.depth_min = depth_min;
+    l.depth_max = depth_max;
+    l.depth_shift = depth_shift;
+    l.num_sample = num_sample;
+    l.interval_scale = interval_scale;
+    PMN_LAUNCH((aggregate_regress_local_kernel<9, DQ>), dim3((h * w + NPX - 1) / NPX, B), dim3(NPX * DQ), 0, (hipStream_t)stream, a, l);
+    PMN_CHECK_LAUNCH();
+    return PMN_OK;
+}
diff --git a/patchmatchnet_amd/csrc/gather_corr.hip b/patchmatchnet_amd/csrc/gather_corr.hip
--- a/patchmatchnet_amd/csrc/gather_corr.hip
+++ b/patchmatchnet_amd/csrc/gather_corr.hip
@@ -1,7 +1,7 @@
 #include <type_traits>
 
 #include "gather_common.hpp"
-
+#include "hyp_local.hpp"
 
 template <int LPI, int SL>
 __device__ __forceinline__ int group_bcast_i(int v) {
@@ -742,6 +742,117 @@
     }
     PMN_CHECK_LAUNCH();
     return PMN_OK;
+}
+
+template <int C, int G, int DT>
+__global__ __launch_bounds__(PMN_BLOCK, 4) void gather_corr_kernel_local(const GatherArgs a, const LocalHypArgs l) {
+    constexpr int LPI = C / 4, NPIX = PMN_BLOCK / LPI, CG = C / G, LPG = CG / 4, PAD = 32 / G;
+    constexpr int DSTEP = PMN_BLOCK / NPIX, NIT = DT / DSTEP, NI = NIT < 4 ? NIT : 4, RPL = DT / LPI;
+    constexpr int SS = NPIX * DT + PAD;
+    static_assert(CG == 4 || CG == 8, "group size must be 4 or 8 channels");
+    static_assert(NIT >= 1 && DT % LPI == 0, "DT covers the item-role stride and is a multiple of the lane-group size");
+
+    const int tid = threadIdx.x;
+    const int b = blockIdx.y;
+    const int tile = pmn_xcd_tile(blockIdx.x, a.ntiles);
+    const int N = a.N, h = a.h, w = a.w, hs = a.hs, ws = a.ws;
+    const int hw = h * w;
+    const int p0 = tile * NPIX;
+
+    extern __shared__ float4 smem4[];
+    float* simt = reinterpret_cast<float*>(smem4);
+    float* wlds_a = simt + ((G * SS + 3) & ~3);
+    for (int i = tid; i < PMN_MLP_FLOATS; i += PMN_BLOCK) wlds_a[i] = a.mlp_a[i];
+
+    const int pixA = tid % NPIX, dA0 = tid / NPIX;
+    const int pA = p0 + pixA;
+    const bool okA = pA < hw;
+    const int yA = okA ? pA / w : 0, xA = okA ? pA - yA * w : 0;
+
+    const int grp = tid / LPI, lc = tid % LPI;
+    const int pB = p0 + grp;
+    const bool okB = pB < hw;
+    float4 refq = make_float4(0.f, 0.f, 0.f, 0.f);
+    if (okB) refq = reinterpret_cast<const float4*>(a.ref)[((size_t)b * hw + pB) * LPI + lc];
+    const int yB = okB ? pB / w : 0, xB = okB ? pB - yB * w : 0;
+    const int wv = w >> a.vw_shift, hwv = (h >> a.vw_shift) * wv;
+    const int vw_idx = (yB >> a.vw_shift) * wv + (xB >> a.vw_shift);
+    const bool owner = (lc % LPG) == 0;
+    const int gB = lc / LPG;
+
+    float acc[DT];
+#pragma unroll
+    for (int d = 0; d < DT; ++d) acc[d] = 0.0f;
+    const float xf = (float)xB, yf = (float)yB;
+    float rdep[RPL];
+    {
+        const PmnLocalRange lr = pmn_local_range(l.depth_min, l.depth_max, b, l.num_sample, l.interval_scale);
+        const float inv_prev = pmn_div(1.0f, okB ? pmn_local_prev(l.prev, b, yB, xB, h, w, l.depth_shift) : 1.0f);
+#pragma unroll
+        for (int j = 0; j < RPL; ++j) {
+            const int d = lc + j * LPI;
+            rdep[j] = pmn_local_sample(lr, inv_prev, d);
+            if (okB) l.xnorm[((size_t)b * hw + pB) * DT + d] = pmn_local_xnorm(lr, rdep[j]);
+        }
+    }
+    for (int v = 0; v < N; ++v) {
+        const PmnPose lane_pose = pmn_make_pose(a.proj + ((size_t)b * N + v) * 16, xf, yf, h, w);
+        float rw00[RPL], rw01[RPL], rw10[RPL], rw11[RPL];
+        int roff[RPL];
+#pragma unroll
+        for (int j = 0; j < RPL; ++j) {
+            PmnTaps t;
+            t.off = 0;
+            t.w00 = t.w01 = t.w10 = t.w11 = 0.0f;
+            if (okB) {
+                float ix, iy;
+                pmn_pose_position(lane_pose, rdep[j], h, w, hs, ws, ix, iy);
+                t = pmn_make_taps(ix, iy, hs, ws);
+            }
+            rw00[j] = t.w00; rw01[j] = t.w01; rw10[j] = t.w10; rw11[j] = t.w11;
+            roff[j] = t.off;
+        }
+        const char* sbase = pmn_view_base<C>(a, v, b, hs, ws);
+        const unsigned lane_bytes = lc * 16u, row_bytes = (unsigned)ws * (C * 4);
+        const float vw = okB ? a.vw_in[((size_t)b * N + v) * hwv + vw_idx] : 0.0f;
+        constexpr int NB = 2;
+        static_assert(DT % NB == 0, "hypothesis bound is a multiple of the batch");
+#pragma unroll
+        for (int d0 = 0; d0 < DT; d0 += NB) {
+            PmnCorners cn[NB];
+            float4 wq[NB];
+#pragma unroll
+            for (int i = 0; i < NB; ++i) {
+                const int d = d0 + i;
+                int off;
+                bcast_record<LPI>(d % LPI, rw00[d / LPI], rw01[d / LPI], rw10[d / LPI], rw11[d / LPI], roff[d / LPI], wq[i], off);
+                cn[i] = load_corners<C>(sbase, (unsigned)off * (C * 4) + lane_bytes, row_bytes);
+            }
+            __builtin_amdgcn_sched_barrier(0);
+#pragma unroll
+            for (int i = 0; i < NB; ++i) acc[d0 + i] = mul_add_unfused(acc[d0 + i], blend_corners<LPG, CG>(cn[i], wq[i], refq), vw);
+            __builtin_amdgcn_sched_barrier(0);
+        }
+    }
+    if (owner) {
+#pragma unroll
+        for (int d = 0; d < DT; ++d) simt[gB * SS + d * NPIX + grp] = acc[d];
+    }
+    __syncthreads();
+    if (!okA) return;
+    float wtot = 1e-5f;
+    const int vwi = (yA >> a.vw_shift) * wv + (xA >> a.vw_shift);
+    for (int v = 0; v < N; ++v) wtot += a.vw_in[((size_t)b * N + v) * hwv + vwi];
+    float x[NIT][G], o[NIT];
+#pragma unroll
+    for (int j = 0; j < NIT; ++j) {
+        const int d = dA0 + j * DSTEP;
+#pragma unroll
+        for (int g = 0; g < G; ++g) x[j][g] = simt[g * SS + d * NPIX + pixA] / wtot;
+    }
+    mlp_items<G, NIT, NI>(wlds_a, x, o);
+#pragma unroll
+    for (int j = 0; j < NIT; ++j) a.out[((size_t)b * hw + pA) * DT + dA0 + j * DSTEP] = o[j];
 }
 
 
@@ -872,6 +983,46 @@
                                view_weights_out, vw_argmax_out, similarity_out, stream);
 }
 
+extern "C" int pmn_warp_correlate_local(const float* ref_nhwc, const float* src_nhwc, const void* src_view_table, const float* rel_proj,
+                                        const float* prev_depth, int depth_shift, const float* depth_min, const float* depth_max,
+                                        int num_sample, float interval_scale, const float* view_weights_in, int vw_shift,
+                                        const float* similarity_mlp, int B, int N, int C, int G, int h, int w, int hs, int ws,
+                                        float* cost_out, float* xnorm_out, void* stream) {
+    if (!ref_nhwc || (!src_nhwc && !src_view_table) || !rel_proj || !prev_depth || !depth_min || !depth_max || !view_weights_in ||
+        !similarity_mlp || !cost_out || !xnorm_out)
+        return PMN_ERR_ARG;
+    if (B < 1 || N < 1 || h < 2 || w < 2 || hs < 2 || ws < 2 || vw_shift < 0 || vw_shift > 2 || depth_shift < 0 || depth_shift > 1)
+        return PMN_ERR_ARG;
+    if (((h | w) & ((1 << vw_shift) - 1)) || (depth_shift && ((h | w) & 1))) return PMN_ERR_ARG;
+    if (C != 16 || G != 4 || num_sample != 8) return PMN_ERR_SHAPE;
+    constexpr int CT = 16, GT = 4, DT = 8, NPIX = PMN_BLOCK / (CT / 4), SS = NPIX * DT + 32 / GT;
+    GatherArgs a;
+    memset(&a, 0, sizeof(a));
+    a.ref = ref_nhwc;
+    a.src = src_view_table ? nullptr : src_nhwc;
+    a.src_tab = static_cast<const unsigned long long*>(src_view_table);
+    a.proj = rel_proj;
+    a.vw_in = view_weights_in;
+    a.mlp_a = similarity_mlp;
+    a.out = cost_out;
+    a.B = B; a.N = N; a.D = DT; a.h = h; a.w = w; a.hs = hs; a.ws = ws;
+    a.vw_shift = vw_shift;
+    a.ntiles = (h * w + NPIX - 1) / NPIX;
+    LocalHypArgs l;
+    memset(&l, 0, sizeof(l));
+    l.prev = prev_depth;
+    l.depth_min = depth_min;
+    l.depth_max = depth_max;
+    l.xnorm = xnorm_out;
+    l.depth_shift = depth_shift;
+    l.num_sample = num_sample;
+    l.interval_scale = interval_scale;
+    const size_t lds = (size_t)((GT * SS + 3) & ~3) * 4 + MLP_LDS_FLOATS * 4;
+    PMN_LAUNCH((gather_corr_kernel_local<CT, GT, DT>), dim3(a.ntiles, B), dim3(PMN_BLOCK), lds, (hipStream_t)stream, a, l);
+    PMN_CHECK_LAUNCH();
+    return PMN_OK;
+}
+
 extern "C" int pmn_feature_weight(const float* ref_nhwc, const float* eval_offsets, const int* eval_table_host,
                                   const float* mlp, int B, int C, int G, int K, int h, int w, float* out_feature_weight,
                                   void* stream) {
diff --git a/patchmatchnet_amd/csrc/hyp_local.hpp b/patchmatchnet_amd/csrc/hyp_local.hpp
--- /dev/null
+++ b/patchmatchnet_amd/csrc/hyp_local.hpp
@@ -0,0 +1,46 @@
+#pragma once
+#include "pmn_common.hpp"
+
+struct LocalHypArgs {
+    const float* prev;
+    const float* depth_min;
+    const float* depth_max;
+    float* xnorm;
+    int depth_shift, num_sample;
+    float interval_scale;
+};
+
+struct PmnLocalRange {
+    float inv_min, inv_max, interval, range, rrange;
+    int k0;
+};
+
+__device__ __forceinline__ PmnLocalRange pmn_local_range(const float* depth_min, const float* depth_max, int b, int num_sample,
+                                                         float interval_scale) {
+#pragma clang fp contract(off)
+    PmnLocalRange r;
+    r.inv_min = 1.0f / depth_min[b];
+    r.inv_max = 1.0f / depth_max[b];
+    r.interval = (r.inv_min - r.inv_max) * interval_scale;
+    r.range = r.inv_min - r.inv_max;
+    r.rrange = pmn_rcp_refined(r.range);
+    r.k0 = -((num_sample + 1) / 2);
+    return r;
+}
+
+__device__ __forceinline__ float pmn_local_prev(const float* prev, int b, int y, int x, int h, int w, int depth_shift) {
+    const int ws = w >> depth_shift;
+    return prev[(size_t)b * (h >> depth_shift) * ws + (size_t)(y >> depth_shift) * ws + (x >> depth_shift)];
+}
+
+__device__ __forceinline__ float pmn_local_sample(const PmnLocalRange& r, float inv_prev, int j) {
+#pragma clang fp contract(off)
+    float inv = inv_prev + r.interval * (float)(r.k0 + j);
+    inv = fminf(fmaxf(inv, r.inv_max), r.inv_min);
+    return pmn_div(1.0f, inv);
+}
+
+__device__ __forceinline__ float pmn_local_xnorm(const PmnLocalRange& r, float v) {
+#pragma clang fp contract(off)
+    return pmn_div_by(pmn_div(1.0f, v) - r.inv_max, r.range, r.rrange);
+}
diff --git a/patchmatchnet_amd/csrc/hypotheses.hip b/patchmatchnet_amd/csrc/hypotheses.hip
--- a/patchmatchnet_amd/csrc/hypotheses.hip
+++ b/patchmatchnet_amd/csrc/hypotheses.hip
@@ -1,6 +1,6 @@
 #include <cstring>
 
-#include "pmn_common.hpp"
+#include "hyp_local.hpp"
 #define PMN_DIV48(u) ((u) / 48.0f)
 #define PMN_DIV48R(u) pmn_div_by((u), 48.0f, r48)
 
@@ -144,12 +144,10 @@
     const int b = blockIdx.y;
     if (p >= hw) return;
     const int y = p / w, x = p - y * w;
-    const float inv_min = 1.0f / a.depth_min[b];
-    const float inv_max = 1.0f / a.depth_max[b];
+    const PmnLocalRange lr = pmn_local_range(a.depth_min, a.depth_max, b, a.num_sample, a.interval_scale);
+    const float inv_min = lr.inv_min, inv_max = lr.inv_max, interval = lr.interval;
     constexpr int D = D0T + KT;
-    const float interval = (inv_min - inv_max) * a.interval_scale;
-    const int k0 = -((a.num_sample + 1) / 2);
-    const int kc = k0 + a.num_sample / 2;
+    const int kc = lr.k0 + a.num_sample / 2;
     const bool from_noise = a.noise != nullptr;
     const float r48 = pmn_uniform(pmn_rcp_refined(48.0f));
 
@@ -168,18 +166,13 @@
             v[j] = pmn_div(1.0f, inv);
         }
     } else {
-        const float dprev =
-            a.depth[(size_t)b * (h >> a.depth_shift) * ws + (size_t)(y >> a.depth_shift) * ws + (x >> a.depth_shift)];
+        const float dprev = pmn_local_prev(a.depth, b, y, x, h, w, a.depth_shift);
         if (D0T == 1) {
             v[0] = dprev;
         } else {
             const float inv_prev = pmn_div(1.0f, dprev);
 #pragma unroll
-            for (int j = 0; j < D0T; ++j) {
-                float inv = inv_prev + interval * (float)(k0 + j);
-                inv = fminf(fmaxf(inv, inv_max), inv_min);
-                v[j] = pmn_div(1.0f, inv);
-            }
+            for (int j = 0; j < D0T; ++j) v[j] = pmn_local_sample(lr, inv_prev, j);
         }
     }
 
@@ -252,12 +245,11 @@
         }
     }
 
-    const float range = inv_min - inv_max, rrange = pmn_rcp_refined(range);
 #pragma unroll
     for (int j = 0; j < D; ++j) {
         const size_t o = ((size_t)b * D + j) * hw + p;
         a.depth_sample[o] = v[j];
-        a.xnorm[((size_t)b * hw + p) * D + j] = pmn_div_by(pmn_div(1.0f, v[j]) - inv_max, range, rrange);
+        a.xnorm[((size_t)b * hw + p) * D + j] = pmn_local_xnorm(lr, v[j]);
     }
 }
 
diff --git a/patchmatchnet_amd/net.py b/patchmatchnet_amd/net.py
--- a/patchmatchnet_amd/net.py
+++ b/patchmatchnet_amd/net.py
@@ -392,7 +392,8 @@
                 src_projs=list(src_proj), depth_min=depth_min, depth_max=depth_max, depth=depth,
                 view_weights=view_weights, depth_shift=depth_shift, vw_shift=vw_shift,
                 noise=noise if stage == self.stages - 1 else None, debug=dbg, ref_nhwc=ref_nhwc, src_nhwc=src_nhwc,
-                rel_proj=None if rel_all is None else rel_all[self.stages - 1 - stage], precomputed=precomputed.get(stage))
+                rel_proj=None if rel_all is None else rel_all[self.stages - 1 - stage], precomputed=precomputed.get(stage),
+                want_score=stage == 1 or debug is not None)
             if debug is not None:
                 debug[stage] = dbg
             depth_patchmatch[stage] = depths
diff --git a/patchmatchnet_amd/ops.py b/patchmatchnet_amd/ops.py
--- a/patchmatchnet_amd/ops.py
+++ b/patchmatchnet_amd/ops.py
@@ -2,7 +2,7 @@
 
 import ctypes
 import threading
-from typing import List, Optional, Sequence, Tuple
+from typing import List, NamedTuple, Optional, Sequence, Tuple
 
 import numpy as np
 import torch
@@ -369,11 +369,72 @@
         return out
 
 
-def warp_correlate(ref_nhwc: torch.Tensor, src_nhwc, rel_proj: torch.Tensor, depth_sample: torch.Tensor,
+class LocalHypotheses(NamedTuple):
+    prev: torch.Tensor
+    depth_shift: int
+    depth_min: torch.Tensor
+    depth_max: torch.Tensor
+    num_sample: int
+    interval_scale: float
+
+    @staticmethod
+    def covers(C: int, G: int, num_sample: int, K: int) -> bool:
+        return (C, G, num_sample, K) == (16, 4, 8, 9)
+
+    def check(self, B: int, h: int, w: int) -> None:
+        for n, t in (("prev", self.prev), ("depth_min", self.depth_min), ("depth_max", self.depth_max)):
+            _dev(t, "local." + n)
+        if tuple(self.prev.shape) != (B, 1, h >> self.depth_shift, w >> self.depth_shift) or self.depth_min.numel() != B or \
+                self.depth_max.numel() != B:
+            raise PmnError(f"local hypotheses: prev must be [B,1,{h >> self.depth_shift},{w >> self.depth_shift}], depth_min / depth_max [B]")
+
+
+def _warp_correlate_local(ref_nhwc, src_nhwc, rel_proj, local: LocalHypotheses, view_weights, vw_shift, similarity_mlp, G):
+    table = src_nhwc if isinstance(src_nhwc, SourceTable) else None
+    if table is None:
+        _dev(src_nhwc, "src_nhwc")
+    _dev(rel_proj, "rel_proj")
+    B, h, w, C = ref_nhwc.shape
+    N, Bs, hs, ws, Cs = src_nhwc.shape
+    D = local.num_sample
+    local.check(B, h, w)
+    if view_weights is None:
+        raise PmnError("warp_correlate: local hypotheses need view weights (the PixelwiseNet launch reads a hypothesis map)")
+    _dev(view_weights, "view_weights")
+    if Bs != B or Cs != C or tuple(rel_proj.shape) != (B, N, 4, 4):
+        raise PmnError("warp_correlate: inconsistent shapes")
+    if tuple(view_weights.shape) != (B, N, h >> vw_shift, w >> vw_shift):
+        raise PmnError("Patchmatch Evaluation: Different number of images and view weights")
+    dev = ref_nhwc.device
+    sim_p = _mlp_dev(similarity_mlp, "similarity_mlp").data_ptr()
+    cost = torch.empty((B, h, w, D), dtype=torch.float32, device=dev).permute(0, 3, 1, 2)
+    xn = torch.empty((B, h, w, D), dtype=torch.float32, device=dev).permute(0, 3, 1, 2)
+    _note((ref_nhwc, src_nhwc if table is None else table.table, rel_proj, local.prev, local.depth_min, local.depth_max, view_weights,
+           similarity_mlp), (cost, xn))
+    with torch.cuda.device(dev):
+        if _TIMING is not None and _TIMING_ON:
+            ev0, ev1 = torch.cuda.Event(enable_timing=True), torch.cuda.Event(enable_timing=True)
+            ev0.record()
+        check(_lib.lib().pmn_warp_correlate_local(
+            ref_nhwc.data_ptr(), None if table is not None else src_nhwc.data_ptr(), None if table is None else table.table.data_ptr(),
+            rel_proj.data_ptr(), local.prev.data_ptr(), int(local.depth_shift), local.depth_min.data_ptr(), local.depth_max.data_ptr(),
+            D, float(local.interval_scale), view_weights.data_ptr(), vw_shift, sim_p, B, N, C, G, h, w, hs, ws, cost.data_ptr(),
+            xn.data_ptr(), _stream(cost)), "pmn_warp_correlate_local")
+        if _TIMING is not None and _TIMING_ON:
+            ev1.record()
+            _TIMING.append((ev0, ev1, 4 * B * h * w * ((1 + N) * C + D + N + G * D), f"C{C}_D{D}_{h}x{w}_N{N}_vw"))
+    return cost, view_weights, None, None, xn
+
+
+def warp_correlate(ref_nhwc: torch.Tensor, src_nhwc, rel_proj: torch.Tensor, depth_sample: Optional[torch.Tensor],
                    view_weights: Optional[torch.Tensor], vw_shift: int, similarity_mlp: torch.Tensor,
                    pixelwise_mlp: Optional[torch.Tensor], G: int, want_similarity: bool = False,
-                   want_argmax: bool = False):
+                   want_argmax: bool = False, local: Optional[LocalHypotheses] = None):
     _dev(ref_nhwc, "ref_nhwc")
+    if local is not None:
+        if depth_sample is not None or want_similarity or want_argmax:
+            raise PmnError("warp_correlate: local hypotheses replace depth_sample and have no debug outputs")
+        return _warp_correlate_local(ref_nhwc, src_nhwc, rel_proj, local, view_weights, vw_shift, similarity_mlp, G)
     table = src_nhwc if isinstance(src_nhwc, SourceTable) else None
     if table is None:
         _dev(src_nhwc, "src_nhwc")
@@ -419,8 +480,8 @@
 
 
 def aggregate_regress(cost: torch.Tensor, depth_sample: torch.Tensor, xnorm: torch.Tensor, feature_weight_: torch.Tensor,
-                      eval_offsets: torch.Tensor, table: np.ndarray, interval_scale: float, is_inverse: bool
-                      ) -> Tuple[torch.Tensor, torch.Tensor]:
+                      eval_offsets: torch.Tensor, table: np.ndarray, interval_scale: float, is_inverse: bool,
+                      want_score: bool = True) -> Tuple[Optional[torch.Tensor], torch.Tensor]:
     for n, t in (("depth_sample", depth_sample), ("feature_weight", feature_weight_), ("eval_offsets", eval_offsets)):
         _dev(t, n)
     cost, xnorm = _dlast(cost, "cost"), _dlast(xnorm, "xnorm")
@@ -430,15 +491,39 @@
             tuple(feature_weight_.shape) != (B, K, h, w) or tuple(eval_offsets.shape) != (B, 2 * K, h, w):
         raise PmnError("aggregate_regress: inconsistent shapes")
     tab, tab_p = _host_i32(table, 2 * K, "table")
-    score = torch.empty((B, D, h, w), dtype=torch.float32, device=cost.device)
+    skip = not want_score and K <= 9 and D % 4 == 0
+    score = None if skip else torch.empty((B, D, h, w), dtype=torch.float32, device=cost.device)
     depth = torch.empty((B, h, w), dtype=torch.float32, device=cost.device)
     _note((cost, depth_sample, xnorm, feature_weight_, eval_offsets), (score, depth))
     with torch.cuda.device(cost.device):
-        check(_lib.lib().pmn_aggregate_regress(cost.data_ptr(), depth_sample.data_ptr(), xnorm.data_ptr(),
-                                               feature_weight_.data_ptr(), eval_offsets.data_ptr(), tab_p, K,
-                                               float(interval_scale), 1 if is_inverse else 0, B, D, h, w,
-                                               score.data_ptr(), depth.data_ptr(), _stream(cost)),
+        fn = _lib.lib().pmn_aggregate_regress_opt if skip else _lib.lib().pmn_aggregate_regress
+        check(fn(cost.data_ptr(), depth_sample.data_ptr(), xnorm.data_ptr(), feature_weight_.data_ptr(), eval_offsets.data_ptr(), tab_p,
+                 K, float(interval_scale), 1 if is_inverse else 0, B, D, h, w, _ptr(score), depth.data_ptr(), _stream(cost)),
               "pmn_aggregate_regress")
+    return (score if want_score else None), depth
+
+
+def aggregate_regress_local(cost: torch.Tensor, xnorm: torch.Tensor, local: LocalHypotheses, feature_weight_: torch.Tensor,
+                            eval_offsets: torch.Tensor, table: np.ndarray, interval_scale: float, want_score: bool = True
+                            ) -> Tuple[Optional[torch.Tensor], torch.Tensor]:
+    for n, t in (("feature_weight", feature_weight_), ("eval_offsets", eval_offsets)):
+        _dev(t, n)
+    cost, xnorm = _dlast(cost, "cost"), _dlast(xnorm, "xnorm")
+    B, D, h, w = cost.shape
+    K = feature_weight_.shape[1]
+    local.check(B, h, w)
+    if D != local.num_sample or tuple(xnorm.shape) != (B, D, h, w) or tuple(feature_weight_.shape) != (B, K, h, w) or \
+            tuple(eval_offsets.shape) != (B, 2 * K, h, w):
+        raise PmnError("aggregate_regress_local: inconsistent shapes")
+    tab, tab_p = _host_i32(table, 2 * K, "table")
+    score = torch.empty((B, D, h, w), dtype=torch.float32, device=cost.device) if want_score else None
+    depth = torch.empty((B, h, w), dtype=torch.float32, device=cost.device)
+    _note((cost, xnorm, local.prev, local.depth_min, local.depth_max, feature_weight_, eval_offsets), (score, depth))
+    with torch.cuda.device(cost.device):
+        check(_lib.lib().pmn_aggregate_regress_local(
+            cost.data_ptr(), xnorm.data_ptr(), local.prev.data_ptr(), int(local.depth_shift), local.depth_min.data_ptr(),
+            local.depth_max.data_ptr(), D, feature_weight_.data_ptr(), eval_offsets.data_ptr(), tab_p, K, float(interval_scale), B, h, w,
+            _ptr(score), depth.data_ptr(), _stream(cost)), "pmn_aggregate_regress_local")
     return score, depth
 
 
diff --git a/patchmatchnet_amd/patchmatch.py b/patchmatchnet_amd/patchmatch.py
--- a/patchmatchnet_amd/patchmatch.py
+++ b/patchmatchnet_amd/patchmatch.py
@@ -113,7 +113,8 @@
     def forward(self, ref_feature: torch.Tensor, src_features: List[torch.Tensor], ref_proj: torch.Tensor,
                 src_projs: List[torch.Tensor], depth_sample: torch.Tensor, grid: Optional[torch.Tensor],
                 weight: Optional[torch.Tensor], view_weights: torch.Tensor, is_inverse: bool, *,
-                fused: Optional[dict] = None, debug: Optional[dict] = None) -> Tuple[torch.Tensor, torch.Tensor, torch.Tensor]:
+                fused: Optional[dict] = None, debug: Optional[dict] = None, want_score: bool = True
+                ) -> Tuple[torch.Tensor, torch.Tensor, torch.Tensor]:
         N = len(src_features) if src_features is not None else fused["src_nhwc"].shape[0]
         if src_features is not None and src_projs is not None and len(src_features) != len(src_projs):
             raise AssertionError("Patchmatch Evaluation: Different number of images and projection matrices")
@@ -131,6 +132,14 @@
         if src_nhwc is None:
             src_nhwc, sizes = ops.stack_sources_padded([s.detach() for s in src_features])
             rel_proj = ops.rescale_projection_rows(rel_proj, sizes, tuple(src_nhwc.shape[2:4]))
+        local = f.get("local")
+        if local is not None:
+            cost, vw, _, _, xnorm = ops.warp_correlate(
+                ref_nhwc, src_nhwc, rel_proj.contiguous(), None, view_weights.contiguous(), int(f.get("vw_shift", 0)),
+                self.similarity_net.packed_device(), None, self.G, local=local)
+            score, depth = ops.aggregate_regress_local(cost, xnorm, local, f["feature_weight"], f["eval_offsets"], f["table"],
+                                                       f["interval_scale"], want_score=want_score)
+            return depth, (score if score is not None else torch.empty(0, device=depth.device)), vw.detach()
         depth_sample = depth_sample.contiguous()
         cost, vw, argmax, sim = ops.warp_correlate(
             ref_nhwc, src_nhwc, rel_proj.contiguous(), depth_sample, view_weights.contiguous() if have_vw else None,
@@ -139,7 +148,9 @@
             want_similarity=debug is not None, want_argmax=debug is not None and not have_vw)
         if fused is not None and grid is None:
             score, depth = ops.aggregate_regress(cost, depth_sample, f["xnorm"], f["feature_weight"], f["eval_offsets"],
-                                                 f["table"], f["interval_scale"], is_inverse)
+                                                 f["table"], f["interval_scale"], is_inverse, want_score=want_score)
+            if score is None:
+                score = torch.empty(0, device=depth.device)
         else:
             if grid is None or weight is None:
                 raise PmnError("Evaluation.forward needs grid and weight (reference signature) or the fused-form arguments")
@@ -194,6 +205,7 @@
 
         self.hip_offset_heads = True
         self.f16_split = True
+        self.local_hypotheses = True
         self.f16_domain_error: Optional[str] = None
         self.heads_hook = None
         self._heads = None
@@ -259,7 +271,8 @@
                 view_weights: torch.Tensor, depth_shift: int = 0, vw_shift: int = 0, noise: Optional[torch.Tensor] = None,
                 debug: Optional[list] = None, ref_nhwc: Optional[torch.Tensor] = None,
                 src_nhwc: Optional[torch.Tensor] = None, rel_proj: Optional[torch.Tensor] = None,
-                precomputed: Optional[dict] = None) -> Tuple[List[torch.Tensor], torch.Tensor, torch.Tensor]:
+                precomputed: Optional[dict] = None, want_score: bool = True
+                ) -> Tuple[List[torch.Tensor], torch.Tensor, torch.Tensor]:
         if len(src_features) != len(src_projs):
             raise AssertionError("Patchmatch Evaluation: Different number of images and projection matrices")
         if not ref_feature.is_cuda:
@@ -290,19 +303,28 @@
             if first_random and noise is None:
                 noise = torch.rand(size=(batch, 48, height, width), device=device)
             propagate = self.propagate_neighbors > 0 and not (self.stage == 1 and it == self.patchmatch_iteration)
-            hyp, xnorm = ops.init_hypotheses(
-                noise.contiguous() if first_random else None,
-                None if first_random else depth_sample.detach().contiguous(), cur_shift, depth_min, depth_max,
-                self.depth_initialization.patchmatch_num_sample, self.patchmatch_interval_scale,
-                propa_offsets if propagate else None, self._ptable if propagate else None, height, width)
+            num_sample = self.depth_initialization.patchmatch_num_sample
+            had_view_weights = not is_empty(view_weights)
+            local = None
+            if self.local_hypotheses and not propagate and not first_random and had_view_weights and is_inverse and debug is None and \
+                    ops.LocalHypotheses.covers(ref_nhwc.shape[-1], self.G, num_sample, self.evaluate_neighbors):
+                local = ops.LocalHypotheses(depth_sample.detach().contiguous(), cur_shift, depth_min, depth_max, num_sample,
+                                            self.patchmatch_interval_scale)
+                hyp = xnorm = None
+            else:
+                hyp, xnorm = ops.init_hypotheses(
+                    noise.contiguous() if first_random else None,
+                    None if first_random else depth_sample.detach().contiguous(), cur_shift, depth_min, depth_max,
+                    num_sample, self.patchmatch_interval_scale,
+                    propa_offsets if propagate else None, self._ptable if propagate else None, height, width)
             rec = {} if debug is not None else None
-            had_view_weights = not is_empty(view_weights)
+            keep_score = debug is not None or (want_score and it == self.patchmatch_iteration)
             d, score, view_weights = self.evaluation(
                 ref_feature=ref_feature, src_features=src_features, ref_proj=ref_proj, src_projs=src_projs, depth_sample=hyp,
                 grid=None, weight=None, view_weights=view_weights, is_inverse=is_inverse,
                 fused=dict(xnorm=xnorm, eval_offsets=eval_offsets, table=self._etable, feature_weight=feature_weight,
                            interval_scale=self.patchmatch_interval_scale, vw_shift=vw_shift, ref_nhwc=ref_nhwc,
-                           src_nhwc=src_nhwc, rel_proj=rel_proj), debug=rec)
+                           src_nhwc=src_nhwc, rel_proj=rel_proj, local=local), debug=rec, want_score=keep_score)
             if not had_view_weights:
                 vw_shift = 0
             if rec is not None:
```

New measurement: 396.2 (median of 6 runs). About the same (+0.7%).
